# TissueImageAnalytics/cerberus

Measured on AMD Instinct MI355X. Metric: Mpx/sec WSI tiled inference (all heads), higher is better.
Workload: dtype f32

## Files before the change

cerberus_amd/csrc/cerb_api.hip:

```cpp
#include "cerb_net.h"

static thread_local std::string g_err;
int cerb_set_error(const std::string& m) {
    g_err = m;
    return 1;
}
extern "C" int cerb_version(void) { return 4; }
extern "C" const char* cerb_last_error(void) { return g_err.c_str(); }
std::atomic<long long> g_devbuf_bytes{0};
extern "C" size_t cerb_device_bytes_held(void) { const long long v = g_devbuf_bytes.load(); return v > 0 ? (size_t)v : 0; }
thread_local hipStream_t g_call_stream = nullptr;

static int alloc_dev(cerb_net* net, size_t bytes, void** out) {
    if (net->reusing) {
        if (net->reuse_cursor >= net->n_finalize_allocs || net->dev_alloc_bytes[net->reuse_cursor] != bytes)
            return fail("reload: the tensors do not have the shapes the handle was finalized with");
        *out = net->dev_allocs[net->reuse_cursor++];
        return 0;
    }
    void* d = nullptr;
    HIP_OK(hipMalloc(&d, bytes));
    net->dev_allocs.push_back(d);
    net->dev_alloc_bytes.push_back(bytes);
    *out = d;
// ... 246 lines not shown
}

void cerb_host_pack_patch_class(const float* w1, const float* b1, const float* scale2, const float* shift2, const float* w2, const float* b2, int out_ch,
                                std::vector<float>* w1t_out, std::vector<float>* b1f_out, std::vector<float>* w2t_out, std::vector<float>* b2f_out) {
    std::vector<float>&w1t = *w1t_out, &b1f = *b1f_out, &w2t = *w2t_out, &b2f = *b2f_out;
    w1t.assign(512 * 256, 0.f); b1f.assign(256, 0.f); w2t.assign(256 * 16, 0.f); b2f.assign(16, 0.f);
    for (int o = 0; o < 256; ++o) {
        for (int c = 0; c < 512; ++c) w1t[(size_t)c * 256 + o] = w1[(size_t)o * 512 + c] * scale2[o];
        b1f[o] = b1[o] * scale2[o] + shift2[o];
    }
    for (int o = 0; o < out_ch; ++o) {
        for (int c = 0; c < 256; ++c) w2t[(size_t)c * 16 + o] = w2[(size_t)o * 256 + c];
        b2f[o] = b2[o];
    }
}

static int store_bn(cerb_net* net, const std::string& name, const std::vector<std::string>& bnkeys, int ch) {
    std::vector<float> ga, be;
    for (const std::string& k : bnkeys) {
        const HostTensor *w, *b;
        if (get(net, k + ".weight", {ch}, &w) || get(net, k + ".bias", {ch}, &b)) return 1;
        ga.insert(ga.end(), w->data.begin(), w->data.end());
        be.insert(be.end(), b->data.begin(), b->data.end());
    }
    cerb_net::BnDev d;
    d.C = ch;
    d.groups = (int)bnkeys.size();
    if (upload(net, ga, &d.gamma) || upload(net, be, &d.beta)) return 1;
    for (size_t g = 0; g < bnkeys.size(); ++g) {
        net->param_slots[bnkeys[g] + ".weight"].push_back({d.gamma + g * ch, ch});
        net->param_slots[bnkeys[g] + ".bias"].push_back({d.beta + g * ch, ch});
    }
    net->bn[name] = d;
    net->bn_keys[name] = bnkeys;
    return 0;
}

static int make_conv(cerb_net* net, const std::string& name, const std::vector<std::string>& wkeys,
                     const std::vector<std::string>& bkeys, const std::vector<std::string>& bnkeys, int cout, int cin, int ks,
                     int stride) {
    const int CB = cerb_conv_chunk(ks, stride);
    if (cout % 64 || cin % CB) return fail("conv " + name + ": unsupported channel counts");
    std::vector<float> wp, bp, wwino, hw;
    const bool wino = (ks == 3 && stride == 1 && cin % 32 == 0);
    for (size_t g = 0; g < wkeys.size(); ++g) {
        const HostTensor* w;
        if (get(net, wkeys[g], {cout, cin, ks, ks}, &w)) return 1;
        Fold f;
        bool have_bn = !bnkeys.empty() && net->fold_bn;
        if (have_bn && bn_fold(net, bnkeys[g], cout, &f)) return 1;
        if (net->fold_bn) {
            pack_conv(w->data.data(), have_bn ? f.scale.data() : nullptr, cout, cin, ks, CB, &wp);
            if (wino) {
                pack_wino(w->data.data(), have_bn ? f.scale.data() : nullptr, cout, cin, &wwino);
                const size_t b0 = hw.size();
                hw.insert(hw.end(), w->data.begin(), w->data.end());
                if (have_bn)
                    for (int co = 0; co < cout; ++co)
                        for (size_t e = 0; e < (size_t)cin * 9; ++e) hw[b0 + (size_t)co * cin * 9 + e] *= f.scale[co];
            }
        }
        const HostTensor* b = nullptr;
        if (!bkeys.empty() && get(net, bkeys[g], {cout}, &b)) return 1;
        for (int c = 0; c < cout; ++c) {
            float v = b ? b->data[c] : 0.f;
            if (have_bn) v = v * f.scale[c] + f.shift[c];
            bp.push_back(v);
        }
    }
    if (!net->fold_bn && !bnkeys.empty() && store_bn(net, name, bnkeys, cout)) return 1;
    if (!net->fold_bn) {
        std::vector<float> rw, rb;
        for (size_t g = 0; g < wkeys.size(); ++g) {
            const HostTensor* w;
            if (get(net, wkeys[g], {cout, cin, ks, ks}, &w)) return 1;
            rw.insert(rw.end(), w->data.begin(), w->data.end());
            if (!bkeys.empty()) {
                const HostTensor* b;
                if (get(net, bkeys[g], {cout}, &b)) return 1;
                rb.insert(rb.end(), b->data.begin(), b->data.end());
            }
        }
        cerb_net::RawW r;
        r.wkeys = wkeys; r.bkeys = bkeys; r.bnkeys = bnkeys;
        if (upload(net, rw, &r.w) || (!rb.empty() && upload(net, rb, &r.b))) return 1;
        for (size_t g = 0; g < wkeys.size(); ++g) {
            const long long nwg = (long long)cout * cin * ks * ks;
            net->param_slots[wkeys[g]].push_back({r.w + g * nwg, nwg});
            if (r.b) net->param_slots[bkeys[g]].push_back({r.b + g * cout, cout});
        }
        net->raw[name] = r;
    }
    PackedConv pc;
    pc.cin = cin; pc.cout = cout; pc.ks = ks; pc.stride = stride; pc.groups = (int)wkeys.size();
    if (upload(net, bp, &pc.b)) return 1;
    if (!net->fold_bn)
        for (size_t g = 0; g < bkeys.size(); ++g) net->param_slots[bkeys[g]].push_back({pc.b + g * cout, cout});
    if (net->fold_bn) {
        if (upload(net, wp, &pc.w)) return 1;
        if (wino && upload(net, wwino, &pc.wino)) return 1;
        pc.host_w.swap(hw);
    } else {
        const float* rawd = net->raw[name].w;
        const size_t G = wkeys.size(), nw = (size_t)cout * cin * ks * ks, nu = (size_t)cout * cin * 16;
        const bool dgrad = ks == 3 && cin % 64 == 0 && cout % 32 == 0;
        void *dwp = nullptr, *dwi = nullptr, *ddg = nullptr;
        if (alloc_dev(net, G * nw * 4, &dwp) || (wino && alloc_dev(net, G * nu * 4, &dwi)) || (dgrad && alloc_dev(net, G * nu * 4, &ddg))) return 1;
        pc.w = reinterpret_cast<float*>(dwp);
        pc.wino = reinterpret_cast<float*>(dwi);
        pc.wino_dgrad = reinterpret_cast<float*>(ddg);
        for (size_t g = 0; g < G; ++g) {
            HIP_OK(cerb_launch_pack_conv(rawd + g * nw, pc.w + g * nw, cout, cin, ks, CB, 0));
            if (wino) HIP_OK(cerb_launch_pack_wino(rawd + g * nw, pc.wino + g * nu, cout, cin, 0, 0));
            if (dgrad) HIP_OK(cerb_launch_pack_wino(rawd + g * nw, pc.wino_dgrad + g * nu, cin, cout, 1, 0));
        }
    }
    net->conv[name] = pc;
    return 0;
}


extern "C" int cerb_net_finalize(cerb_net* net) {
    if (!net) return fail("cerb_net_finalize: null handle");
    if (net->finalized) return 0;
    if (!net->fold_bn && net->trunk_idx.size() != net->dense_idx.size())
        return fail("cerb_net_finalize: a decoder with several output heads runs in inference only (the training tape sums one head's gradient per decoder)");
    {
        const HostTensor* w;
        if (get(net, "backbone.conv1.weight", {64, 3, 7, 7}, &w)) return 1;
        Fold f;
        if (bn_fold(net, "backbone.bn1", 64, &f)) return 1;
        if (!net->fold_bn) {
            f.scale.assign(64, 1.f);
            f.shift.assign(64, 0.f);
            if (store_bn(net, "stem", {"backbone.bn1"}, 64)) return 1;
        }
        std::vector<float> wp;
        cerb_host_pack_stem(w->data.data(), f.scale.data(), &wp);
        if (upload(net, wp, &net->stem_w) || upload(net, f.shift, &net->stem_b)) return 1;
        if (!net->fold_bn) {
            if (upload(net, w->data, &net->stem_raw)) return 1;
            net->param_slots["backbone.conv1.weight"].push_back({net->stem_raw, 64 * 147});
        }
    }
    int inpl = 64;
    for (int li = 0; li < 4; ++li) {
        const int planes = kFilters[li + 1];
        for (int b = 0; b < kLayers[li]; ++b) {
            const std::string p = "backbone.layer" + std::to_string(li + 1) + "." + std::to_string(b);
            const int stride = (b == 0 && li > 0) ? 2 : 1;
            if (make_conv(net, p + ".conv1", {p + ".conv1.weight"}, {}, {p + ".bn1"}, planes, inpl, 3, stride)) return 1;
            if (make_conv(net, p + ".conv2", {p + ".conv2.weight"}, {}, {p + ".bn2"}, planes, planes, 3, 1)) return 1;
            if (stride != 1 || inpl != planes)
                if (make_conv(net, p + ".downsample", {p + ".downsample.0.weight"}, {}, {p + ".downsample.1"}, planes, inpl, 1, stride)) return 1;
            inpl = planes;
        }
    }
    if (make_conv(net, "conv_map", {"conv_map.weight"}, {}, {}, 256, 512, 1, 1)) return 1;
    const int dec_in[4] = {256, 128, 64, 64};
    const int dec_u[4][2] = {{256, 128}, {128, 64}, {64, 64}, {64, 64}};
    if (!net->dense_idx.empty()) {
        for (int u = 0; u < 4; ++u) {
            int c = dec_in[u];
            for (int j = 0; j < 2; ++j) {
                std::vector<std::string> wk, bk, bnk;
                for (int di : net->trunk_idx) {
                    const std::string p = "decoder_head." + net->dec[di].name + "." + std::to_string(u) + ".block." + std::to_string(j);
                    wk.push_back(p + ".conv.weight");
                    bk.push_back(p + ".conv.bias");
                    bnk.push_back(p + ".bn");
                }
                if (make_conv(net, "dec." + std::to_string(u) + "." + std::to_string(j), wk, bk, bnk, dec_u[u][j], c, 3, 1)) return 1;
                c = dec_u[u][j];
            }
        }
        for (int di : net->dense_idx) {
            const DecoderCfg& d = net->dec[di];
            const std::string p = "output_head." + d.name + "." + d.head + ".x";
            const HostTensor *w1, *b1, *w2, *b2;
            Fold f;
            if (get(net, p + ".0.block.0.conv.weight", {96, 64, 1, 1}, &w1) || get(net, p + ".0.block.0.conv.bias", {96}, &b1) ||
                bn_fold(net, p + ".0.block.0.bn", 96, &f) || get(net, p + ".1.conv.weight", {d.out_ch, 96, 1, 1}, &w2) ||
                get(net, p + ".1.conv.bias", {d.out_ch}, &b2))
                return 1;
            std::vector<float> w1p, b1p, w2p, b2p, w2q;
            cerb_host_pack_head(w1->data.data(), b1->data.data(), f.scale.data(), f.shift.data(), w2->data.data(), b2->data.data(), d.out_ch, &w1p, &b1p, &w2p, &b2p, &w2q);
            if (!net->fold_bn) {
                float *r1, *rb1, *r2, *rb2;
                if (upload(net, w1->data, &r1) || upload(net, b1->data, &rb1) || upload(net, w2->data, &r2) || upload(net, b2->data, &rb2)) return 1;
                net->head_rw1.push_back(r1); net->head_rb1.push_back(rb1); net->head_rw2.push_back(r2); net->head_rb2.push_back(rb2);
                net->param_slots[p + ".0.block.0.conv.weight"].push_back({r1, 96 * 64});
                net->param_slots[p + ".0.block.0.conv.bias"].push_back({rb1, 96});
                net->param_slots[p + ".1.conv.weight"].push_back({r2, (long long)d.out_ch * 96});
                net->param_slots[p + ".1.conv.bias"].push_back({rb2, d.out_ch});
                if (store_bn(net, "head." + std::to_string(net->head_rw1.size() - 1), {p + ".0.block.0.bn"}, 96)) return 1;
            }
            float *dw1, *db1, *dw2, *db2;
            float* dw2q;
            if (upload(net, w1p, &dw1) || upload(net, b1p, &db1) || upload(net, w2p, &dw2) || upload(net, b2p, &db2) || upload(net, w2q, &dw2q)) return 1;
            net->head_w1.push_back(dw1); net->head_b1.push_back(db1); net->head_w2.push_back(dw2); net->head_b2.push_back(db2); net->head_w2q.push_back(dw2q);
        }
    }
    if (net->pc_idx >= 0) {
        const int oc = net->dec[net->pc_idx].out_ch;
        const std::string p = "decoder_head.Patch-Class";
        Fold f1, f2;
        const HostTensor *w1, *b1, *w2, *b2;
        if (bn_fold(net, p + ".bn1", 512, &f1) || bn_fold(net, p + ".bn2", 256, &f2) || get(net, p + ".conv1.weight", {256, 512, 1, 1}, &w1) ||
            get(net, p + ".conv1.bias", {256}, &b1) || get(net, p + ".conv2.weight", {oc, 256, 1, 1}, &w2) || get(net, p + ".conv2.bias", {oc}, &b2))
            return 1;
        if (!net->fold_bn) {
            if (upload(net, w1->data, &net->pc_rw1) || upload(net, b1->data, &net->pc_rb1) || upload(net, w2->data, &net->pc_rw2) ||
                upload(net, b2->data, &net->pc_rb2) || store_bn(net, "pc.bn1", {p + ".bn1"}, 512) || store_bn(net, "pc.bn2", {p + ".bn2"}, 256))
                return 1;
            net->param_slots[p + ".conv1.weight"].push_back({net->pc_rw1, 256 * 512});
            net->param_slots[p + ".conv1.bias"].push_back({net->pc_rb1, 256});
            net->param_slots[p + ".conv2.weight"].push_back({net->pc_rw2, (long long)oc * 256});
            net->param_slots[p + ".conv2.bias"].push_back({net->pc_rb2, oc});
        }
        std::vector<float> w1t, b1f, w2t, b2f;
        cerb_host_pack_patch_class(w1->data.data(), b1->data.data(), f2.scale.data(), f2.shift.data(), w2->data.data(), b2->data.data(), oc, &w1t, &b1f, &w2t, &b2f);
        if (upload(net, f1.scale, &net->pc_bn1s) || upload(net, f1.shift, &net->pc_bn1b) || upload(net, w1t, &net->pc_w1t) ||
            upload(net, b1f, &net->pc_b1) || upload(net, w2t, &net->pc_w2t) || upload(net, b2f, &net->pc_b2))
            return 1;
    }
    if (!net->fold_bn) {
        std::vector<float> z(512, 0.f);
        if (upload(net, z, &net->zero_bias)) return 1;
    }
    if (!net->fold_bn) HIP_OK(hipDeviceSynchronize());
    if (net->reusing && net->reuse_cursor != net->n_finalize_allocs) return fail("reload: fewer tensors than the handle was finalized with");
    if (!net->reusing) net->n_finalize_allocs = net->dev_allocs.size();
    net->reusing = false;
    net->host.clear();
    net->finalized = true;
    return 0;
}

int prof_begin(cerb_net* net, const std::string& name, const std::string& kernel, double flops, hipStream_t st) {
    if (!net->profiling) return 0;
    if (net->prof_n == net->prof.size()) {
        cerb_net::ProfRec r;
        HIP_OK(hipEventCreate(&r.e0));
        HIP_OK(hipEventCreate(&r.e1));
        net->prof.push_back(r);
    }
    cerb_net::ProfRec& r = net->prof[net->prof_n];
    r.name = name; r.kernel = kernel; r.flops = flops;
    HIP_OK(hipEventRecord(r.e0, st));
    net->prof_open = true;
    return 0;
}
int prof_end(cerb_net* net, hipStream_t st) {
    if (!net->profiling) return 0;
    HIP_OK(hipEventRecord(net->prof[net->prof_n].e1, st));
    net->prof_n++;
    net->prof_open = false;
    return 0;
}

int train_wino2_fresh(cerb_net* net, const std::string& name, PackedConv& cm, int dgrad, hipStream_t st) {
    if (net->fold_bn) return 0;
    bool& used = dgrad ? cm.wino_dgrad_used : cm.wino_used;
    bool& stale = dgrad ? cm.wino_dgrad_stale : cm.wino_stale;
    used = true;
    if (!stale) return 0;
    auto rit = net->raw.find(name);
    if (rit == net->raw.end()) return fail("conv " + name + ": no raw weights to re-pack");
    const size_t nw = (size_t)cm.cout * cm.cin * 9, nu = (size_t)cm.cout * cm.cin * 16;
    for (int g = 0; g < cm.groups; ++g)
        HIP_OK(cerb_launch_pack_wino(rit->second.w + g * nw, (dgrad ? cm.wino_dgrad : cm.wino) + g * nu, dgrad ? cm.cin : cm.cout, dgrad ? cm.cout : cm.cin, dgrad, st));
    stale = false;
    return 0;
}

int train_wino4_slot(cerb_net* net, const std::string& name, PackedConv& cm, int w4b, int dgrad, hipStream_t st, float** out) {
    float*& slot = cm.wino4_t[w4b][dgrad];
    if (!slot) {
        auto rit = net->raw.find(name);
        if (rit == net->raw.end()) return fail("conv " + name + ": no raw weights for the F(4x4) transform");
        const size_t nw = (size_t)cm.cout * cm.cin * 9, nu = (size_t)cm.cout * cm.cin * 36;
        void* d = nullptr;
        HIP_OK(hipMalloc(&d, (size_t)cm.groups * nu * 4));
        net->dev_allocs.push_back(d);
        net->dev_alloc_bytes.push_back((size_t)cm.groups * nu * 4);
        slot = (float*)d;
        (void)nw;
        HIP_OK(cerb_launch_pack_wino4(rit->second.w, slot, dgrad ? cm.cin : cm.cout, dgrad ? cm.cout : cm.cin, dgrad, w4b, cm.groups, st));
    }
    *out = slot;
    return 0;
}

static constexpr int kPlanarLowest = 0;
static constexpr int kEncPlanarStages = 0x7;
static const char* const kPlanarFamily[4] = {"conv_wino4_planar<f4x4,16x16x2,eighth-res>", "conv_wino4_planar<f4x4,16x16x2,quarter-res>",
                                             "conv_wino4p<f4x4,16x16x2,planar,half-res>", "conv_wino4p<f4x4,16x16x2,planar>"};
static const char* const kEncPlanarFamily = "conv_wino4_enc<f4x4,16x16x2>";
static const char* const kEncPlanarFamilyRes = "conv_wino4_enc<f4x4,16x16x2,res>";
static const char* const kPlanarEntryFamily[4] = {"upsample2_add_planar<eighth-res>", "upsample2_add_planar<quarter-res>", "upsample2_add_planar", "upsample2_add_planar"};

int run_conv(cerb_net* net, const std::string& name, const float* in, const float* prev, const float* resid, float* out, int N,
             int H, int W, int relu, int mode, long long in_gs, long long prev_gs, hipStream_t st, double* macs,
             const int* roi, long long planar_out_gs) {
    auto it = net->conv.find(name);
    if (it == net->conv.end()) return fail("internal: conv " + name + " not packed");
    const PackedConv& c = it->second;
    struct BnReq {
        cerb_net* n;
        ~BnReq() { n->conv_bn_part = nullptr; }
    } bn_req{net};
    net->conv_bn_bpg = 0;
    ConvParams p;
    memset(&p, 0, sizeof(p));
    p.in = in; p.prev = prev; p.wpack = c.w; p.bias = c.b; p.resid = resid; p.out = out;
    p.N = N; p.H = H; p.W = W; p.Cin = c.cin; p.Cout = c.cout;
    p.Ho = (c.stride == 2) ? H / 2 : H;
    p.Wo = (c.stride == 2) ? W / 2 : W;
    p.relu = relu;
    p.groups = c.groups;
    p.in_gs = in_gs; p.prev_gs = prev_gs;
    p.w_gs = (long long)c.cout * c.cin * c.ks * c.ks;
    p.bias_gs = c.cout;
    p.resid_gs = 0;
    p.out_gs = (long long)N * p.Ho * p.Wo * c.cout;
    p.pk_off = net->packed_items ? 0 : 1;
    if (macs) {
        *macs += (double)c.groups * N * p.Ho * p.Wo * (double)c.cout * c.cin * c.ks * c.ks;
        if (!out) return 0;
    }
    const double fl = 2.0 * (double)c.groups * N * p.Ho * p.Wo * (double)c.cout * c.cin * c.ks * c.ks;
    const long long map_px = (long long)p.Ho * p.Wo;
    const bool use_w4 = net->conv_algo == 5 || net->conv_algo == 7 || (net->conv_algo == 6 && map_px >= 256);
    const bool planar = planar_out_gs > 0;
    static const long long w4b_max_px = [] {
        const char* e = cerb_dev_getenv("CERB_W4B_MAX_PX");
        return e ? atoll(e) : 4096ll;
    }();
    const bool w4b = !planar && (net->conv_algo == 7 || (net->conv_algo == 6 && map_px <= w4b_max_px)) && c.cin % 64 == 0;
    const bool enc_planar = planar && net->planar_level == 4;
    if (enc_planar && c.stride == 2) {
        if (resid || mode != 0 || !net->fold_bn) return fail("internal: conv " + name + " cannot store tile-planar");
        p.out_gs = planar_out_gs;
        p.pl_byp = cerb_planar_blocks(p.Ho);
        p.pl_bxp = cerb_planar_blocks(p.Wo);
        const std::string kn = "conv_igemm_planar<ks" + std::to_string(c.ks) + ",s2" + (p.Wo < 32 ? ",16x16>" : ",8x32>");
        if (prof_begin(net, name, kn, fl, st)) return 1;
        HIP_OK(cerb_launch_conv(p, c.ks, c.stride, mode, st));
        if (prof_end(net, st)) return 1;
        return 0;
    }
    if (planar && !(use_w4 && c.wino && mode == 0 && net->fold_bn && (!resid || enc_planar))) return fail("internal: conv " + name + " cannot take the planar path");
    if (use_w4 && c.wino && mode == 0 && (!it->second.host_w.empty() || !net->fold_bn)) {
        PackedConv& cm = it->second;
        float* train_slot = nullptr;
        if (!net->fold_bn && train_wino4_slot(net, name, cm, w4b ? 1 : 0, 0, st, &train_slot)) return 1;
        float*& slot4 = !net->fold_bn ? train_slot : (w4b ? cm.wino4b : cm.wino4);
        if (!slot4) {
            std::vector<float> w4;
            for (int g = 0; g < cm.groups; ++g) pack_wino4(cm.host_w.data() + (size_t)g * cm.cout * cm.cin * 9, cm.cout, cm.cin, &w4, w4b ? 1 : 0);
            void* d = nullptr;
            HIP_OK(hipMalloc(&d, w4.size() * 4));
            net->dev_allocs.push_back(d);
            net->dev_alloc_bytes.push_back(w4.size() * 4);
            HIP_OK(hipMemcpy(d, w4.data(), w4.size() * 4, hipMemcpyHostToDevice));
            slot4 = (float*)d;
        }
        p.wpack = slot4;
        p.w_gs = (long long)c.cout * c.cin * 36;
        double fl_done = fl;
        if (roi && roi[1] > roi[0] && roi[3] > roi[2]) {
            p.roi_y0 = roi[0]; p.roi_y1 = roi[1]; p.roi_x0 = roi[2]; p.roi_x1 = roi[3];
            const double ty = (roi[1] + 15) / 16 - roi[0] / 16, tx = (roi[3] + 15) / 16 - roi[2] / 16;
            fl_done = fl * (ty * 16.0 * tx * 16.0) / ((double)p.Ho * p.Wo);
        }
        if (planar) {
            p.out_gs = planar_out_gs;
            p.level_tag = enc_planar ? (resid ? 4 : 3) : net->planar_level == 3 ? 1 : net->planar_level == 2 ? 0 : 2;
            p.pl_byp = cerb_planar_blocks(p.Ho);
            p.pl_bxp = cerb_planar_blocks(p.Wo);
        }
        if (prof_begin(net, name, enc_planar ? (resid ? kEncPlanarFamilyRes : kEncPlanarFamily) : planar ? kPlanarFamily[net->planar_level & 3] : w4b ? (cerb_wino4b_packed(p) ? (resid ? "conv_wino4b<f4x4,16t,res>" : "conv_wino4b<f4x4,16t>") : (resid ? "conv_wino4b<f4x4,16x16,res>" : "conv_wino4b<f4x4,16x16>")) : (resid ? "conv_wino4<f4x4,16x16x2,res>" : "conv_wino4<f4x4,16x16x2>"), fl_done, st)) return 1;
        if (net->conv_bn_part && !planar && !resid && !(roi && roi[1] > roi[0] && roi[3] > roi[2])) {
            p.bn_part = net->conv_bn_part;
            net->conv_bn_bpg = w4b ? cerb_wino4b_bn_blocks(p) : N * ((p.Ho + 15) / 16) * ((p.Wo + 15) / 16);
        }
        HIP_OK(planar ? cerb_launch_wino4p(p, st) : w4b ? cerb_launch_wino4b(p, st) : cerb_launch_wino4(p, st));
        if (prof_end(net, st)) return 1;
        return 0;
    }
    if (net->conv_algo && c.wino && mode == 0) {
        if (train_wino2_fresh(net, name, it->second, 0, st)) return 1;
        p.wpack = c.wino;
        p.w_gs = (long long)c.cout * c.cin * 16;
        double fl_done = fl;
        if (roi && roi[1] > roi[0] && roi[3] > roi[2]) {
            p.roi_y0 = roi[0]; p.roi_y1 = roi[1]; p.roi_x0 = roi[2]; p.roi_x1 = roi[3];
            const double ty = (roi[1] + 7) / 8 - roi[0] / 8, tx = (roi[3] + 15) / 16 - roi[2] / 16;
            fl_done = fl * (ty * 8.0 * tx * 16.0) / ((double)p.Ho * p.Wo);
        }
        if (prof_begin(net, name, resid ? "conv_wino<f2x2,8x16,res>" : "conv_wino<f2x2,8x16>", fl_done, st)) return 1;
        HIP_OK(cerb_launch_wino(p, st));
        if (prof_end(net, st)) return 1;
        return 0;
    }
    const std::string kn = "conv_igemm<ks" + std::to_string(c.ks) + ",s" + std::to_string(c.stride) + ",mode" + std::to_string(mode) +
                           (p.Wo < 32 ? ",16x16>" : ",8x32>");
    if (prof_begin(net, name, kn, fl, st)) return 1;
    HIP_OK(cerb_launch_conv(p, c.ks, c.stride, mode, st));
    if (prof_end(net, st)) return 1;
    return 0;
}

static int forward_impl(cerb_net* net, const cerb_forward_io* io, hipStream_t st, double* macs) {
    g_call_stream = st;
    const bool dry = (macs != nullptr) && (io->tiles == nullptr) && (io->tiles_f32 == nullptr);
    const int N = io->n, H = io->h, W = io->w;
    if (N <= 0 || H <= 0 || W <= 0 || (H % 16) || (W % 16)) return fail("cerb_net_forward: tile H,W must be positive multiples of 16");
    const int out_h = io->out_h > 0 ? io->out_h : H, out_w = io->out_w > 0 ? io->out_w : W;
    if (out_h > H || out_w > W) return fail("cerb_net_forward: crop larger than tile");
    const int hs[5] = {H, H / 2, H / 4, H / 8, H / 16}, ws[5] = {W, W / 2, W / 4, W / 8, W / 16};
    const size_t D = net->trunk_idx.size();
    const size_t guard = cerb_conv_guard_bytes(W);
    const int planar_lowest = [] {
        const char* e = cerb_dev_getenv("CERB_PLANAR_LOWEST");
        return e ? atoi(e) : kPlanarLowest;
    }();
    auto level_is_planar = [&](int u) {
        if (dry || !net->planar || !net->fold_bn || net->conv_algo != 6 || net->head_algo < 1) return false;
        for (int v = 3; v >= u; --v) {
            if (v < planar_lowest) return false;
            auto c0 = net->conv.find("dec." + std::to_string(v) + ".0"), c1 = net->conv.find("dec." + std::to_string(v) + ".1");
            if (c0 == net->conv.end() || c1 == net->conv.end() || !c0->second.wino || !c1->second.wino) return false;
            const long long px = (long long)hs[3 - v] * ws[3 - v];
            if ((hs[3 - v] & 3) || (ws[3 - v] & 3)) return false;
            const bool ok = v >= 2 ? px >= 4096 && c0->second.cin == 64 && c0->second.cout == 64 && c1->second.cout == 64
                                   : px >= 256 && c0->second.cin % 16 == 0 && c0->second.cout % 64 == 0 && c1->second.cin == c0->second.cout && c1->second.cout % 64 == 0;
            if (!ok) return false;
        }
        return true;
    };
    if (!dry) {
        if (net->x0.ensure((size_t)N * H * W * 64 * 4, guard) || net->pool.ensure((size_t)N * hs[1] * ws[1] * 64 * 4, guard)) return fail_alloc();
        for (int i = 1; i < 5; ++i)
            if (net->x[i].ensure((size_t)N * hs[i] * ws[i] * kFilters[i] * 4, guard)) return fail_alloc();
        if (net->ta.ensure((size_t)N * hs[1] * ws[1] * 64 * 4, guard) || net->tb.ensure((size_t)N * hs[1] * ws[1] * 64 * 4, guard) ||
            net->cm.ensure((size_t)N * hs[4] * ws[4] * 256 * 4, guard))
            return fail_alloc();
        if (D) {
            static const bool exact_ws = cerb_dev_getenv("CERB_LEGACY_WS") == nullptr;
            size_t need_sum = 0, need_mid = 0;
            const int oc[4] = {128, 64, 64, 64};
            for (int u = 0; u < 4; ++u) {
                if (exact_ws && level_is_planar(u)) continue;
                const std::string n0 = "dec." + std::to_string(u) + ".0";
                auto c0 = net->conv.find(n0);
                const size_t px = (size_t)D * N * hs[3 - u] * ws[3 - u];
                need_sum = std::max(need_sum, px * (size_t)(c0 != net->conv.end() ? c0->second.cin : 256) * 4);
                need_mid = std::max(need_mid, px * (size_t)(c0 != net->conv.end() ? c0->second.cout : 256) * 4);
            }
            if (!exact_ws) need_sum = need_mid = D * (size_t)N * H * W * 64 * 4;
            if (net->dmid.ensure(need_mid, guard)) return fail_alloc();
            if (net->conv_algo && net->dsum.ensure(need_sum, guard)) return fail_alloc();
            for (int u = 0; u < 4; ++u) {
                if (exact_ws && level_is_planar(u)) continue;
                if (net->dout[u].ensure(D * (size_t)N * hs[3 - u] * ws[3 - u] * oc[u] * 4, guard)) return fail_alloc();
            }
        }
    }
    if (macs) *macs += (double)N * H * W * 64.0 * 147.0;
    if (!dry) {
        StemParams sp;
        sp.tiles = io->tiles; sp.tiles_f32 = io->tiles ? nullptr : io->tiles_f32; sp.wpack = net->stem_w; sp.bias = net->stem_b; sp.out = net->x0.p; sp.N = N; sp.H = H; sp.W = W; sp.relu = 1;
        sp.tiles_x = sp.tiles_y = 0;
        if (prof_begin(net, "stem", "stem_conv7x7", 2.0 * N * H * W * 64.0 * 147.0, st)) return 1;
        HIP_OK(cerb_launch_stem(sp, st));
        if (prof_end(net, st)) return 1;
    }
    const int enc_mask = [] {
        const char* e = cerb_dev_getenv("CERB_ENC_PLANAR");
        return e ? atoi(e) : kEncPlanarStages;
    }();
    auto encoder_stage_is_planar = [&](int li) {
        if (dry || !net->planar || !net->fold_bn || net->conv_algo != 6 || !((enc_mask >> li) & 1)) return false;
        const int hh = hs[li + 1], ww = ws[li + 1], planes = kFilters[li + 1];
        if ((hh & 15) || (ww & 15) || hh < 16 || ww < 16 || planes % 64) return false;
        for (int b = 0; b < kLayers[li]; ++b)
            for (int j = 1; j <= 2; ++j) {
                auto c = net->conv.find("backbone.layer" + std::to_string(li + 1) + "." + std::to_string(b) + ".conv" + std::to_string(j));
                if (c == net->conv.end()) return false;
                if (c->second.stride == 1 && (!c->second.wino || c->second.host_w.empty() || c->second.cin % 16)) return false;
            }
        return true;
    };
    if (!dry) {
        if (encoder_stage_is_planar(0)) {
            if (net->enc_a[0].ensure(1, N, hs[1], ws[1], 64, st)) return fail_alloc();
            if (prof_begin(net, "maxpool", "maxpool3x3s2_planar", 0.0, st)) return 1;
            HIP_OK(cerb_launch_maxpool_planar(net->x0.p, net->enc_a[0].b.p, N, H, W, 64, st));
            if (prof_end(net, st)) return 1;
        } else {
            if (prof_begin(net, "maxpool", "maxpool3x3s2", 0.0, st)) return 1;
            HIP_OK(cerb_launch_maxpool(net->x0.p, net->pool.p, N, H, W, 64, st));
            if (prof_end(net, st)) return 1;
        }
    }
    float* cur = dry ? nullptr : net->pool.p;
    int inpl = 64;
    for (int li = 0; li < 4; ++li) {
        const int planes = kFilters[li + 1];
        const int Hi = (li == 0) ? hs[1] : hs[li], Wi = (li == 0) ? ws[1] : ws[li];
        if (encoder_stage_is_planar(li)) {
            PlanarBuf &ba = net->enc_a[li], &bb = net->enc_b[li];
            const int hh = hs[li + 1], ww = ws[li + 1];
            if (ba.ensure(1, N, hh, ww, planes, st) || bb.ensure(1, N, hh, ww, planes, st)) return fail_alloc();
            const int keep_level = net->planar_level;
            net->planar_level = 4;
            struct Restore { cerb_net* n; int v; ~Restore() { n->planar_level = v; } } restore{net, keep_level};
            for (int b = 0; b < kLayers[li]; ++b) {
                const std::string p = "backbone.layer" + std::to_string(li + 1) + "." + std::to_string(b);
                if (b == 0 && li > 0) {
                    if (run_conv(net, p + ".conv1", cur, nullptr, nullptr, bb.b.p, N, Hi, Wi, 1, 0, 0, 0, st, macs, nullptr, bb.gs())) return 1;
                    if (run_conv(net, p + ".downsample", cur, nullptr, nullptr, ba.b.p, N, Hi, Wi, 0, 0, 0, 0, st, macs, nullptr, ba.gs())) return 1;
                } else if (run_conv(net, p + ".conv1", ba.b.p, nullptr, nullptr, bb.b.p, N, hh, ww, 1, 0, ba.gs(), 0, st, macs, nullptr, bb.gs())) {
                    return 1;
                }
                if (run_conv(net, p + ".conv2", bb.b.p, nullptr, ba.b.p, ba.b.p, N, hh, ww, 1, 0, bb.gs(), 0, st, macs, nullptr, ba.gs())) return 1;
            }
            if (prof_begin(net, "backbone.layer" + std::to_string(li + 1) + ".exit", "planar_to_nhwc", 0.0, st)) return 1;
            HIP_OK(cerb_launch_planar_to_nhwc(ba.b.p, net->x[li + 1].p, N, hh, ww, planes, st));
            if (prof_end(net, st)) return 1;
            cur = net->x[li + 1].p;
            inpl = planes;
            continue;
        }
        for (int b = 0; b < kLayers[li]; ++b) {
            const std::string p = "backbone.layer" + std::to_string(li + 1) + "." + std::to_string(b);
            const int stride = (b == 0 && li > 0) ? 2 : 1;
            const int hin = (b == 0) ? Hi : hs[li + 1], win = (b == 0) ? Wi : ws[li + 1];
            float* t1 = dry ? nullptr : net->ta.p;
            const bool last = (b == kLayers[li] - 1);
            float* outb = dry ? nullptr : (((kLayers[li] - 1 - b) % 2 == 0) ? net->x[li + 1].p : net->tb.p);
            (void)last;
            const float* idt = cur;
            if (run_conv(net, p + ".conv1", cur, nullptr, nullptr, t1, N, hin, win, 1, 0, 0, 0, st, macs)) return 1;
            if (stride != 1 || inpl != planes) {
                float* ds = dry ? nullptr : net->pool.p;
                if (run_conv(net, p + ".downsample", cur, nullptr, nullptr, ds, N, hin, win, 0, 0, 0, 0, st, macs)) return 1;
                idt = ds;
            }
            if (run_conv(net, p + ".conv2", t1, nullptr, idt, outb, N, hs[li + 1], ws[li + 1], 1, 0, 0, 0, st, macs)) return 1;
            cur = outb;
            inpl = planes;
        }
    }
    if (run_conv(net, "conv_map", dry ? nullptr : net->x[4].p, nullptr, nullptr, dry ? nullptr : net->cm.p, N, hs[4], ws[4], 0, 0, 0, 0, st, macs)) return 1;

    const long long tile_stride = io->tile_stride ? io->tile_stride : (long long)out_h * out_w;
    const long long row_stride = io->row_stride ? io->row_stride : out_w;
    if (net->pc_idx >= 0) {
        if (macs) *macs += (double)N * (512.0 * 256 + 256.0 * net->dec[net->pc_idx].out_ch);
        const bool want = io->out && io->out[net->pc_idx];
        const bool wantl = io->logits && io->logits[net->pc_idx];
        if (!dry && (want || wantl)) {
            PatchClassParams pp;
            memset(&pp, 0, sizeof(pp));
            pp.x4 = net->x[4].p; pp.bn1_s = net->pc_bn1s; pp.bn1_b = net->pc_bn1b; pp.w1t = net->pc_w1t; pp.b1 = net->pc_b1;
            pp.w2t = net->pc_w2t; pp.b2 = net->pc_b2;
            pp.N = N; pp.Hf = hs[4]; pp.Wf = ws[4]; pp.out_ch = net->dec[net->pc_idx].out_ch;
            pp.out_h = out_h; pp.out_w = out_w;
            pp.logits = wantl ? io->logits[net->pc_idx] : nullptr;
            pp.out = want ? (float*)io->out[net->pc_idx] : nullptr;
            pp.tile_off = io->tile_off; pp.tile_stride = tile_stride; pp.row_stride = row_stride;
            if (prof_begin(net, "patch_class", "patch_class", 2.0 * N * (512.0 * 256 + 256.0 * pp.out_ch), st)) return 1;
            HIP_OK(cerb_launch_patch_class(pp, st));
            if (prof_end(net, st)) return 1;
        }
    }
    if (D) {
        const float* skips[4] = {dry ? nullptr : net->x[3].p, dry ? nullptr : net->x[2].p, dry ? nullptr : net->x[1].p, dry ? nullptr : net->x0.p};
        const float* prev = dry ? nullptr : net->cm.p;
        long long prev_gs = 0;
        const int oc[4] = {128, 64, 64, 64};
        int roi_out[4][4], roi_mid[4][4], roi_sum[4][4];
        const bool any_logits = [&] {
            if (!io->logits) return false;
            for (size_t k = 0; k < net->dec.size(); ++k)
                if (io->logits[k]) return true;
            return false;
        }();
        const bool use_roi = !dry && net->crop_roi && (net->conv_algo == 1 || net->conv_algo >= 5) && !any_logits && (out_h < H || out_w < W);
        if (use_roi) {
            int y0 = (int)((H - out_h) * 0.5), x0 = (int)((W - out_w) * 0.5), y1 = y0 + out_h, x1 = x0 + out_w;
            for (int u = 3; u >= 0; --u) {
                const int hh = hs[3 - u], ww = ws[3 - u];
                auto widen = [&](int* r, const int* in, int d) {
                    r[0] = std::max(0, (in[0] - d) & ~3); r[1] = std::min(hh, (in[1] + d + 3) & ~3);
                    r[2] = std::max(0, (in[2] - d) & ~3); r[3] = std::min(ww, (in[3] + d + 3) & ~3);
                };
                const int win[4] = {y0, y1, x0, x1};
                widen(roi_out[u], win, 0);
                widen(roi_mid[u], roi_out[u], 1);
                widen(roi_sum[u], roi_mid[u], 1);
                y0 = std::max(0, roi_sum[u][0] / 2 - 1); y1 = std::min(hh / 2, (roi_sum[u][1] - 1) / 2 + 2);
                x0 = std::max(0, roi_sum[u][2] / 2 - 1); x1 = std::min(ww / 2, (roi_sum[u][3] - 1) / 2 + 2);
            }
        }
        bool feat_planar = false, prev_planar = false;
        for (int u = 0; u < 4; ++u) {
            const int hh = hs[3 - u], ww = ws[3 - u];
            const std::string n0 = "dec." + std::to_string(u) + ".0", n1 = "dec." + std::to_string(u) + ".1";
            const int cmid = net->conv[n0].cout;
            const int cin0 = net->conv[n0].cin;
            const bool lvl_planar = level_is_planar(u);
            if (lvl_planar) {
                PlanarBuf &bs = u == 3 ? net->psum : u == 2 ? net->psum2 : u == 1 ? net->psum1 : net->psum0;
                PlanarBuf &bm = u == 3 ? net->pmid : u == 2 ? net->pmid2 : u == 1 ? net->pmid1 : net->pmid0;
                const int cout1 = net->conv[n1].cout;
                PlanarBuf& bo = cout1 == cin0 ? bs : u == 1 ? net->pout1 : net->pout0;
                if (bs.ensure((int)D, N, hh, ww, cin0, st) || bm.ensure((int)D, N, hh, ww, cmid, st) || (&bo != &bs && bo.ensure((int)D, N, hh, ww, cout1, st)))
                    return fail_alloc();
                if (prof_begin(net, n0 + ".up", kPlanarEntryFamily[u], 0.0, st)) return 1;
                HIP_OK(cerb_launch_upsample2_add_planar(skips[u], prev, bs.b.p, (int)D, N, hh, ww, cin0, prev_gs, bs.gs(), use_roi ? roi_sum[u] : nullptr, prev_planar ? 1 : 0, st));
                if (prof_end(net, st)) return 1;
                net->planar_level = u;
                if (run_conv(net, n0, bs.b.p, nullptr, nullptr, bm.b.p, N, hh, ww, 1, 0, bs.gs(), 0, st, macs, use_roi ? roi_mid[u] : nullptr, bm.gs()))
                    return 1;
                if (run_conv(net, n1, bm.b.p, nullptr, nullptr, bo.b.p, N, hh, ww, 1, 0, bm.gs(), 0, st, macs, use_roi ? roi_out[u] : nullptr, bo.gs()))
                    return 1;
                if (u == 3) feat_planar = true;
                prev = bo.b.p;
                prev_gs = bo.gs();
                prev_planar = true;
                continue;
            }
            if (prev_planar) return fail("internal: a tile-planar decoder level feeds an NHWC one");
            if (net->conv_algo && net->conv[n0].wino && !dry) {
                if (prof_begin(net, n0 + ".up", "upsample2_add", 0.0, st)) return 1;
                HIP_OK(cerb_launch_upsample2_add(skips[u], prev, net->dsum.p, (int)D, N, hh, ww, cin0, prev_gs, use_roi ? roi_sum[u] : nullptr, st));
                if (prof_end(net, st)) return 1;
                if (run_conv(net, n0, net->dsum.p, nullptr, nullptr, net->dmid.p, N, hh, ww, 1, 0, (long long)N * hh * ww * cin0, 0, st, macs,
                             use_roi ? roi_mid[u] : nullptr))
                    return 1;
            } else if (run_conv(net, n0, skips[u], prev, nullptr, dry ? nullptr : net->dmid.p, N, hh, ww, 1, 1, 0, prev_gs, st, macs)) return 1;
            if (run_conv(net, n1, dry ? nullptr : net->dmid.p, nullptr, nullptr, dry ? nullptr : net->dout[u].p, N, hh, ww, 1, 0,
                         (long long)N * hh * ww * cmid, 0, st, macs, use_roi ? roi_out[u] : nullptr))
                return 1;
            prev = dry ? nullptr : net->dout[u].p;
            prev_gs = (long long)N * hh * ww * oc[u];
        }
        HeadParams hps[8];
        int n_hp = 0;
        double head_flops = 0.0;
        for (size_t k = 0; k < net->dense_idx.size(); ++k) {
            const int di = net->dense_idx[k];
            const size_t tk = (size_t)net->trunk_of[k];
            const DecoderCfg& d = net->dec[di];
            if (macs) *macs += (double)N * H * W * (64.0 * 96 + 96.0 * d.out_ch);
            const bool want = io->out && io->out[di];
            const bool wantl = io->logits && io->logits[di];
            if (dry || !(want || wantl)) continue;
            HeadParams hp;
            memset(&hp, 0, sizeof(hp));
            hp.feat = feat_planar ? net->psum.b.p + tk * net->psum.gs() : net->dout[3].p + tk * (size_t)N * H * W * 64;
            hp.feat_planar = feat_planar ? 1 : 0;
            hp.pl_byp = cerb_planar_blocks(H);
            hp.pl_bxp = cerb_planar_blocks(W);
            hp.w1p = net->head_w1[k]; hp.b1 = net->head_b1[k]; hp.w2p = net->head_w2[k]; hp.b2 = net->head_b2[k]; hp.w2q = net->head_w2q[k];
            hp.N = N; hp.H = H; hp.W = W; hp.out_ch = d.out_ch; hp.kind = d.kind;
            hp.crop_y0 = (int)((H - out_h) * 0.5); hp.crop_x0 = (int)((W - out_w) * 0.5);
            hp.out_h = want ? out_h : 0; hp.out_w = want ? out_w : 0;
            hp.roi = use_roi ? 1 : 0;
            hp.logits = wantl ? io->logits[di] : nullptr;
            hp.absmax_bits = io->logit_absmax ? io->logit_absmax + di : nullptr;
            if (want) {
                if (d.kind == 0) hp.out_inst = (float*)io->out[di];
                else if (io->type_is_u8) hp.out_type_u8 = (unsigned char*)io->out[di];
                else hp.out_type_i64 = (long long*)io->out[di];
            }
            hp.tile_off = io->tile_off; hp.tile_stride = tile_stride; hp.row_stride = row_stride;
            const double head_px = hp.roi ? (double)out_h * (((hp.crop_x0 + out_w + 15) / 16 - hp.crop_x0 / 16) * 16.0) : (double)H * W;
            const double fl = 2.0 * N * head_px * (64.0 * 96 + 96.0 * d.out_ch);
            if (net->head_algo == 0) {
                if (prof_begin(net, "head." + d.name, "head", fl, st)) return 1;
                HIP_OK(cerb_launch_head(hp, st));
                if (prof_end(net, st)) return 1;
            } else {
                if (n_hp == 8) {
                    if (prof_begin(net, "heads", "head_group", head_flops, st)) return 1;
                    HIP_OK(cerb_launch_head_group(hps, n_hp, st, net->head_algo == 1 ? 1 : 0));
                    if (prof_end(net, st)) return 1;
                    n_hp = 0;
                    head_flops = 0.0;
                }
                hps[n_hp++] = hp;
                head_flops += fl;
            }
        }
        if (n_hp > 0) {
            if (prof_begin(net, "heads", "head_group", head_flops, st)) return 1;
            HIP_OK(cerb_launch_head_group(hps, n_hp, st, net->head_algo == 1 ? 1 : 0));
            if (prof_end(net, st)) return 1;
        }
    }
    if (!dry && io->feats) {
        const float* src[6] = {net->x0.p, net->x[1].p, net->x[2].p, net->x[3].p, net->cm.p, net->x[4].p};
        const size_t nb[6] = {(size_t)N * H * W * 64, (size_t)N * hs[1] * ws[1] * 64, (size_t)N * hs[2] * ws[2] * 128,
                              (size_t)N * hs[3] * ws[3] * 256, (size_t)N * hs[4] * ws[4] * 256, (size_t)N * hs[4] * ws[4] * 512};
        for (int i = 0; i < 6; ++i)
            if (io->feats[i]) HIP_OK(hipMemcpyAsync(io->feats[i], src[i], nb[i] * 4, hipMemcpyDeviceToDevice, st));
    }
    return 0;
}

extern "C" int cerb_net_begin_reload(cerb_net* net) {
    if (!net) return fail("cerb_net_begin_reload: null handle");
    HIP_OK(hipDeviceSynchronize());
    while (net->dev_allocs.size() > net->n_finalize_allocs) {
        (void)hipFree(net->dev_allocs.back());
        net->dev_allocs.pop_back();
        net->dev_alloc_bytes.pop_back();
    }
    net->reusing = true;
    net->reuse_cursor = 0;
    net->param_slots.clear();
    net->conv.clear();
    net->bn.clear();
    net->raw.clear();
    net->grads.clear();
    net->head_w1.clear(); net->head_b1.clear(); net->head_w2.clear(); net->head_b2.clear(); net->head_w2q.clear();
    net->head_rw1.clear(); net->head_rb1.clear(); net->head_rw2.clear(); net->head_rb2.clear();
    net->host.clear();
    net->finalized = false;
    return 0;
}
extern "C" int cerb_net_update_params(cerb_net* net, int count, const char* const* keys, const float* const* dev_src, void* hip_stream) {
    if (!net || count < 0 || (count && (!keys || !dev_src))) return fail("cerb_net_update_params: bad arguments");
    if (!net->finalized || net->fold_bn) return fail("cerb_net_update_params: needs a finalized handle packed for training (cerb_net_set_fold_bn(net, 0))");
    hipStream_t st = (hipStream_t)hip_stream;
    std::vector<float*> cd;
    std::vector<const float*> cs;
    std::vector<long long> cn;
    for (int i = 0; i < count; ++i) {
        auto it = net->param_slots.find(keys[i]);
        if (it == net->param_slots.end()) continue;
        if (!dev_src[i]) return fail(std::string("cerb_net_update_params: null source for ") + keys[i]);
        for (const cerb_net::ParamSlot& sl : it->second) {
            cd.push_back(sl.dst); cs.push_back(dev_src[i]); cn.push_back(sl.n);
        }
    }
    HIP_OK(cerb_launch_copy_multi((int)cd.size(), cd.data(), cs.data(), cn.data(), &net->copy_tab, &net->copy_tab_bytes, &net->copy_tab_host, st));
    HIP_OK(cerb_launch_pack_stem(net->stem_raw, net->stem_w, st));
    static const bool per_conv = cerb_dev_getenv("CERB_PACK_PER_CONV") != nullptr;
    std::vector<PackJob> jobs;
    auto job = [&](const float* w, float* out, long long total, int cout, int cin, int kind, int a, int b) { jobs.push_back(PackJob{w, out, total, cout, cin, kind, a, b, 0}); };
    for (auto& kv : net->conv) {
        PackedConv& pc = kv.second;
        const float* rawd = net->raw[kv.first].w;
        if (pc.wino && !pc.wino_used) pc.wino_stale = true;
        if (pc.wino_dgrad && !pc.wino_dgrad_used) pc.wino_dgrad_stale = true;
        const size_t nw = (size_t)pc.cout * pc.cin * pc.ks * pc.ks, nu = (size_t)pc.cout * pc.cin * 16, nu4 = (size_t)pc.cout * pc.cin * 36;
        for (int g = 0; g < pc.groups; ++g) {
            if (per_conv) {
                HIP_OK(cerb_launch_pack_conv(rawd + g * nw, pc.w + g * nw, pc.cout, pc.cin, pc.ks, cerb_conv_chunk(pc.ks, pc.stride), st));
                if (pc.wino && pc.wino_used) HIP_OK(cerb_launch_pack_wino(rawd + g * nw, pc.wino + g * nu, pc.cout, pc.cin, 0, st));
                if (pc.wino_dgrad && pc.wino_dgrad_used) HIP_OK(cerb_launch_pack_wino(rawd + g * nw, pc.wino_dgrad + g * nu, pc.cin, pc.cout, 1, st));
                continue;
            }
            job(rawd + g * nw, pc.w + g * nw, (long long)nw, pc.cout, pc.cin, 0, pc.ks * pc.ks, cerb_conv_chunk(pc.ks, pc.stride));
            if (pc.wino && pc.wino_used) job(rawd + g * nw, pc.wino + g * nu, (long long)nu, pc.cout, pc.cin, 1, 0, 0);
            if (pc.wino_dgrad && pc.wino_dgrad_used) job(rawd + g * nw, pc.wino_dgrad + g * nu, (long long)nu, pc.cin, pc.cout, 1, 1, 0);
        }
        for (int l = 0; l < 2; ++l)
            for (int dg = 0; dg < 2; ++dg)
                if (pc.wino4_t[l][dg]) {
                    if (per_conv) {
                        HIP_OK(cerb_launch_pack_wino4(rawd, pc.wino4_t[l][dg], dg ? pc.cin : pc.cout, dg ? pc.cout : pc.cin, dg, l, pc.groups, st));
                        continue;
                    }
                    for (int g = 0; g < pc.groups; ++g)
                        job(rawd + g * nw, pc.wino4_t[l][dg] + g * nu4, (long long)nu4, dg ? pc.cin : pc.cout, dg ? pc.cout : pc.cin, 2, dg, l);
                }
    }
    if (!jobs.empty()) HIP_OK(cerb_launch_pack_multi(jobs.data(), (int)jobs.size(), &net->pack_tab, &net->pack_tab_bytes, &net->pack_tab_host, st));
    return 0;
}
extern "C" int cerb_net_set_fold_bn(cerb_net* net, int fold) {
    if (!net) return fail("cerb_net_set_fold_bn: null handle");
    if (net->finalized) return fail("cerb_net_set_fold_bn: must be called before cerb_net_finalize");
    net->fold_bn = fold ? 1 : 0;
    return 0;
}

extern "C" int cerb_net_forward(cerb_net* net, const cerb_forward_io* io, void* hip_stream) {
    if (!net || !io) return fail("cerb_net_forward: null argument");
    if (!net->finalized) return fail("cerb_net_forward: call cerb_net_finalize first");
    if (!io->tiles && !io->tiles_f32) return fail("cerb_net_forward: null tiles pointer (neither tiles nor tiles_f32)");
    if (!net->fold_bn) return fail("cerb_net_forward: the network was packed for training (cerb_net_set_fold_bn(net, 0)); use cerb_net_forward_train");
    net->prof_n = 0;
    return forward_impl(net, io, (hipStream_t)hip_stream, nullptr);
}

extern "C" double cerb_net_flops(const cerb_net* net, int n, int h, int w) {
    if (!net || !net->finalized) return -1.0;
    cerb_forward_io io;
    memset(&io, 0, sizeof(io));
    io.n = n; io.h = h; io.w = w;
    double macs = 0.0;
    if (forward_impl(const_cast<cerb_net*>(net), &io, nullptr, &macs)) return -1.0;
    return 2.0 * macs;
}

extern "C" int cerb_net_set_crop_roi(cerb_net* net, int enable) {
    if (!net) return fail("cerb_net_set_crop_roi: null handle");
    net->crop_roi = enable ? 1 : 0;
    return 0;
}
extern "C" int cerb_net_set_conv_algo(cerb_net* net, int algo) {
    if (!net) return fail("cerb_net_set_conv_algo: null handle");
    if (algo < 0 || algo > 7 || (algo >= 2 && algo <= 4))
        return fail("cerb_net_set_conv_algo: algo must be 0 (direct), 1 (Winograd F(2x2) fp32), 5 (Winograd F(4x4) fp32), 7 (F(4x4), one-block items with 32-channel chunks) or 6 (F(4x4) for maps of 16 x 16 pixels and more -- 7's kernel up to 64 x 64, 5's above --, else F(2x2): the default); 2-4 were experiments (scripts/experiments/)");
    net->conv_algo = algo;
    return 0;
}

extern "C" int cerb_net_set_bn_eval(cerb_net* net, const char* bn_prefix, const float* running_mean, const float* running_var, int channels) {
    if (!net || !bn_prefix) return fail("cerb_net_set_bn_eval: null argument");
    if (!net->finalized || net->fold_bn) return fail("cerb_net_set_bn_eval: needs a finalized network packed with cerb_net_set_fold_bn(net, 0)");
    for (auto& kv : net->bn_keys) {
        const std::vector<std::string>& keys = kv.second;
        for (size_t g = 0; g < keys.size(); ++g) {
            if (keys[g] != bn_prefix) continue;
            auto it = net->bn.find(kv.first);
            if (it == net->bn.end()) return fail(std::string("cerb_net_set_bn_eval: internal: no BatchNorm ") + kv.first);
            cerb_net::BnDev& b = it->second;
            if (!running_mean || !running_var) {
                if (g < b.eval.size()) b.eval[g] = 0;
                return 0;
            }
            if (channels != b.C) return fail(std::string("cerb_net_set_bn_eval: ") + bn_prefix + " has " + std::to_string(b.C) + " channels");
            if (!b.run_mean) {
                void* d = nullptr;
                HIP_OK(hipMalloc(&d, (size_t)2 * b.groups * b.C * 4));
                net->dev_allocs.push_back(d);
                net->dev_alloc_bytes.push_back((size_t)2 * b.groups * b.C * 4);
                b.run_mean = (float*)d;
                b.run_rstd = b.run_mean + (size_t)b.groups * b.C;
                b.eval.assign(b.groups, 0);
            }
            std::vector<float> rs(b.C);
            for (int c = 0; c < b.C; ++c) rs[c] = 1.0f / sqrtf(running_var[c] + 1e-5f);
            HIP_OK(hipMemcpy(b.run_mean + g * b.C, running_mean, (size_t)b.C * 4, hipMemcpyHostToDevice));
            HIP_OK(hipMemcpy(b.run_rstd + g * b.C, rs.data(), (size_t)b.C * 4, hipMemcpyHostToDevice));
            b.eval[g] = 1;
            return 0;
        }
    }
    return fail(std::string("cerb_net_set_bn_eval: no BatchNorm with the state-dict prefix ") + bn_prefix);
}

extern "C" int cerb_net_set_planar(cerb_net* net, int enable) {
    if (!net) return fail("cerb_net_set_planar: null handle");
    if (enable < 0 || enable > 1) return fail("cerb_net_set_planar: 0 (NHWC) or 1 (tile-planar, conv_wino4p.hip)");
    net->planar = enable;
    return 0;
}

extern "C" int cerb_net_set_packed_items(cerb_net* net, int enable) {
    if (!net) return fail("cerb_net_set_packed_items: null handle");
    if (enable < 0 || enable > 1) return fail("cerb_net_set_packed_items: 0 (16 x 16 blocks everywhere) or 1 (16 consecutive tiles per item on maps that are not whole blocks)");
    net->packed_items = enable;
    return 0;
}

extern "C" int cerb_net_set_head_algo(cerb_net* net, int algo) {
    if (!net) return fail("cerb_net_set_head_algo: null handle");
    if (algo < 0 || algo > 2) return fail("cerb_net_set_head_algo: algo must be 0 (one launch per head), 1 (grouped launch) or 2 (round 3's grouped launch)");
    net->head_algo = algo;
    return 0;
}

extern "C" int cerb_net_profile_enable(cerb_net* net, int enable) {
    if (!net) return fail("cerb_net_profile_enable: null handle");
    net->profiling = enable != 0;
    net->prof_n = 0;
    return 0;
}
extern "C" int cerb_net_profile_count(cerb_net* net) { return net ? (int)net->prof_n : 0; }
extern "C" int cerb_net_profile_get(cerb_net* net, int idx, char* name, int name_cap, char* kernel, int kernel_cap, double* flops, float* ms) {
    if (!net || idx < 0 || (size_t)idx >= net->prof_n) return fail("cerb_net_profile_get: index out of range");
    cerb_net::ProfRec& r = net->prof[idx];
    HIP_OK(hipEventSynchronize(r.e1));
    HIP_OK(hipEventElapsedTime(ms, r.e0, r.e1));
    snprintf(name, name_cap, "%s", r.name.c_str());
    snprintf(kernel, kernel_cap, "%s", r.kernel.c_str());
    *flops = r.flops;
    return 0;
}

extern "C" int cerb_event_create(void** ev) {
    hipEvent_t e;
    HIP_OK(hipEventCreate(&e));
    *ev = (void*)e;
    return 0;
}
extern "C" int cerb_event_record(void* ev, void* hip_stream) {
    HIP_OK(hipEventRecord((hipEvent_t)ev, (hipStream_t)hip_stream));
    return 0;
}
extern "C" int cerb_event_elapsed_ms(void* a, void* b, float* ms) {
    HIP_OK(hipEventSynchronize((hipEvent_t)b));
    HIP_OK(hipEventElapsedTime(ms, (hipEvent_t)a, (hipEvent_t)b));
    return 0;
}
extern "C" int cerb_event_destroy(void* ev) {
    HIP_OK(hipEventDestroy((hipEvent_t)ev));
    return 0;
}
```

cerberus_amd/csrc/cerb_common.h:

```cpp
#pragma once
#include "cerb_dev.h"
#include <hip/hip_runtime.h>
#include <stdint.h>

typedef float f32x4 __attribute__((ext_vector_type(4)));
typedef float f32x16 __attribute__((ext_vector_type(16)));

#define CERB_WAVE 64

struct ConvParams {
    const float* in;
    const float* prev;
    const float* wpack;
    const float* bias;
    const float* resid;
    float* out;
    int N, H, W, Cin, Ho, Wo, Cout;
    int relu;
    int tiles_x, tiles_y;
    int roi_y0, roi_y1, roi_x0, roi_x1;
    int ty_off, tx_off;
    int groups;
    long long in_gs, prev_gs, w_gs, bias_gs, resid_gs, out_gs;
    int pl_byp, pl_bxp;
    int level_tag;
    double* bn_part;
    int bn_bpg;
    int pk_ty, pk_tx, pk_ntile;
    const float *bst_y, *bst_mean, *bst_rstd, *bst_gamma, *bst_beta;
    long long bst_y_gs;
    int pk_off;
};

__host__ __device__ static inline int cerb_planar_blocks(int px) { return (px + 15) / 16 + 2; }
static inline long long cerb_planar_elems(int n, int h, int w, int c) {
    return (long long)n * cerb_planar_blocks(h) * cerb_planar_blocks(w) * (c / 16) * 4096;
}
__host__ __device__ __forceinline__ long long cerb_planar_offset(int n, int y, int x, int cc, int byp, int bxp, int ncc) {
    return ((((long long)n * byp + (y >> 4) + 1) * bxp + (x >> 4) + 1) * ncc + cc) * 4096 + ((((y & 3) << 2) + (x & 3)) * 16 + (((y >> 2) & 3) << 2) + ((x >> 2) & 3)) * 16;
}

struct HeadParams {
    const float* feat;
    const float* w1p;
    const float* b1;
    const float* w2p;
    const float* w2q;
    const float* b2;
    int N, H, W;
    int out_ch;
    int kind;
    int crop_y0, crop_x0, out_h, out_w;
    int roi;
    int rows, row0, xa0, nxb;
    float* logits;
    float* out_inst;
    unsigned char* out_type_u8;
    long long* out_type_i64;
    const long long* tile_off;
    long long tile_stride;
    long long row_stride;
    unsigned int* absmax_bits;
    int feat_planar;
    int pl_byp, pl_bxp;
};

__device__ __forceinline__ int xcd_remap(int bid, int nblk) {
    const int q = nblk >> 3, r = nblk & 7;
    const int xcd = bid & 7, idx = bid >> 3;
    const int base = (xcd < r) ? xcd * (q + 1) : r * (q + 1) + (xcd - r) * q;
    return base + idx;
}
```

cerberus_amd/csrc/cerb_net.h:

```cpp
#ifndef CERB_NET_H
#define CERB_NET_H
#include <hip/hip_runtime.h>

#include <algorithm>
#include <cmath>
#include <cstdio>
#include <cstdlib>
#include <cstring>
#include <map>
#include <atomic>
#include <string>
#include <vector>

#include "../../include/cerberus_hip.h"
#include "cerb_common.h"

hipError_t cerb_launch_conv(const ConvParams& p, int ks, int stride, int mode, hipStream_t st);
hipError_t cerb_launch_wino(ConvParams p, hipStream_t st);
hipError_t cerb_launch_wino4(ConvParams p, hipStream_t st);
hipError_t cerb_launch_wino4b(ConvParams p, hipStream_t st);
int cerb_wino4b_bn_blocks(const ConvParams& p);
bool cerb_wino4b_packed(const ConvParams& p);
hipError_t cerb_launch_wino4p(ConvParams p, hipStream_t st);
hipError_t cerb_launch_upsample2_add_planar(const float* skip, const float* prev, float* out, int groups, int N, int H, int W, int C, long long prev_gs,
                                            long long out_gs, const int* roi, int prev_planar, hipStream_t st);
hipError_t cerb_launch_upsample2_add(const float* skip, const float* prev, float* out, int groups, int N, int H, int W, int C,
                                     long long prev_gs, const int* roi, hipStream_t st);
extern "C" int cerb_conv_chunk(int ks, int stride);
struct StemParams {
    const unsigned char* tiles;
    const float* tiles_f32;
    const float* wpack;
    const float* bias;
    float* out;
    int N, H, W, tiles_x, tiles_y;
    int relu;
};
hipError_t cerb_launch_stem(StemParams p, hipStream_t st);
size_t cerb_bn_workspace_bytes(int groups, long long rows, int C);
hipError_t cerb_launch_bn_stats(const float* x, long long group_stride, long long rows, int C, int groups, float eps, float* mean, float* rstd,
                                float* var_unbiased, void* ws, hipStream_t st);
hipError_t cerb_launch_bn_apply(float* x, const float* src, const float* resid, long long group_stride, long long rows, int C, int groups, const float* mean,
                                const float* rstd, const float* gamma, const float* beta, int relu, hipStream_t st);
hipError_t cerb_launch_bn_finalize(const double* partial, int blocks, long long rows, int C, float eps, float* mean, float* rstd, float* var_unbiased, hipStream_t st,
                                   int groups = 1, void* fold_ws = nullptr);
size_t cerb_bn_fold_workspace_bytes(int groups, int C);
hipError_t cerb_launch_pointwise(const float* in, const float* w, const float* bias, float* out, long long rows, int cin, int cout, const float* in_scale,
                                 hipStream_t st, double* bn_part = nullptr, int* bn_blocks = nullptr);
hipError_t cerb_launch_crop_gap(const float* x, int N, int H, int W, int C, int y0, int ch, int x0, int cw, float* out, hipStream_t st);
hipError_t cerb_launch_copy_multi(int count, float* const* dst, const float* const* src, const long long* n, void** dev_tab, size_t* dev_bytes,
                                  std::vector<char>* host_prev, hipStream_t st);
hipError_t cerb_launch_bn_bwd(const float* dz, const float* z, const float* y, float* dy, float* dresid, long long group_stride, long long rows, int C, int groups,
                              const float* mean, const float* rstd, const float* gamma, const float* beta, float* dgamma, float* dbeta, int relu, int dy_assign, void* ws, hipStream_t st, unsigned long long eval_mask = 0, int dresid_assign = 0,
                              const double* pre_part = nullptr, int pre_bpg = 0);
int cerb_head_bwd2_blocks();
hipError_t cerb_launch_conv_bwd(const float* x, const float* dy, const float* w, float* dx, float* dw, float* db, int G, int N, int H, int W, int Cin, int Cout,
                                int ks, int stride, long long x_gs, hipStream_t st);
hipError_t cerb_launch_stem_wgrad(const unsigned char* tiles, const float* dy, float* dw, int N, int H, int W, hipStream_t st);
hipError_t cerb_launch_maxpool_bwd(const float* x, const float* ypool, const float* dy, float* dx, int N, int H, int W, int C, hipStream_t st);
hipError_t cerb_launch_maxpool_idx(const float* in, float* out, unsigned* idx, int N, int H, int W, int C, hipStream_t st);
hipError_t cerb_launch_maxpool_bwd_idx(const unsigned* idx, const float* dy, float* dx, int N, int H, int W, int C, hipStream_t st);
bool cerb_upadd_bwd_fused_ok(int H, int W, int C, int G);
hipError_t cerb_launch_upadd_bwd(const float* dout, float* dskip, float* dprev, int G, int N, int H, int W, int C, long long prev_gs, int shared_prev, hipStream_t st,
                                 unsigned group_mask = 0xffffffffu, int skip_assign = 0, int prev_assign = 0);
hipError_t cerb_launch_pointwise_bwd(const float* x, const float* dy, const float* w, float* dx, float* dw, float* db, long long rows, int cin, int cout,
                                     const float* in_scale, int dx_assign, hipStream_t st);
hipError_t cerb_launch_crop_gap_bwd(const float* dg, float* dx, int N, int H, int W, int C, int y0, int ch, int x0, int cw, hipStream_t st);
hipError_t cerb_launch_adam(float* p, const float* g, float* m, float* v, long long n, float lr, float b1, float b2, float eps, int step, hipStream_t st);
size_t cerb_wgrad_workspace_bytes(int G, int N, int Ho, int Wo, int Cin, int Cout, int ks, int* slices_out);
size_t cerb_stem_wgrad_workspace_bytes();
hipError_t cerb_launch_pack_stem(const float* w_raw, float* out, hipStream_t st);
struct PackJob {
    const float* w;
    float* out;
    long long total;
    int cout, cin, kind, a, b, pad;
};
hipError_t cerb_launch_pack_multi(const PackJob* jobs, int count, void** dev_tab, size_t* dev_bytes, std::vector<char>* host_prev, hipStream_t st);
hipError_t cerb_launch_adam_multi(int count, float* const* p, const float* const* g, float* const* m, float* const* v, const long long* n, float lr, float b1,
                                  float b2, float eps, int step, hipStream_t st);
hipError_t cerb_launch_pack_conv(const float* w_raw, float* out, int cout, int cin, int ks, int chunk, hipStream_t st);
hipError_t cerb_launch_pack_wino(const float* w_raw, float* out, int cout, int cin, int dgrad, hipStream_t st);
hipError_t cerb_launch_pack_wino4(const float* w_raw, float* out, int cout, int cin, int dgrad, int chunk32, int groups, hipStream_t st);
hipError_t cerb_launch_dilate2(const float* dy, float* d, long long n, int H, int W, int C, hipStream_t st);
size_t cerb_pw_wgrad_small_workspace_bytes(long long rows, int cin, int cout);
hipError_t cerb_launch_pw_wgrad_small(const float* x, const float* dy, float* dw, long long rows, int cin, int cout, void* ws, hipStream_t st);
size_t cerb_pw_bwd_small_workspace_bytes(long long rows, int cin, int cout);
hipError_t cerb_launch_pw_bwd_small(const float* x, const float* dy, const float* w, float* dx, float* dw, float* db, long long rows, int cin, int cout,
                                    int dx_assign, void* ws, hipStream_t st);
hipError_t cerb_launch_stem_wgrad_mfma(const unsigned char* tiles, const float* dy, float* dw, int N, int H, int W, void* ws, hipStream_t st);
hipError_t cerb_launch_colsum(const float* d, long long group_stride, long long rows, int C, int G, float* out, void* ws, hipStream_t st);
bool cerb_wgrad_wino_supported(int H, int W, int Cin, int Cout);
size_t cerb_wgrad_wino_workspace_bytes(int G, int N, int H, int W, int Cin, int Cout);
hipError_t cerb_launch_wgrad_wino(const float* x, const float* dy, float* dw, int G, int N, int H, int W, int Cin, int Cout, long long x_gs, void* ws, hipStream_t st,
                                  float* db);
hipError_t cerb_launch_wgrad(const float* x, const float* dy, float* dw, int G, int N, int H, int W, int Cin, int Cout, int ks, int stride, long long x_gs, void* ws,
                             hipStream_t st, float* db = nullptr);
bool cerb_head_train_supported(long long rows, int cin, int chid, int out);
hipError_t cerb_launch_head_fwd1(const float* prev, const float* w1, const float* b1, float* hid, long long rows, double* bn_part, int* bn_blocks, hipStream_t st,
                                 const float* const* in_bn = nullptr);
hipError_t cerb_launch_head_fwd2(const float* hid, const float* mean, const float* rstd, const float* gamma, const float* beta, const float* w2, const float* b2,
                                 float* logits, long long rows, int out, hipStream_t st);
size_t cerb_head_bwd_workspace_bytes(long long rows, int out);
hipError_t cerb_launch_head_bwd1(const float* hid, const float* dlog, const float* mean, const float* rstd, const float* gamma, const float* beta, const float* w2,
                                 float* dw2, float* db2, float* dgamma, float* dbeta, long long rows, int out, void* ws, hipStream_t st);
hipError_t cerb_launch_head_bwd2(const float* hid, const float* dlog, const float* prev, const float* mean, const float* rstd, const float* gamma, const float* beta,
                                 const float* dgamma, const float* dbeta, const float* w1, const float* w2, float* dprev, float* dw1, float* db1, long long rows, int out,
                                 int eval_mode, int assign, void* ws, hipStream_t st, const float* const* in_bn = nullptr, double* in_part = nullptr);
hipError_t cerb_launch_maxpool(const float* in, float* out, int N, int H, int W, int C, hipStream_t st);
hipError_t cerb_launch_maxpool_planar(const float* in, float* out, int N, int H, int W, int C, hipStream_t st);
hipError_t cerb_launch_planar_to_nhwc(const float* in, float* out, int N, int H, int W, int C, hipStream_t st);
hipError_t cerb_launch_head(const HeadParams& p, hipStream_t st);
hipError_t cerb_launch_head_group(const HeadParams* heads, int n_heads, hipStream_t st, int w2_44);
struct PatchClassParams {
    const float* x4;
    const float* bn1_s;
    const float* bn1_b;
    const float* w1t;
    const float* b1;
    const float* w2t;
    const float* b2;
    int N, Hf, Wf, out_ch;
    int out_h, out_w;
    float* logits;
    float* out;
    const long long* tile_off;
    long long tile_stride, row_stride;
};
hipError_t cerb_launch_patch_class(const PatchClassParams& p, hipStream_t st);

int cerb_set_error(const std::string& m);
static inline int fail(const std::string& m) { return cerb_set_error(m); }
static inline int fail_alloc() { return cerb_set_error("workspace allocation failed") + 1; }
#define HIP_OK(expr)                                                                              \
    do {                                                                                          \
        hipError_t e_ = (expr);                                                                   \
        if (e_ != hipSuccess) return fail(std::string(#expr) + ": " + hipGetErrorString(e_));     \
    } while (0)

struct HostTensor {
    std::vector<int64_t> shape;
    std::vector<float> data;
};

extern "C" size_t cerb_conv_guard_bytes(int tile_w);
extern thread_local hipStream_t g_call_stream;
extern std::atomic<long long> g_devbuf_bytes;
struct DevBuf {
    float* p = nullptr;
    char* raw = nullptr;
    size_t bytes = 0, guard = 0, held = 0;
    int ensure(size_t need, size_t g) {
        if (need <= bytes && g <= guard) return 0;
        release();
        if (hipMalloc(&raw, need + 2 * g) != hipSuccess) {
            raw = nullptr;
            return 1;
        }
        g_devbuf_bytes += (long long)(need + 2 * g);
        held = need + 2 * g;
        if (hipMemsetAsync(raw, 0, need + 2 * g, g_call_stream) != hipSuccess) return 1;
        p = reinterpret_cast<float*>(raw + g);
        bytes = need;
        guard = g;
        return 0;
    }
    void release() {
        if (raw) {
            (void)hipFree(raw);
            g_devbuf_bytes -= (long long)held;
        }
        held = 0;
        raw = nullptr;
        p = nullptr;
        bytes = guard = 0;
    }
};

struct PlanarBuf {
    DevBuf b;
    int h = 0, w = 0, c = 0, groups = 0;
    long long cap_n = 0;
    long long per_image() const { return cerb_planar_elems(1, h, w, c); }
    long long gs() const { return cap_n * per_image(); }
    int ensure(int G, int N, int H, int W, int C, hipStream_t st) {
        if (H == h && W == w && C == c && G == groups && N <= cap_n) return 0;
        const size_t need = (size_t)G * (size_t)N * (size_t)cerb_planar_elems(1, H, W, C) * 4;
        if (need > b.bytes) {
            if (b.ensure(need, 0)) return 1;
        } else if (hipMemsetAsync(b.raw, 0, b.bytes + 2 * b.guard, st) != hipSuccess) {
            return 1;
        }
        h = H; w = W; c = C; groups = G;
        cap_n = (long long)(b.bytes / ((size_t)G * (size_t)cerb_planar_elems(1, H, W, C) * 4));
        return 0;
    }
    void release() { b.release(); h = w = c = groups = 0; cap_n = 0; }
};

struct PackedConv {
    int cin = 0, cout = 0, ks = 0, stride = 1, groups = 1;
    float* w = nullptr;
    float* wino = nullptr;
    float* wino_dgrad = nullptr;
    bool wino_used = false, wino_dgrad_used = false, wino_stale = false, wino_dgrad_stale = false;
    float* wino4_t[2][2] = {{nullptr, nullptr}, {nullptr, nullptr}};
    float* wino4b = nullptr;
    float* wino4 = nullptr;
    std::vector<float> host_w;
    float* b = nullptr;
};

struct DecoderCfg {
    std::string name, head;
    int out_ch = 0;
    int kind = 0;
};

struct cerb_net {
    std::vector<DecoderCfg> dec;
    std::vector<int> dense_idx;
    std::vector<int> trunk_idx;
    std::vector<int> trunk_of;
    int pc_idx = -1;
    std::map<std::string, HostTensor> host;
    bool finalized = false;
    float *stem_w = nullptr, *stem_b = nullptr;
    std::map<std::string, PackedConv> conv;
    std::vector<float*> head_w1, head_b1, head_w2, head_b2, head_w2q;
    float *pc_bn1s = nullptr, *pc_bn1b = nullptr, *pc_w1t = nullptr, *pc_b1 = nullptr, *pc_w2t = nullptr, *pc_b2 = nullptr;
    std::vector<void*> dev_allocs;
    std::vector<size_t> dev_alloc_bytes;
    size_t n_finalize_allocs = 0, reuse_cursor = 0;
    bool reusing = false;
    int fold_bn = 1;
    struct BnDev {
        float *gamma = nullptr, *beta = nullptr;
        int C = 0, groups = 1;
        float *run_mean = nullptr, *run_rstd = nullptr;
        std::vector<char> eval;
    };
    std::map<std::string, BnDev> bn;
    std::vector<float*> head_rw1, head_rb1, head_rw2, head_rb2;
    float *pc_rw1 = nullptr, *pc_rb1 = nullptr, *pc_rw2 = nullptr, *pc_rb2 = nullptr;
    DevBuf t_mean, t_rstd, t_ws, t_hid, t_gap, t_pc1, t_idn, t_dil;
    struct RawW { float* w = nullptr; float* b = nullptr; std::vector<std::string> wkeys, bkeys, bnkeys; };
    std::map<std::string, RawW> raw;
    struct ParamSlot { float* dst; long long n; };
    std::map<std::string, std::vector<ParamSlot>> param_slots;
    float* stem_raw = nullptr;
    std::vector<DevBuf> tape;
    size_t tape_pos = 0;
    void* copy_tab = nullptr;
    size_t copy_tab_bytes = 0;
    std::vector<char> copy_tab_host;
    void* pack_tab = nullptr;
    size_t pack_tab_bytes = 0;
    std::vector<char> pack_tab_host;
    float* zero_bias = nullptr;
    std::map<std::string, std::pair<float*, long long>> grads;
    std::map<std::string, std::vector<std::string>> bn_keys;
    DevBuf x0, pool, x[5], ta, tb, cm, dmid, dsum, dout[4];
    PlanarBuf psum, pmid, pout;
    int planar_level = 3;
    PlanarBuf psum2, pmid2, pout2;
    PlanarBuf psum1, pmid1, pout1, psum0, pmid0, pout0;
    PlanarBuf enc_a[4], enc_b[4];
    int packed_items = 1;
    int planar = 1;
    bool profiling = false;
    int crop_roi = 1;
    int head_algo = 1;
    int conv_algo = 6;
    struct ProfRec { std::string name, kernel; double flops; hipEvent_t e0, e1; };
    std::vector<ProfRec> prof;
    size_t prof_n = 0;
    bool prof_open = false;
    double* conv_bn_part = nullptr;
    int conv_bn_bpg = 0;
    hipStream_t side = nullptr;
    hipEvent_t ev_fork = nullptr, ev_join = nullptr;
    DevBuf t_ws2;
    ~cerb_net() {
        if (side) { (void)hipStreamSynchronize(side); (void)hipStreamDestroy(side); }
        if (ev_fork) (void)hipEventDestroy(ev_fork);
        if (ev_join) (void)hipEventDestroy(ev_join);
        t_ws2.release();
        for (auto& r : prof) { (void)hipEventDestroy(r.e0); (void)hipEventDestroy(r.e1); }
        for (void* p : dev_allocs) (void)hipFree(p);
        if (copy_tab) (void)hipFree(copy_tab);
        if (pack_tab) (void)hipFree(pack_tab);
        x0.release(); pool.release(); ta.release(); tb.release(); cm.release(); dmid.release(); dsum.release(); psum.release(); pmid.release(); pout.release(); psum2.release(); pmid2.release(); pout2.release(); psum1.release(); pmid1.release(); pout1.release(); psum0.release(); pmid0.release(); pout0.release();
        t_mean.release(); t_rstd.release(); t_ws.release(); t_hid.release(); t_gap.release(); t_pc1.release(); t_idn.release(); t_dil.release();
        for (auto& b : enc_a) b.release();
        for (auto& b : enc_b) b.release();
        for (auto& b : tape) b.release();
        for (auto& b : x) b.release();
        for (auto& b : dout) b.release();
    }
};


static const int kLayers[4] = {3, 4, 6, 3};
static const int kFilters[5] = {64, 64, 128, 256, 512};
void cerb_host_pack_conv(const float* w, int cout, int cin, int ks, int chunk, std::vector<float>* out);
void cerb_host_pack_stem(const float* w, const float* scale, std::vector<float>* out);
void cerb_host_pack_head(const float* w1, const float* b1, const float* scale, const float* shift, const float* w2, const float* b2, int out_ch,
                         std::vector<float>* w1p, std::vector<float>* b1p, std::vector<float>* w2p, std::vector<float>* b2p, std::vector<float>* w2q);
void cerb_host_pack_patch_class(const float* w1, const float* b1, const float* scale2, const float* shift2, const float* w2, const float* b2, int out_ch,
                                std::vector<float>* w1t, std::vector<float>* b1f, std::vector<float>* w2t, std::vector<float>* b2f);
void cerb_host_pack_wino(const float* w, int cout, int cin, std::vector<float>* out);
void cerb_host_pack_wino4(const float* w, int cout, int cin, int layout, std::vector<float>* out);
int prof_begin(cerb_net* net, const std::string& name, const std::string& kernel, double flops, hipStream_t st);
int prof_end(cerb_net* net, hipStream_t st);
int train_wino2_fresh(cerb_net* net, const std::string& name, PackedConv& cm, int dgrad, hipStream_t st);
int train_wino4_slot(cerb_net* net, const std::string& name, PackedConv& cm, int w4b, int dgrad, hipStream_t st, float** out);
int run_conv(cerb_net* net, const std::string& name, const float* in, const float* prev, const float* resid, float* out, int N, int H, int W, int relu, int mode,
             long long in_gs, long long prev_gs, hipStream_t st, double* macs, const int* roi = nullptr, long long planar_out_gs = 0);
#endif
```

cerberus_amd/csrc/conv_igemm.hip:

```cpp
#include "wino_common.h"

__device__ __forceinline__ f32x4 splat4(float x) {
    f32x4 r = {x, x, x, x};
    return r;
}

template <int KS, int STRIDE, int TH, int TW, int CB, int MODE>
struct ConvCfg {
    static constexpr int PAD = KS / 2;
    static constexpr int GSTEP = (KS == 1) ? STRIDE : 1;
    static constexpr int LSTEP = (KS == 1) ? 1 : STRIDE;
    static constexpr int IH = (KS == 1) ? TH : (TH - 1) * STRIDE + KS;
    static constexpr int IW = (KS == 1) ? TW : (TW - 1) * STRIDE + KS;
    static constexpr int PS = CB + 4;
    static constexpr int NG = CB / 8;
    static constexpr int T = KS * KS;
    static constexpr int NQ = T * NG;
    static constexpr int PARTS = CB / 4;
    static constexpr int PPS = 256 / PARTS;
    static constexpr int NF = IH * IW * PARTS;
    static constexpr int RPS = 32 / TW;
    static constexpr int NM = (IH + RPS - 1) / RPS;
    static constexpr int NE = (2 * IH * 8 + 255) / 256;
    static constexpr int ITER = (MODE == 1) ? NM + NE : (NF + 255) / 256;
    static constexpr int MAIN_FLOATS = IH * IW * PS;
    static constexpr int AR = TH / 2 + 2, AC = TW / 2 + 2;
    static constexpr int NA = AR * AC * PARTS;
    static constexpr int AITER = (NA + 255) / 256;
    static constexpr int AUX_FLOATS = (MODE == 1) ? AR * AC * PS : 0;
    static constexpr int LDS_FLOATS = MAIN_FLOATS + AUX_FLOATS;
    static constexpr int LDS_BYTES = LDS_FLOATS * 4;
    static constexpr int S_PREV = ITER;
    static constexpr int S_BAR = ITER + AITER + 6;
    static constexpr int S_COMB = S_BAR + 1;
    static constexpr int WD = (MODE == 0 && STRIDE == 1) ? 3 : 2;
};

struct Item {
    int g, cb, n, oy0, ox0, tx, ty;
};

template <int KS, int STRIDE, int TH, int TW, int CB, int MODE, bool PL = false>
__global__ __launch_bounds__(256, 2) void conv_igemm_kernel(ConvParams p) {
    using C = ConvCfg<KS, STRIDE, TH, TW, CB, MODE>;
    constexpr int WD = C::WD;
    static_assert(TH * TW == 256, "tile must hold 256 pixels (4 waves x 2 x 32)");
    static_assert(MODE == 0 || (KS == 3 && STRIDE == 1 && CB == 32 && C::IH % C::RPS == 0 && C::S_COMB + C::ITER <= C::NQ),
                  "MODE 1 schedule must fit in one chunk");
    static_assert(C::ITER <= 2 * C::NQ || KS == 1, "every staging slice needs a step");
    extern __shared__ __attribute__((aligned(16))) float lds[];

    const int tid = threadIdx.x;
    const int lane = tid & 63;
    const int wave = tid >> 6;
    const int j = lane & 31;
    const int h = lane >> 5;

    const int ncb = p.Cout >> 6;
    const int ntile = p.N * p.tiles_y * p.tiles_x;
    const int per_group = ntile * ncb;
    const int total = per_group * p.groups;
    const int nchunk = p.Cin / CB;
    const int lb = xcd_remap(blockIdx.x, gridDim.x);
    const int base_cnt = total / (int)gridDim.x, rem_cnt = total % (int)gridDim.x;
    int item = lb * base_cnt + min(lb, rem_cnt);
    const int item_end = item + base_cnt + (lb < rem_cnt ? 1 : 0);
    if (item >= item_end) return;

    auto decode = [&](int it) {
        Item w;
        w.g = it / per_group;
        int L = it - w.g * per_group;
        w.cb = L % ncb;
        int t_ = L / ncb;
        w.tx = t_ % p.tiles_x;
        t_ /= p.tiles_x;
        w.ty = t_ % p.tiles_y;
        w.n = t_ / p.tiles_y;
        w.oy0 = w.ty * TH;
        w.ox0 = w.tx * TW;
        return w;
    };
    auto advance = [&](Item w) {
        if (++w.cb == ncb) {
            w.cb = 0;
            if (++w.tx == p.tiles_x) {
                w.tx = 0;
                if (++w.ty == p.tiles_y) {
                    w.ty = 0;
                    if (++w.n == p.N) {
                        w.n = 0;
                        ++w.g;
                    }
                }
            }
        }
        w.oy0 = w.ty * TH;
        w.ox0 = w.tx * TW;
        return w;
    };
    auto in_base = [&](const Item& w) {
        return reinterpret_cast<const char*>(p.in + w.g * p.in_gs) +
               ((((long long)w.n * p.H + (w.oy0 * STRIDE - C::PAD)) * p.W + (w.ox0 * STRIDE - C::PAD)) * p.Cin) * 4;
    };
    auto w_base = [&](const Item& w) {
        return reinterpret_cast<const char*>(p.wpack + w.g * p.w_gs + (long long)w.cb * nchunk * C::NQ * 2 * 256);
    };
    auto touches_border = [&](const Item& w) {
        const int y0 = w.oy0 * STRIDE - C::PAD, x0 = w.ox0 * STRIDE - C::PAD;
        return y0 < 0 || x0 < 0 || y0 + (C::IH - 1) * C::GSTEP + 1 > p.H || x0 + (C::IW - 1) * C::GSTEP + 1 > p.W;
    };

    constexpr int RPS = C::RPS, NM = C::NM, NE = C::NE;
    unsigned soff[MODE == 1 ? 1 + NE : C::ITER];
    int ldsw0, ldswE = 0;
    bool e_last_ok = true;
    const int rowb = p.W * p.Cin * 4;
    if (MODE == 1) {
        const int mrow = (tid >> 3) / TW, mcol = (tid >> 3) % TW, part = tid & 7;
        soff[0] = (unsigned)(((mrow * p.W + mcol) * p.Cin + part * 4) * 4);
        ldsw0 = (mrow * C::IW + mcol) * C::PS + part * 4;
        const int e_iy = tid >> 4, e_ix = TW + ((tid >> 3) & 1);
#pragma unroll
        for (int k = 0; k < NE; ++k) {
            const int iy = min(e_iy + 16 * k, C::IH - 1);
            soff[1 + k] = (unsigned)(((iy * p.W + e_ix) * p.Cin + part * 4) * 4);
        }
        ldswE = (e_iy * C::IW + e_ix) * C::PS + part * 4;
        e_last_ok = e_iy + 16 * (NE - 1) < C::IH;
    } else {
#pragma unroll
        for (int s = 0; s < C::ITER; ++s) {
            const int f = min(tid + s * 256, C::NF - 1);
            const int pix = f / C::PARTS, part = f % C::PARTS;
            soff[s] = (unsigned)((((pix / C::IW) * C::GSTEP * p.W + (pix % C::IW) * C::GSTEP) * p.Cin + part * 4) * 4);
        }
        ldsw0 = (tid / C::PARTS) * C::PS + (tid % C::PARTS) * 4;
    }
    const unsigned wlane = (unsigned)lane * 16u;
    int ldsb[2];
    unsigned ooff[2];
#pragma unroll
    for (int q = 0; q < 2; ++q) {
        const int pl = (wave * 2 + q) * 32 + j;
        const int py = pl / TW, px = pl % TW;
        ldsb[q] = ((py * C::LSTEP) * C::IW + px * C::LSTEP) * C::PS + 4 * h;
        if constexpr (PL)
            ooff[q] = (unsigned)(((px >> 4) * (p.Cout >> 4) * 4096 + ((py & 3) * 4 + (px & 3)) * 256 + ((py >> 2) * 4 + ((px >> 2) & 3)) * 16 + 4 * h) * 4);
        else
            ooff[q] = (unsigned)(((py * p.Wo + px) * p.Cout + 4 * h) * 4);
    }
    float* aux = lds + C::MAIN_FLOATS;
    int aoffM = 0, aoffE[NE];
    float wM[4] = {0.f, 0.f, 0.f, 0.f}, wE[4] = {0.f, 0.f, 0.f, 0.f};
    int auxw0 = 0;
    if (MODE == 1) {
        const int mrow = (tid >> 3) / TW, mcol = (tid >> 3) % TW, part = tid & 7;
        aoffM = (mcol >> 1) * C::PS + part * 4;
        const float lxM = (mcol & 1) ? 0.75f : 0.25f;
        const float lyM = (RPS == 2 && (mrow & 1)) ? 0.75f : 0.25f;
        wM[0] = (1.f - lyM) * (1.f - lxM), wM[1] = (1.f - lyM) * lxM, wM[2] = lyM * (1.f - lxM), wM[3] = lyM * lxM;
        const int e_iy = tid >> 4, e_b = (tid >> 3) & 1;
#pragma unroll
        for (int k = 0; k < NE; ++k) aoffE[k] = ((min(e_iy + 16 * k, C::IH - 1) >> 1) * C::AC + TW / 2) * C::PS + part * 4;
        const float lxE = e_b ? 0.75f : 0.25f, lyE = (e_iy & 1) ? 0.75f : 0.25f;
        wE[0] = (1.f - lyE) * (1.f - lxE), wE[1] = (1.f - lyE) * lxE, wE[2] = lyE * (1.f - lxE), wE[3] = lyE * lxE;
        auxw0 = (tid / C::PARTS) * C::PS + (tid % C::PARTS) * 4;
    }

    f32x4 v[C::ITER];
    f32x4 pvv[C::AITER > 0 ? C::AITER : 1];
    unsigned poff[MODE == 1 ? C::AITER : 1];

    auto issue = [&](__amdgpu_buffer_rsrc_t r, int chunk_off, int s) {
        if (MODE == 1) {
            if (s < NM) v[s] = buf_load(r, soff[0], chunk_off + s * RPS * rowb);
            else v[s] = buf_load(r, soff[1 + s - NM], chunk_off);
        } else {
            v[s] = buf_load(r, soff[s], chunk_off);
        }
    };
    auto prev_offsets = [&](const Item& w) {
        const int Hp = p.H >> 1, Wp = p.W >> 1;
#pragma unroll
        for (int k = 0; k < C::AITER; ++k) {
            const int f = min(tid + k * 256, C::NA - 1);
            const int apix = f / C::PARTS, part = f % C::PARTS;
            const int py = min(max((w.oy0 >> 1) - 1 + apix / C::AC, 0), Hp - 1), px = min(max((w.ox0 >> 1) - 1 + apix % C::AC, 0), Wp - 1);
            poff[k] = (unsigned)(((py * Wp + px) * p.Cin + part * 4) * 4);
        }
    };
    auto prev_base = [&](const Item& w) {
        return reinterpret_cast<const char*>(p.prev + w.g * p.prev_gs + (long long)w.n * (p.H >> 1) * (p.W >> 1) * p.Cin);
    };
    auto write_prev = [&]() {
#pragma unroll
        for (int k = 0; k < C::AITER; ++k)
            if (tid + k * 256 < C::NA) *reinterpret_cast<f32x4*>(aux + auxw0 + k * C::PPS * C::PS) = pvv[k];
    };
    auto combine = [&](int s) {
        const bool main = s < NM;
        const float* a = main ? aux + aoffM + ((s * RPS) >> 1) * C::AC * C::PS : aux + aoffE[main ? 0 : s - NM];
        const f32x4 p00 = *reinterpret_cast<const f32x4*>(a);
        const f32x4 p01 = *reinterpret_cast<const f32x4*>(a + C::PS);
        const f32x4 p10 = *reinterpret_cast<const f32x4*>(a + C::AC * C::PS);
        const f32x4 p11 = *reinterpret_cast<const f32x4*>(a + C::AC * C::PS + C::PS);
        const bool swap = main && RPS == 1 && (s & 1);
        const float* wt = main ? wM : wE;
        f32x4 r = v[s];
        r = __builtin_elementwise_fma(splat4(wt[swap ? 2 : 0]), p00, r);
        r = __builtin_elementwise_fma(splat4(wt[swap ? 3 : 1]), p01, r);
        r = __builtin_elementwise_fma(splat4(wt[swap ? 0 : 2]), p10, r);
        r = __builtin_elementwise_fma(splat4(wt[swap ? 1 : 3]), p11, r);
        v[s] = r;
    };
    auto slice_iy = [&](int s) { return MODE == 1 ? (s < NM ? s * RPS + (tid >> 3) / TW : (tid >> 4) + 16 * (s - NM)) : ((tid + s * 256) / C::PARTS) / C::IW; };
    auto slice_ix = [&](int s) { return MODE == 1 ? (s < NM ? (tid >> 3) % TW : TW + ((tid >> 3) & 1)) : ((tid + s * 256) / C::PARTS) % C::IW; };
    auto slice_ptr = [&](int s) { return MODE == 1 ? (s < NM ? lds + ldsw0 + s * RPS * C::IW * C::PS : lds + ldswE + (s - NM) * 16 * C::IW * C::PS) : lds + ldsw0 + s * C::PPS * C::PS; };
    auto slice_live = [&](int s) { return MODE == 1 ? (s < C::ITER - 1 || e_last_ok) : (tid + s * 256 < C::NF); };
    auto write_tile = [&](const Item& w, bool masked) {
        if (!masked) {
#pragma unroll
            for (int s = 0; s < C::ITER; ++s)
                if (slice_live(s)) *reinterpret_cast<f32x4*>(slice_ptr(s)) = v[s];
        } else {
#pragma unroll
            for (int s = 0; s < C::ITER; ++s) {
                const int gy = w.oy0 * STRIDE - C::PAD + slice_iy(s) * C::GSTEP, gx = w.ox0 * STRIDE - C::PAD + slice_ix(s) * C::GSTEP;
                const bool ok = gy >= 0 && gy < p.H && gx >= 0 && gx < p.W;
                const f32x4 z = {0.f, 0.f, 0.f, 0.f};
                if (slice_live(s)) *reinterpret_cast<f32x4*>(slice_ptr(s)) = ok ? v[s] : z;
            }
        }
    };

    Item w = decode(item);
    {
        const __amdgpu_buffer_rsrc_t r0 = make_rsrc(in_base(w));
#pragma unroll
        for (int s = 0; s < C::ITER; ++s) issue(r0, 0, s);
    }
    if (MODE == 1) {
        prev_offsets(w);
        const __amdgpu_buffer_rsrc_t rp = make_rsrc(prev_base(w));
#pragma unroll
        for (int k = 0; k < C::AITER; ++k) pvv[k] = buf_load(rp, poff[k], 0);
        write_prev();
        __syncthreads();
#pragma unroll
        for (int s = 0; s < C::ITER; ++s) combine(s);
    }
    __amdgpu_buffer_rsrc_t rw = make_rsrc(w_base(w));
    f32x4 wq[WD + 1][2];
#pragma unroll
    for (int d = 0; d < WD; ++d)
#pragma unroll
        for (int s = 0; s < 2; ++s) wq[d][s] = buf_load(rw, wlane, (d * 2 + s) * 1024);

    for (;;) {
        f32x16 acc[2][2];
#pragma unroll
        for (int s = 0; s < 2; ++s)
#pragma unroll
            for (int q = 0; q < 2; ++q)
#pragma unroll
                for (int r = 0; r < 16; ++r) acc[s][q][r] = 0.f;

        const bool more_items = item + 1 < item_end;
        const Item wnx = more_items ? advance(w) : w;
        const __amdgpu_buffer_rsrc_t rw_nx = more_items ? make_rsrc(w_base(wnx)) : rw;
        const bool mask_cur = touches_border(w);

        for (int ch = 0; ch < nchunk; ++ch) {
            __syncthreads();
            write_tile(w, mask_cur);
            __syncthreads();

            const bool last_ch = (ch == nchunk - 1);
            const Item wp_ = last_ch ? wnx : w;
            const int chp = last_ch ? 0 : ch + 1;
            const __amdgpu_buffer_rsrc_t r_stage = make_rsrc(in_base(wp_));
            const int stage_off = chp * (CB * 4);
            __amdgpu_buffer_rsrc_t r_prev = r_stage;
            if (MODE == 1) {
                r_prev = make_rsrc(prev_base(wp_));
                if (last_ch) prev_offsets(wp_);
            }
            const int wcur_off = ch * (C::NQ * 2048);
            const __amdgpu_buffer_rsrc_t rw_over = last_ch ? rw_nx : rw;
            const int wover_off = last_ch ? 0 : (ch + 1) * (C::NQ * 2048);

            f32x4 b0 = *reinterpret_cast<const f32x4*>(lds + ldsb[0]), b1 = *reinterpret_cast<const f32x4*>(lds + ldsb[1]);
            f32x4 bn0 = b0, bn1 = b1;
#pragma unroll
            for (int tap = 0; tap < C::T; ++tap) {
#pragma unroll
                for (int G = 0; G < C::NG; ++G) {
                    const int q = tap * C::NG + G;
                    {
                        if (q + WD < C::NQ) {
                            wq[WD][0] = buf_load(rw, wlane, wcur_off + ((q + WD) * 2 + 0) * 1024);
                            wq[WD][1] = buf_load(rw, wlane, wcur_off + ((q + WD) * 2 + 1) * 1024);
                        } else {
                            wq[WD][0] = buf_load(rw_over, wlane, wover_off + ((q + WD - C::NQ) * 2 + 0) * 1024);
                            wq[WD][1] = buf_load(rw_over, wlane, wover_off + ((q + WD - C::NQ) * 2 + 1) * 1024);
                        }
                        if (q + 1 < C::NQ) {
                            const int tap1 = (q + 1) / C::NG, G1 = (q + 1) % C::NG;
                            const int toff1 = ((tap1 / KS) * C::IW + (tap1 % KS)) * C::PS + G1 * 8;
                            bn0 = *reinterpret_cast<const f32x4*>(lds + ldsb[0] + toff1);
                            bn1 = *reinterpret_cast<const f32x4*>(lds + ldsb[1] + toff1);
                        }
                    }
#pragma unroll
                    for (int s = q; s < C::ITER; s += C::NQ) issue(r_stage, stage_off, s);
                    if (MODE == 1) {
                        if (q >= C::S_PREV && q < C::S_PREV + C::AITER) pvv[q - C::S_PREV] = buf_load(r_prev, poff[q - C::S_PREV], stage_off);
                        if (q == C::S_BAR) {
                            write_prev();
                            __syncthreads();
                        }
                        if (q >= C::S_COMB && q - C::S_COMB < C::ITER) combine(q - C::S_COMB);
                    }
                    __builtin_amdgcn_sched_barrier(0);
#pragma unroll
                    for (int t = 0; t < 4; ++t) {
                        acc[0][0] = __builtin_amdgcn_mfma_f32_32x32x2f32(wq[0][0][t], b0[t], acc[0][0], 0, 0, 0);
                        acc[1][0] = __builtin_amdgcn_mfma_f32_32x32x2f32(wq[0][1][t], b0[t], acc[1][0], 0, 0, 0);
                        acc[0][1] = __builtin_amdgcn_mfma_f32_32x32x2f32(wq[0][0][t], b1[t], acc[0][1], 0, 0, 0);
                        acc[1][1] = __builtin_amdgcn_mfma_f32_32x32x2f32(wq[0][1][t], b1[t], acc[1][1], 0, 0, 0);
                    }
#pragma unroll
                    for (int d = 0; d < WD; ++d) {
                        wq[d][0] = wq[d + 1][0];
                        wq[d][1] = wq[d + 1][1];
                    }
                    b0 = bn0;
                    b1 = bn1;
                }
            }
        }

        {
            const float* bias = p.bias + w.g * p.bias_gs + w.cb * 64 + h * 4;
            const long long origin = PL ? ((((long long)w.n * p.pl_byp + (w.oy0 >> 4) + 1) * p.pl_bxp + (w.ox0 >> 4) + 1) * (p.Cout >> 4) + w.cb * 4) * 4096 + ((w.oy0 >> 2) & 3) * 64
                                        : (((long long)w.n * p.Ho + w.oy0) * p.Wo + w.ox0) * p.Cout + w.cb * 64;
            const __amdgpu_buffer_rsrc_t r_out = make_rsrc(p.out + w.g * p.out_gs + origin);
            const __amdgpu_buffer_rsrc_t r_res = make_rsrc(p.resid ? p.resid + w.g * p.resid_gs + origin : p.out);
            const bool has_res = p.resid != nullptr;
            const bool partial = (w.oy0 + TH > p.Ho) || (w.ox0 + TW > p.Wo);
#pragma unroll
            for (int q = 0; q < 2; ++q) {
                if (partial) {
                    const int pl = (wave * 2 + q) * 32 + j;
                    if (w.oy0 + pl / TW >= p.Ho || w.ox0 + pl % TW >= p.Wo) continue;
                }
#pragma unroll
                for (int s = 0; s < 2; ++s) {
#pragma unroll
                    for (int rq = 0; rq < 4; ++rq) {
                        const int co = s * 32 + rq * 8;
                        f32x4 o = {acc[s][q][rq * 4 + 0], acc[s][q][rq * 4 + 1], acc[s][q][rq * 4 + 2], acc[s][q][rq * 4 + 3]};
                        o = o + *reinterpret_cast<const f32x4*>(bias + co);
                        if (!PL && has_res) o = o + buf_load(r_res, ooff[q], co * 4);
                        if (p.relu) {
                            o[0] = fmaxf(o[0], 0.f);
                            o[1] = fmaxf(o[1], 0.f);
                            o[2] = fmaxf(o[2], 0.f);
                            o[3] = fmaxf(o[3], 0.f);
                        }
                        buf_store(o, r_out, ooff[q], PL ? (co >> 4) * 16384 + (co & 15) * 4 : co * 4);
                    }
                }
            }
        }
        if (!more_items) break;
        ++item;
        w = wnx;
        rw = rw_nx;
    }
}

template <int KS, int STRIDE, int TH, int TW, int CB, int MODE, bool PL = false>
static hipError_t launch_cfg(ConvParams p, hipStream_t st) {
    using C = ConvCfg<KS, STRIDE, TH, TW, CB, MODE>;
    p.tiles_x = (p.Wo + TW - 1) / TW;
    p.tiles_y = (p.Ho + TH - 1) / TH;
    const long long items = (long long)p.groups * p.N * p.tiles_x * p.tiles_y * (p.Cout / 64);
    auto kern = conv_igemm_kernel<KS, STRIDE, TH, TW, CB, MODE, PL>;
    static bool attr_done[64] = {};
    if (cerb_attr_needed(attr_done)) {
        hipError_t e = hipFuncSetAttribute(reinterpret_cast<const void*>(kern), hipFuncAttributeMaxDynamicSharedMemorySize, C::LDS_BYTES);
        if (e != hipSuccess) return e;
    }
    const int blocks_per_cu = (C::LDS_BYTES * 2 <= 160 * 1024) ? 2 : 1;
    long long grid = 256ll * blocks_per_cu;
    if (grid > items) grid = items;
    hipLaunchKernelGGL(kern, dim3((unsigned)grid), dim3(256), C::LDS_BYTES, st, p);
    return hipGetLastError();
}

extern "C" int cerb_conv_chunk(int ks, int stride) { return (stride == 2) ? 16 : 32; }

extern "C" size_t cerb_conv_guard_bytes(int tile_w) { return (size_t)17 * (size_t)tile_w * 64 * 4 + (64u << 10); }

hipError_t cerb_launch_conv(const ConvParams& p, int ks, int stride, int mode, hipStream_t st) {
    const bool small = p.Wo < 32;
    if (p.pl_byp > 0) {
        if (stride != 2 || mode != 0 || p.resid || (p.Ho & 15) || (p.Wo & 15) || p.Ho < 16 || p.Wo < 16 || p.groups != 1 || p.pl_byp != cerb_planar_blocks(p.Ho) ||
            p.pl_bxp != cerb_planar_blocks(p.Wo))
            return hipErrorInvalidValue;
        if (ks == 3) return small ? launch_cfg<3, 2, 16, 16, 16, 0, true>(p, st) : launch_cfg<3, 2, 8, 32, 16, 0, true>(p, st);
        if (ks == 1) return small ? launch_cfg<1, 2, 16, 16, 16, 0, true>(p, st) : launch_cfg<1, 2, 8, 32, 16, 0, true>(p, st);
        return hipErrorInvalidValue;
    }
    if (ks == 3 && stride == 1 && mode == 0) return small ? launch_cfg<3, 1, 16, 16, 32, 0>(p, st) : launch_cfg<3, 1, 8, 32, 32, 0>(p, st);
    if (ks == 3 && stride == 1 && mode == 1) return small ? launch_cfg<3, 1, 16, 16, 32, 1>(p, st) : launch_cfg<3, 1, 8, 32, 32, 1>(p, st);
    if (ks == 3 && stride == 2 && mode == 0) return small ? launch_cfg<3, 2, 16, 16, 16, 0>(p, st) : launch_cfg<3, 2, 8, 32, 16, 0>(p, st);
    if (ks == 1 && stride == 1 && mode == 0) return small ? launch_cfg<1, 1, 16, 16, 32, 0>(p, st) : launch_cfg<1, 1, 8, 32, 32, 0>(p, st);
    if (ks == 1 && stride == 2 && mode == 0) return small ? launch_cfg<1, 2, 16, 16, 16, 0>(p, st) : launch_cfg<1, 2, 8, 32, 16, 0>(p, st);
    return hipErrorInvalidValue;
}
```

cerberus_amd/csrc/dev_entry.hip:

```cpp
#include "cerb_net.h"

#define DEV_NEED(cond) \
    do {               \
        if (!(cond)) return (int)hipErrorInvalidValue; \
    } while (0)

extern "C" {

int cerb_dev_wgrad_wino_supported(int H, int W, int Cin, int Cout) { return cerb_wgrad_wino_supported(H, W, Cin, Cout) ? 1 : 0; }
size_t cerb_dev_wgrad_wino_workspace_bytes(int G, int N, int H, int W, int Cin, int Cout) {
    return cerb_wgrad_wino_supported(H, W, Cin, Cout) ? cerb_wgrad_wino_workspace_bytes(G, N, H, W, Cin, Cout) : 0;
}
int cerb_dev_wgrad_wino(const float* x, const float* dy, float* dw, float* db, int G, int N, int H, int W, int Cin, int Cout, long long x_gs, void* ws, void* st) {
    DEV_NEED(x && dy && dw && ws && G > 0 && N > 0);
    return (int)cerb_launch_wgrad_wino(x, dy, dw, G, N, H, W, Cin, Cout, x_gs, ws, (hipStream_t)st, db);
}

size_t cerb_dev_wgrad_workspace_bytes(int G, int N, int Ho, int Wo, int Cin, int Cout, int ks, int* slices_out) {
    return cerb_wgrad_workspace_bytes(G, N, Ho, Wo, Cin, Cout, ks, slices_out);
}
int cerb_dev_wgrad(const float* x, const float* dy, float* dw, float* db, int G, int N, int H, int W, int Cin, int Cout, int ks, int stride, long long x_gs, void* ws,
                   void* st) {
    DEV_NEED(x && dy && dw && ws && G > 0 && N > 0 && H > 0 && W > 0);
    return (int)cerb_launch_wgrad(x, dy, dw, G, N, H, W, Cin, Cout, ks, stride, x_gs, ws, (hipStream_t)st, db);
}

size_t cerb_dev_stem_wgrad_mfma_workspace_bytes() { return cerb_stem_wgrad_workspace_bytes(); }
int cerb_dev_stem_wgrad_mfma(const unsigned char* tiles, const float* dy, float* dw, int N, int H, int W, void* ws, void* st) {
    DEV_NEED(tiles && dy && dw && ws && N > 0 && H > 0 && W > 0);
    return (int)cerb_launch_stem_wgrad_mfma(tiles, dy, dw, N, H, W, ws, (hipStream_t)st);
}
int cerb_dev_stem_wgrad(const unsigned char* tiles, const float* dy, float* dw, int N, int H, int W, void* st) {
    DEV_NEED(tiles && dy && dw && N > 0 && H > 0 && W > 0);
    return (int)cerb_launch_stem_wgrad(tiles, dy, dw, N, H, W, (hipStream_t)st);
}

int cerb_dev_conv_bwd(const float* x, const float* dy, const float* w, float* dx, float* dw, float* db, int G, int N, int H, int W, int Cin, int Cout, int ks, int stride,
                      long long x_gs, void* st) {
    DEV_NEED(dy && (dx || dw || db) && (!dx || w) && (!dw || x) && G > 0 && N > 0 && (ks == 1 || ks == 3) && (stride == 1 || stride == 2));
    return (int)cerb_launch_conv_bwd(x, dy, w, dx, dw, db, G, N, H, W, Cin, Cout, ks, stride, x_gs, (hipStream_t)st);
}

size_t cerb_dev_bn_workspace_bytes(int groups, long long rows, int C) { return cerb_bn_workspace_bytes(groups, rows, C); }
size_t cerb_dev_bn_fold_workspace_bytes(int groups, int C) { return cerb_bn_fold_workspace_bytes(groups, C); }
int cerb_dev_bn_stats(const float* x, long long group_stride, long long rows, int C, int groups, float eps, float* mean, float* rstd, float* var_unbiased, void* ws,
                      void* st) {
    DEV_NEED(x && mean && rstd && ws && rows > 0 && groups > 0);
    return (int)cerb_launch_bn_stats(x, group_stride, rows, C, groups, eps, mean, rstd, var_unbiased, ws, (hipStream_t)st);
}
int cerb_dev_bn_finalize(const double* partial, int blocks, long long rows, int C, float eps, float* mean, float* rstd, float* var_unbiased, int groups, void* fold_ws,
                         void* st) {
    DEV_NEED(partial && mean && rstd && blocks > 0 && rows > 0 && groups > 0);
    return (int)cerb_launch_bn_finalize(partial, blocks, rows, C, eps, mean, rstd, var_unbiased, (hipStream_t)st, groups, fold_ws);
}
int cerb_dev_bn_bwd(const float* dz, const float* z, const float* y, float* dy, float* dresid, long long group_stride, long long rows, int C, int groups, const float* mean,
                    const float* rstd, const float* gamma, const float* beta, float* dgamma, float* dbeta, int relu, int dy_assign, int dresid_assign,
                    unsigned long long eval_mask, void* ws, void* st) {
    DEV_NEED(dz && y && dy && mean && rstd && gamma && dgamma && dbeta && ws && rows > 0 && groups > 0 && (!relu || z || (beta && !dresid)));
    return (int)cerb_launch_bn_bwd(dz, z, y, dy, dresid, group_stride, rows, C, groups, mean, rstd, gamma, beta, dgamma, dbeta, relu, dy_assign, ws, (hipStream_t)st, eval_mask,
                                   dresid_assign);
}

int cerb_dev_upadd_bwd_fused_ok(int H, int W, int C, int G) { return cerb_upadd_bwd_fused_ok(H, W, C, G) ? 1 : 0; }
int cerb_dev_upadd_bwd(const float* dout, float* dskip, float* dprev, int G, int N, int H, int W, int C, long long prev_gs, int shared_prev, unsigned group_mask,
                       int skip_assign, int prev_assign, void* st) {
    DEV_NEED(dout && dskip && dprev && G > 0 && N > 0 && H > 0 && W > 0 && H % 2 == 0 && W % 2 == 0 && C % 4 == 0);
    return (int)cerb_launch_upadd_bwd(dout, dskip, dprev, G, N, H, W, C, prev_gs, shared_prev, (hipStream_t)st, group_mask, skip_assign, prev_assign);
}

int cerb_dev_maxpool_idx(const float* in, float* out, unsigned* idx, int N, int H, int W, int C, void* st) {
    DEV_NEED(in && out && idx && N > 0 && H > 0 && W > 0 && C % 4 == 0);
    return (int)cerb_launch_maxpool_idx(in, out, idx, N, H, W, C, (hipStream_t)st);
}
int cerb_dev_maxpool_bwd_idx(const unsigned* idx, const float* dy, float* dx, int N, int H, int W, int C, void* st) {
    DEV_NEED(idx && dy && dx && N > 0 && H > 0 && W > 0 && H % 2 == 0 && W % 2 == 0 && C % 4 == 0);
    return (int)cerb_launch_maxpool_bwd_idx(idx, dy, dx, N, H, W, C, (hipStream_t)st);
}
int cerb_dev_maxpool_bwd(const float* x, const float* ypool, const float* dy, float* dx, int N, int H, int W, int C, void* st) {
    DEV_NEED(x && ypool && dy && dx && N > 0 && H > 0 && W > 0 && H % 2 == 0 && W % 2 == 0 && C % 4 == 0);
    return (int)cerb_launch_maxpool_bwd(x, ypool, dy, dx, N, H, W, C, (hipStream_t)st);
}

int cerb_dev_pointwise_bwd(const float* x, const float* dy, const float* w, float* dx, float* dw, float* db, long long rows, int cin, int cout, const float* in_scale,
                           int dx_assign, void* st) {
    DEV_NEED(dy && (dx || dw || db) && (!dx || w) && (!dw || x) && rows > 0 && cin > 0 && cout > 0);
    return (int)cerb_launch_pointwise_bwd(x, dy, w, dx, dw, db, rows, cin, cout, in_scale, dx_assign, (hipStream_t)st);
}
size_t cerb_dev_pw_bwd_small_workspace_bytes(long long rows, int cin, int cout) { return cerb_pw_bwd_small_workspace_bytes(rows, cin, cout); }
int cerb_dev_pw_bwd_small(const float* x, const float* dy, const float* w, float* dx, float* dw, float* db, long long rows, int cin, int cout, int dx_assign, void* ws,
                          void* st) {
    DEV_NEED(x && dy && w && ws && rows > 0 && cin > 0 && cout > 0);
    return (int)cerb_launch_pw_bwd_small(x, dy, w, dx, dw, db, rows, cin, cout, dx_assign, ws, (hipStream_t)st);
}
size_t cerb_dev_pw_wgrad_small_workspace_bytes(long long rows, int cin, int cout) { return cerb_pw_wgrad_small_workspace_bytes(rows, cin, cout); }
int cerb_dev_pw_wgrad_small(const float* x, const float* dy, float* dw, long long rows, int cin, int cout, void* ws, void* st) {
    DEV_NEED(x && dy && dw && ws && rows > 0 && cin > 0 && cout > 0);
    return (int)cerb_launch_pw_wgrad_small(x, dy, dw, rows, cin, cout, ws, (hipStream_t)st);
}

size_t cerb_dev_colsum_workspace_bytes(int C, int G) { return (size_t)G * 2048 * C * 4; }
int cerb_dev_colsum(const float* d, long long group_stride, long long rows, int C, int G, float* out, void* ws, void* st) {
    DEV_NEED(d && out && ws && rows > 0 && C > 0 && G > 0);
    return (int)cerb_launch_colsum(d, group_stride, rows, C, G, out, ws, (hipStream_t)st);
}
int cerb_dev_crop_gap(const float* x, int N, int H, int W, int C, int y0, int ch, int x0, int cw, float* out, void* st) {
    DEV_NEED(x && out && N > 0 && C > 0 && y0 >= 0 && x0 >= 0 && ch > 0 && cw > 0 && y0 + ch <= H && x0 + cw <= W);
    return (int)cerb_launch_crop_gap(x, N, H, W, C, y0, ch, x0, cw, out, (hipStream_t)st);
}
int cerb_dev_crop_gap_bwd(const float* dg, float* dx, int N, int H, int W, int C, int y0, int ch, int x0, int cw, void* st) {
    DEV_NEED(dg && dx && N > 0 && C > 0 && y0 >= 0 && x0 >= 0 && ch > 0 && cw > 0 && y0 + ch <= H && x0 + cw <= W);
    return (int)cerb_launch_crop_gap_bwd(dg, dx, N, H, W, C, y0, ch, x0, cw, (hipStream_t)st);
}
int cerb_dev_dilate2(const float* dy, float* d, long long n, int H, int W, int C, void* st) {
    DEV_NEED(dy && d && n > 0 && H > 0 && W > 0);
    return (int)cerb_launch_dilate2(dy, d, n, H, W, C, (hipStream_t)st);
}

long long cerb_devfwd_planar_elems(int N, int H, int W, int C) { return cerb_planar_elems(N, H, W, C); }
int cerb_devfwd_upsample2_add(const float* skip, const float* prev, float* out, int G, int N, int H, int W, int C, long long prev_gs, void* st) {
    DEV_NEED(skip && prev && out && G > 0 && N > 0 && H > 0 && W > 0 && H % 2 == 0 && W % 2 == 0 && C % 4 == 0);
    return (int)cerb_launch_upsample2_add(skip, prev, out, G, N, H, W, C, prev_gs, nullptr, (hipStream_t)st);
}
int cerb_devfwd_upsample2_add_planar(const float* skip, const float* prev, float* out, int G, int N, int H, int W, int C, long long prev_gs, long long out_gs,
                                     int prev_planar, void* st) {
    DEV_NEED(skip && prev && out && G > 0 && N > 0 && H > 0 && W > 0 && out_gs >= cerb_planar_elems(N, H, W, C));
    return (int)cerb_launch_upsample2_add_planar(skip, prev, out, G, N, H, W, C, prev_gs, out_gs, nullptr, prev_planar, (hipStream_t)st);
}

static int devfwd_upload(const std::vector<float>& v, float** out) {
    if (hipMalloc((void**)out, v.size() * 4) != hipSuccess) return 1;
    return hipMemcpy(*out, v.data(), v.size() * 4, hipMemcpyHostToDevice) != hipSuccess;
}
int cerb_devfwd_conv3x3(const float* w_host, const float* bias, const float* in, const float* resid, float* out, int N, int H, int W, int Cin, int Cout, int relu,
                        int planar, void* st) {
    DEV_NEED(w_host && bias && in && out && N > 0 && H >= 16 && W >= 16 && H % 16 == 0 && W % 16 == 0 && Cin % 64 == 0 && Cout % 64 == 0);
    std::vector<float> w4;
    cerb_host_pack_wino4(w_host, Cout, Cin, planar ? 0 : 1, &w4);
    float* dw = nullptr;
    DEV_NEED(devfwd_upload(w4, &dw) == 0);
    ConvParams p;
    memset(&p, 0, sizeof(p));
    p.in = in; p.wpack = dw; p.bias = bias; p.resid = resid; p.out = out;
    p.N = N; p.H = p.Ho = H; p.W = p.Wo = W; p.Cin = Cin; p.Cout = Cout; p.relu = relu; p.groups = 1;
    p.w_gs = (long long)Cout * Cin * 36; p.bias_gs = Cout; p.pk_off = 1;
    p.out_gs = planar ? cerb_planar_elems(N, H, W, Cout) : (long long)N * H * W * Cout;
    if (planar) {
        p.level_tag = resid ? 4 : 3;
        p.pl_byp = cerb_planar_blocks(H);
        p.pl_bxp = cerb_planar_blocks(W);
    }
    hipError_t e = planar ? cerb_launch_wino4p(p, (hipStream_t)st) : cerb_launch_wino4b(p, (hipStream_t)st);
    if (e == hipSuccess) e = hipStreamSynchronize((hipStream_t)st);
    (void)hipFree(dw);
    return (int)e;
}
int cerb_devfwd_conv_s2(const float* w_host, const float* bias, const float* in, float* out, int N, int H, int W, int Cin, int Cout, int ks, int relu, int planar, void* st) {
    DEV_NEED(w_host && bias && in && out && N > 0 && H % 32 == 0 && W % 32 == 0 && Cin % 16 == 0 && Cout % 64 == 0 && (ks == 1 || ks == 3));
    std::vector<float> wp;
    cerb_host_pack_conv(w_host, Cout, Cin, ks, cerb_conv_chunk(ks, 2), &wp);
    float* dw = nullptr;
    DEV_NEED(devfwd_upload(wp, &dw) == 0);
    ConvParams p;
    memset(&p, 0, sizeof(p));
    p.in = in; p.wpack = dw; p.bias = bias; p.out = out;
    p.N = N; p.H = H; p.W = W; p.Ho = H / 2; p.Wo = W / 2; p.Cin = Cin; p.Cout = Cout; p.relu = relu; p.groups = 1;
    p.w_gs = (long long)Cout * Cin * ks * ks; p.bias_gs = Cout;
    p.out_gs = planar ? cerb_planar_elems(N, p.Ho, p.Wo, Cout) : (long long)N * p.Ho * p.Wo * Cout;
    if (planar) {
        p.pl_byp = cerb_planar_blocks(p.Ho);
        p.pl_bxp = cerb_planar_blocks(p.Wo);
    }
    hipError_t e = cerb_launch_conv(p, ks, 2, 0, (hipStream_t)st);
    if (e == hipSuccess) e = hipStreamSynchronize((hipStream_t)st);
    (void)hipFree(dw);
    return (int)e;
}
int cerb_devfwd_conv(int launcher, int ks, int stride, int mode, int level_tag, const float* w_raw, int host_pack, int dgrad, const float* in, const float* prev,
                     const float* bias, const float* resid, float* out, double* bn_part, int G, int N, int H, int W, int Cin, int Cout, int relu, long long in_gs,
                     long long prev_gs, long long bias_gs, long long resid_gs, long long out_gs, const int* roi, int pk_off, int pl_byp, int pl_bxp, void* st) {
    DEV_NEED(launcher >= 0 && launcher <= 4 && w_raw && in && bias && out && G > 0 && N > 0 && H > 0 && W > 0 && Cin > 0 && Cout > 0);
    DEV_NEED(!(host_pack && dgrad) && (!bn_part || launcher == 2 || launcher == 3) && ((mode == 1) == (prev != nullptr)));
    if (launcher == 0) {
        DEV_NEED((ks == 1 || ks == 3) && (stride == 1 || stride == 2) && (mode == 0 || (mode == 1 && ks == 3 && stride == 1 && H % 2 == 0 && W % 2 == 0)));
        DEV_NEED(Cin % cerb_conv_chunk(ks, stride) == 0 && Cout % 64 == 0 && !roi && !dgrad && (stride == 1 || (H % 2 == 0 && W % 2 == 0)));
    } else {
        DEV_NEED(ks == 3 && stride == 1 && mode == 0 && Cin % ((launcher == 1 || launcher == 3) ? 32 : 16) == 0 && Cout % 64 == 0);
    }
    const hipStream_t s = (hipStream_t)st;
    const int taps = launcher == 0 ? ks * ks : (launcher == 1 ? 16 : 36);
    const size_t nw = (size_t)Cout * Cin * ks * ks, nu = (size_t)Cout * Cin * taps;
    float* dw = nullptr;
    hipError_t e = hipSuccess;
    if (host_pack) {
        std::vector<float> raw(nw * G), pk;
        DEV_NEED(hipMemcpy(raw.data(), w_raw, raw.size() * 4, hipMemcpyDeviceToHost) == hipSuccess);
        for (int g = 0; g < G; ++g) {
            if (launcher == 0) cerb_host_pack_conv(raw.data() + g * nw, Cout, Cin, ks, cerb_conv_chunk(ks, stride), &pk);
            else if (launcher == 1) cerb_host_pack_wino(raw.data() + g * nw, Cout, Cin, &pk);
            else cerb_host_pack_wino4(raw.data() + g * nw, Cout, Cin, launcher == 3 ? 1 : 0, &pk);
        }
        DEV_NEED(pk.size() == nu * G && devfwd_upload(pk, &dw) == 0);
    } else {
        DEV_NEED(hipMalloc((void**)&dw, nu * G * 4) == hipSuccess);
        if (launcher >= 2) {
            e = cerb_launch_pack_wino4(w_raw, dw, Cout, Cin, dgrad, launcher == 3 ? 1 : 0, G, s);
        } else {
            for (int g = 0; g < G && e == hipSuccess; ++g)
                e = launcher == 0 ? cerb_launch_pack_conv(w_raw + g * nw, dw + g * nu, Cout, Cin, ks, cerb_conv_chunk(ks, stride), s)
                                  : cerb_launch_pack_wino(w_raw + g * nw, dw + g * nu, Cout, Cin, dgrad, s);
        }
    }
    ConvParams p;
    memset(&p, 0, sizeof(p));
    p.in = in; p.prev = prev; p.wpack = dw; p.bias = bias; p.resid = resid; p.out = out; p.bn_part = bn_part;
    p.N = N; p.H = H; p.W = W; p.Cin = Cin; p.Cout = Cout; p.relu = relu; p.groups = G;
    p.Ho = stride == 2 ? H / 2 : H;
    p.Wo = stride == 2 ? W / 2 : W;
    p.in_gs = in_gs; p.prev_gs = prev_gs; p.w_gs = (long long)nu; p.bias_gs = bias_gs; p.resid_gs = resid_gs; p.out_gs = out_gs;
    if (roi) { p.roi_y0 = roi[0]; p.roi_y1 = roi[1]; p.roi_x0 = roi[2]; p.roi_x1 = roi[3]; }
    p.pk_off = pk_off; p.level_tag = level_tag; p.pl_byp = pl_byp; p.pl_bxp = pl_bxp;
    if (e == hipSuccess) {
        switch (launcher) {
            case 0: e = cerb_launch_conv(p, ks, stride, mode, s); break;
            case 1: e = cerb_launch_wino(p, s); break;
            case 2: e = cerb_launch_wino4(p, s); break;
            case 3: e = cerb_launch_wino4b(p, s); break;
            default: e = cerb_launch_wino4p(p, s); break;
        }
    }
    const hipError_t es = hipStreamSynchronize(s);
    if (e == hipSuccess) e = es;
    (void)hipFree(dw);
    return (int)e;
}
static ConvParams devfwd_geom(int N, int H, int W, int Cin, int Cout, int pk_off) {
    ConvParams q;
    memset(&q, 0, sizeof(q));
    q.N = N; q.H = q.Ho = H; q.W = q.Wo = W; q.Cin = Cin; q.Cout = Cout; q.pk_off = pk_off;
    return q;
}
int cerb_devfwd_wino4b_packed(int N, int H, int W, int Cin, int Cout, int pk_off) { return cerb_wino4b_packed(devfwd_geom(N, H, W, Cin, Cout, pk_off)) ? 1 : 0; }
int cerb_devfwd_wino4b_bn_blocks(int N, int H, int W, int Cin, int Cout, int pk_off) { return cerb_wino4b_bn_blocks(devfwd_geom(N, H, W, Cin, Cout, pk_off)); }

int cerb_devfwd_maxpool(const float* in, float* out, int N, int H, int W, int C, int planar, void* st) {
    DEV_NEED(in && out && N > 0 && H > 0 && W > 0 && C % 4 == 0);
    return (int)(planar ? cerb_launch_maxpool_planar(in, out, N, H, W, C, (hipStream_t)st) : cerb_launch_maxpool(in, out, N, H, W, C, (hipStream_t)st));
}
int cerb_devfwd_planar_to_nhwc(const float* in, float* out, int N, int H, int W, int C, void* st) {
    DEV_NEED(in && out && N > 0);
    return (int)cerb_launch_planar_to_nhwc(in, out, N, H, W, C, (hipStream_t)st);
}

int cerb_devfwd_stem(const unsigned char* tiles, const float* tiles_f32, const float* w_raw, const float* scale, const float* shift, int host_pack, float* out, int N,
                     int H, int W, int relu, void* st) {
    DEV_NEED((tiles != nullptr) != (tiles_f32 != nullptr) && w_raw && scale && shift && out && N > 0 && H > 0 && W > 0);
    const hipStream_t s = (hipStream_t)st;
    float *dw = nullptr, *db = nullptr;
    hipError_t e = hipSuccess;
    if (host_pack) {
        std::vector<float> raw(64 * 147), wp;
        DEV_NEED(hipMemcpy(raw.data(), w_raw, raw.size() * 4, hipMemcpyDeviceToHost) == hipSuccess);
        cerb_host_pack_stem(raw.data(), scale, &wp);
        DEV_NEED(devfwd_upload(wp, &dw) == 0);
    } else {
        for (int c = 0; c < 64; ++c) DEV_NEED(scale[c] == 1.f);
        DEV_NEED(hipMalloc((void**)&dw, 7 * 12 * 2 * 64 * 4) == hipSuccess);
        e = cerb_launch_pack_stem(w_raw, dw, s);
    }
    if (devfwd_upload(std::vector<float>(shift, shift + 64), &db) != 0) e = hipErrorOutOfMemory;
    StemParams p;
    memset(&p, 0, sizeof(p));
    p.tiles = tiles; p.tiles_f32 = tiles_f32; p.wpack = dw; p.bias = db; p.out = out; p.N = N; p.H = H; p.W = W; p.relu = relu;
    if (e == hipSuccess) e = cerb_launch_stem(p, s);
    const hipError_t es = hipStreamSynchronize(s);
    if (e == hipSuccess) e = es;
    (void)hipFree(dw);
    (void)hipFree(db);
    return (int)e;
}

struct DevHead {
    const float *w1, *b1, *scale, *shift, *w2, *b2;
    int out_ch, kind, crop_y0, crop_x0, out_h, out_w, roi, pad_;
    float* logits;
    float* out_inst;
    unsigned char* out_type_u8;
    long long* out_type_i64;
    const long long* tile_off;
    long long tile_stride, row_stride;
    unsigned int* absmax_bits;
};
int cerb_devfwd_head(int launcher, const float* feat, int feat_planar, int N, int H, int W, const DevHead* heads, int n_heads, void* st) {
    DEV_NEED(launcher >= 0 && launcher <= 2 && feat && heads && N > 0 && H > 0 && W > 0 && n_heads >= 1 && n_heads <= 8);
    DEV_NEED(launcher != 0 || (n_heads == 1 && !feat_planar));
    for (int i = 0; i < n_heads; ++i) {
        const DevHead& h = heads[i];
        DEV_NEED(h.w1 && h.b1 && h.scale && h.shift && h.w2 && h.b2 && h.out_ch >= 2 && h.out_ch <= 8 && (h.kind == 0 || h.kind == 1));
        DEV_NEED(h.kind == 1 || h.out_ch == 2 || h.out_ch == 3);
        DEV_NEED(h.crop_y0 >= 0 && h.crop_x0 >= 0 && h.out_h > 0 && h.out_w > 0 && h.crop_y0 + h.out_h <= H && h.crop_x0 + h.out_w <= W);
        DEV_NEED(!(h.roi && h.logits) && (h.kind == 0 ? h.out_inst != nullptr : (h.out_type_u8 || h.out_type_i64)));
    }
    const hipStream_t s = (hipStream_t)st;
    HeadParams hp[8];
    std::vector<float*> owned;
    hipError_t e = hipSuccess;
    for (int i = 0; i < n_heads && e == hipSuccess; ++i) {
        const DevHead& h = heads[i];
        std::vector<float> pk[5];
        cerb_host_pack_head(h.w1, h.b1, h.scale, h.shift, h.w2, h.b2, h.out_ch, &pk[0], &pk[1], &pk[2], &pk[3], &pk[4]);
        float* d[5] = {nullptr, nullptr, nullptr, nullptr, nullptr};
        for (int k = 0; k < 5; ++k) {
            if (devfwd_upload(pk[k], &d[k]) != 0) e = hipErrorOutOfMemory;
            owned.push_back(d[k]);
        }
        HeadParams& p = hp[i];
        memset(&p, 0, sizeof(p));
        p.feat = feat; p.w1p = d[0]; p.b1 = d[1]; p.w2p = d[2]; p.b2 = d[3]; p.w2q = d[4];
        p.N = N; p.H = H; p.W = W; p.out_ch = h.out_ch; p.kind = h.kind;
        p.crop_y0 = h.crop_y0; p.crop_x0 = h.crop_x0; p.out_h = h.out_h; p.out_w = h.out_w; p.roi = h.roi;
        p.logits = h.logits; p.out_inst = h.out_inst; p.out_type_u8 = h.out_type_u8; p.out_type_i64 = h.out_type_i64;
        p.tile_off = h.tile_off; p.tile_stride = h.tile_stride; p.row_stride = h.row_stride; p.absmax_bits = h.absmax_bits;
        p.feat_planar = feat_planar;
        if (feat_planar) { p.pl_byp = cerb_planar_blocks(H); p.pl_bxp = cerb_planar_blocks(W); }
    }
    if (e == hipSuccess) e = launcher == 0 ? cerb_launch_head(hp[0], s) : cerb_launch_head_group(hp, n_heads, s, launcher == 2);
    const hipError_t es = hipStreamSynchronize(s);
    if (e == hipSuccess) e = es;
    for (float* q : owned) (void)hipFree(q);
    return (int)e;
}

int cerb_devfwd_patch_class(const float* x4, const float* bn1_scale, const float* bn1_shift, const float* w1, const float* b1, const float* bn2_scale,
                            const float* bn2_shift, const float* w2, const float* b2, int N, int Hf, int Wf, int out_ch, int out_h, int out_w, float* logits, float* out,
                            const long long* tile_off, long long tile_stride, long long row_stride, void* st) {
    DEV_NEED(x4 && bn1_scale && bn1_shift && w1 && b1 && bn2_scale && bn2_shift && w2 && b2 && N > 0 && Hf > 0 && Wf > 0 && out_ch >= 1 && out_ch <= 16);
    DEV_NEED((logits || out) && (!out || (out_h > 0 && out_w > 0)));
    const hipStream_t s = (hipStream_t)st;
    std::vector<float> pk[4];
    cerb_host_pack_patch_class(w1, b1, bn2_scale, bn2_shift, w2, b2, out_ch, &pk[0], &pk[1], &pk[2], &pk[3]);
    float* d[6] = {nullptr, nullptr, nullptr, nullptr, nullptr, nullptr};
    hipError_t e = hipSuccess;
    for (int k = 0; k < 4; ++k)
        if (devfwd_upload(pk[k], &d[k]) != 0) e = hipErrorOutOfMemory;
    if (devfwd_upload(std::vector<float>(bn1_scale, bn1_scale + 512), &d[4]) != 0) e = hipErrorOutOfMemory;
    if (devfwd_upload(std::vector<float>(bn1_shift, bn1_shift + 512), &d[5]) != 0) e = hipErrorOutOfMemory;
    PatchClassParams p;
    memset(&p, 0, sizeof(p));
    p.x4 = x4; p.bn1_s = d[4]; p.bn1_b = d[5]; p.w1t = d[0]; p.b1 = d[1]; p.w2t = d[2]; p.b2 = d[3];
    p.N = N; p.Hf = Hf; p.Wf = Wf; p.out_ch = out_ch; p.out_h = out_h; p.out_w = out_w; p.logits = logits; p.out = out;
    p.tile_off = tile_off; p.tile_stride = tile_stride; p.row_stride = row_stride;
    if (e == hipSuccess) e = cerb_launch_patch_class(p, s);
    const hipError_t es = hipStreamSynchronize(s);
    if (e == hipSuccess) e = es;
    for (float* q : d) (void)hipFree(q);
    return (int)e;
}

int cerb_devfwd_upsample2_add_roi(const float* skip, const float* prev, float* out, int G, int N, int H, int W, int C, long long prev_gs, const int* roi, void* st) {
    DEV_NEED(skip && prev && out && G > 0 && N > 0 && H > 0 && W > 0 && H % 2 == 0 && W % 2 == 0 && C % 4 == 0);
    DEV_NEED(!roi || (roi[0] >= 0 && roi[0] <= roi[1] && roi[1] <= H && roi[2] >= 0 && roi[2] <= roi[3] && roi[3] <= W));
    return (int)cerb_launch_upsample2_add(skip, prev, out, G, N, H, W, C, prev_gs, roi, (hipStream_t)st);
}
int cerb_devfwd_upsample2_add_planar_roi(const float* skip, const float* prev, float* out, int G, int N, int H, int W, int C, long long prev_gs, long long out_gs,
                                         const int* roi, int prev_planar, void* st) {
    DEV_NEED(skip && prev && out && G > 0 && N > 0 && H > 0 && W > 0 && out_gs >= cerb_planar_elems(N, H, W, C));
    DEV_NEED(!roi || (roi[0] >= 0 && roi[0] <= roi[1] && roi[1] <= H && roi[2] >= 0 && roi[2] <= roi[3] && roi[3] <= W));
    return (int)cerb_launch_upsample2_add_planar(skip, prev, out, G, N, H, W, C, prev_gs, out_gs, roi, prev_planar, (hipStream_t)st);
}

int cerb_dev_head_train_supported(long long rows, int cin, int chid, int out) { return cerb_head_train_supported(rows, cin, chid, out) ? 1 : 0; }
int cerb_dev_head_fwd1(const float* prev, const float* w1, const float* b1, float* hid, long long rows, double* bn_part, int* bn_blocks, const float* in_mean,
                       const float* in_rstd, const float* in_gamma, const float* in_beta, void* st) {
    DEV_NEED(prev && w1 && b1 && hid && rows > 0);
    DEV_NEED((in_mean != nullptr) == (in_rstd != nullptr) && (in_mean != nullptr) == (in_gamma != nullptr) && (in_mean != nullptr) == (in_beta != nullptr));
    const float* in_bn[4] = {in_mean, in_rstd, in_gamma, in_beta};
    return (int)cerb_launch_head_fwd1(prev, w1, b1, hid, rows, bn_part, bn_blocks, (hipStream_t)st, in_mean ? in_bn : nullptr);
}
int cerb_dev_head_fwd2(const float* hid, const float* mean, const float* rstd, const float* gamma, const float* beta, const float* w2, const float* b2, float* logits,
                       long long rows, int out, void* st) {
    DEV_NEED(hid && mean && rstd && gamma && beta && w2 && b2 && logits && rows > 0 && out > 0);
    return (int)cerb_launch_head_fwd2(hid, mean, rstd, gamma, beta, w2, b2, logits, rows, out, (hipStream_t)st);
}
size_t cerb_dev_head_bwd_workspace_bytes(long long rows, int out) { return rows > 0 && out > 0 ? cerb_head_bwd_workspace_bytes(rows, out) : 0; }
int cerb_dev_head_bwd1(const float* hid, const float* dlog, const float* mean, const float* rstd, const float* gamma, const float* beta, const float* w2, float* dw2,
                       float* db2, float* dgamma, float* dbeta, long long rows, int out, void* ws, void* st) {
    DEV_NEED(hid && dlog && mean && rstd && gamma && beta && w2 && dw2 && db2 && dgamma && dbeta && ws && rows > 0 && rows % 16 == 0);
    return (int)cerb_launch_head_bwd1(hid, dlog, mean, rstd, gamma, beta, w2, dw2, db2, dgamma, dbeta, rows, out, ws, (hipStream_t)st);
}
int cerb_dev_head_bwd2(const float* hid, const float* dlog, const float* prev, const float* mean, const float* rstd, const float* gamma, const float* beta,
                       const float* dgamma, const float* dbeta, const float* w1, const float* w2, float* dprev, float* dw1, float* db1, long long rows, int out, int eval_mode,
                       int assign, void* ws, const float* in_mean, const float* in_rstd, const float* in_gamma, const float* in_beta, double* in_part, int* in_blocks,
                       void* st) {
    DEV_NEED(hid && dlog && prev && mean && rstd && gamma && beta && dgamma && dbeta && w1 && w2 && dprev && dw1 && db1 && ws && rows > 0);
    DEV_NEED((in_mean != nullptr) == (in_rstd != nullptr) && (in_mean != nullptr) == (in_gamma != nullptr) && (in_mean != nullptr) == (in_beta != nullptr));
    DEV_NEED(!in_part || in_mean);
    if (in_blocks) *in_blocks = (int)std::min<long long>(rows / 64, cerb_head_bwd2_blocks());
    const float* in_bn[4] = {in_mean, in_rstd, in_gamma, in_beta};
    return (int)cerb_launch_head_bwd2(hid, dlog, prev, mean, rstd, gamma, beta, dgamma, dbeta, w1, w2, dprev, dw1, db1, rows, out, eval_mode, assign, ws, (hipStream_t)st,
                                      in_mean ? in_bn : nullptr, in_part);
}
int cerb_dev_pointwise(const float* in, const float* w, const float* bias, float* out, long long rows, int cin, int cout, const float* in_scale, double* bn_part,
                       int* bn_blocks, void* st) {
    DEV_NEED(in && w && bias && out && rows > 0 && cin > 0 && cout > 0);
    return (int)cerb_launch_pointwise(in, w, bias, out, rows, cin, cout, in_scale, (hipStream_t)st, bn_part, bn_blocks);
}
int cerb_dev_bn_apply(float* x, const float* src, const float* resid, long long group_stride, long long rows, int C, int groups, const float* mean, const float* rstd,
                      const float* gamma, const float* beta, int relu, void* st) {
    DEV_NEED(x && mean && rstd && gamma && beta && rows > 0 && C > 0 && groups > 0 && group_stride >= rows * C);
    return (int)cerb_launch_bn_apply(x, src, resid, group_stride, rows, C, groups, mean, rstd, gamma, beta, relu, (hipStream_t)st);
}

}
```

cerberus_amd/csrc/net_kernels.hip:

```cpp
#include "cerb_common.h"

struct StemParams {
    const unsigned char* tiles;
    const float* tiles_f32;
    const float* wpack;
    const float* bias;
    float* out;
    int N, H, W, tiles_x, tiles_y;
    int relu;
};

template <bool F32IN>
__global__ __launch_bounds__(256, 2) void stem_conv7x7_kernel(StemParams p) {
    constexpr int TH = 8, TW = 32, IH = TH + 6, IW = TW + 6, ROW = 120;
    __shared__ __attribute__((aligned(16))) float wl[7 * 12 * 2 * 64];
    __shared__ __attribute__((aligned(16))) float xl[IH * ROW];
    const int tid = threadIdx.x, lane = tid & 63, wave = tid >> 6, j = lane & 31, h = lane >> 5;
    for (int i = tid; i < 7 * 12 * 2 * 64; i += 256) wl[i] = p.wpack[i];
    const int ntile = p.N * p.tiles_y * p.tiles_x;
    for (int tile = blockIdx.x; tile < ntile; tile += gridDim.x) {
        int t_ = tile;
        const int tx = t_ % p.tiles_x;
        t_ /= p.tiles_x;
        const int ty = t_ % p.tiles_y;
        const int n = t_ / p.tiles_y;
        const int oy0 = ty * TH, ox0 = tx * TW;
        __syncthreads();
        const unsigned char* img = F32IN ? nullptr : p.tiles + (long long)n * p.H * p.W * 3;
        const float* imgf = F32IN ? p.tiles_f32 + (long long)n * p.H * p.W * 3 : nullptr;
        for (int i = tid; i < IH * ROW; i += 256) {
            const int iy = i / ROW, c = i % ROW;
            const int gy = oy0 - 3 + iy, gx = ox0 - 3 + c / 3;
            float v = 0.f;
            if (c < IW * 3 && gy >= 0 && gy < p.H && gx >= 0 && gx < p.W) {
                const long long at = ((long long)gy * p.W + gx) * 3 + c % 3;
                v = (F32IN ? imgf[at] : (float)img[at]) / 255.0f;
            }
            xl[i] = v;
        }
        __syncthreads();
        f32x16 acc[2][2];
#pragma unroll
        for (int s = 0; s < 2; ++s)
#pragma unroll
            for (int q = 0; q < 2; ++q)
#pragma unroll
                for (int r = 0; r < 16; ++r) acc[s][q][r] = 0.f;
        const int b0 = (wave * 2 + 0) * ROW + j * 3 + h;
        const int b1 = (wave * 2 + 1) * ROW + j * 3 + h;
#pragma unroll
        for (int ky = 0; ky < 7; ++ky) {
#pragma unroll
            for (int t = 0; t < 12; ++t) {
                const float a0 = wl[((ky * 12 + t) * 2 + 0) * 64 + lane];
                const float a1 = wl[((ky * 12 + t) * 2 + 1) * 64 + lane];
                const float x0 = xl[b0 + ky * ROW + 2 * t];
                const float x1 = xl[b1 + ky * ROW + 2 * t];
                acc[0][0] = __builtin_amdgcn_mfma_f32_32x32x2f32(a0, x0, acc[0][0], 0, 0, 0);
                acc[1][0] = __builtin_amdgcn_mfma_f32_32x32x2f32(a1, x0, acc[1][0], 0, 0, 0);
                acc[0][1] = __builtin_amdgcn_mfma_f32_32x32x2f32(a0, x1, acc[0][1], 0, 0, 0);
                acc[1][1] = __builtin_amdgcn_mfma_f32_32x32x2f32(a1, x1, acc[1][1], 0, 0, 0);
            }
        }
#pragma unroll
        for (int q = 0; q < 2; ++q) {
            const int oy = oy0 + wave * 2 + q, ox = ox0 + j;
            if (oy >= p.H || ox >= p.W) continue;
            float* o = p.out + (((long long)n * p.H + oy) * p.W + ox) * 64;
#pragma unroll
            for (int s = 0; s < 2; ++s)
#pragma unroll
                for (int rq = 0; rq < 4; ++rq) {
                    const int co = s * 32 + rq * 8 + h * 4;
                    f32x4 v = {acc[s][q][rq * 4 + 0], acc[s][q][rq * 4 + 1], acc[s][q][rq * 4 + 2], acc[s][q][rq * 4 + 3]};
                    v = v + *reinterpret_cast<const f32x4*>(p.bias + co);
                    const float floor_ = p.relu ? 0.f : -3.402823466e38f;
                    v[0] = fmaxf(v[0], floor_);
                    v[1] = fmaxf(v[1], floor_);
                    v[2] = fmaxf(v[2], floor_);
                    v[3] = fmaxf(v[3], floor_);
                    *reinterpret_cast<f32x4*>(o + co) = v;
                }
        }
    }
}

hipError_t cerb_launch_stem(StemParams p, hipStream_t st) {
    p.tiles_x = (p.W + 31) / 32;
    p.tiles_y = (p.H + 7) / 8;
    const long long ntile = (long long)p.N * p.tiles_x * p.tiles_y;
    const unsigned grid = (unsigned)(ntile < 256 * 6 ? ntile : 256 * 6);
    if (p.tiles) hipLaunchKernelGGL(stem_conv7x7_kernel<false>, dim3(grid), dim3(256), 0, st, p);
    else hipLaunchKernelGGL(stem_conv7x7_kernel<true>, dim3(grid), dim3(256), 0, st, p);
    return hipGetLastError();
}

__global__ void maxpool3x3s2_kernel(const float* __restrict__ in, float* __restrict__ out, int N, int H, int W, int C, int Ho, int Wo) {
    const long long total = (long long)N * Ho * Wo * (C / 4);
    const long long per_xcd = gridDim.x / 8, vb = (long long)(blockIdx.x & 7) * per_xcd + (blockIdx.x >> 3);
    for (long long i = vb * (long long)blockDim.x + threadIdx.x; i < total; i += (long long)gridDim.x * blockDim.x) {
        const int c4 = (int)(i % (C / 4));
        long long r = i / (C / 4);
        const int ox = (int)(r % Wo);
        r /= Wo;
        const int oy = (int)(r % Ho);
        const int n = (int)(r / Ho);
        f32x4 m = {-INFINITY, -INFINITY, -INFINITY, -INFINITY};
#pragma unroll
        for (int ky = 0; ky < 3; ++ky) {
            const int y = oy * 2 - 1 + ky;
            if (y < 0 || y >= H) continue;
#pragma unroll
            for (int kx = 0; kx < 3; ++kx) {
                const int x = ox * 2 - 1 + kx;
                if (x < 0 || x >= W) continue;
                const f32x4 v = *reinterpret_cast<const f32x4*>(in + (((long long)n * H + y) * W + x) * C + c4 * 4);
                m[0] = fmaxf(m[0], v[0]);
                m[1] = fmaxf(m[1], v[1]);
                m[2] = fmaxf(m[2], v[2]);
                m[3] = fmaxf(m[3], v[3]);
            }
        }
        *reinterpret_cast<f32x4*>(out + i * 4) = m;
    }
}

__global__ void maxpool3x3s2_idx_kernel(const float* __restrict__ in, float* __restrict__ out, unsigned* __restrict__ idx, int N, int H, int W, int C, int Ho, int Wo) {
    const long long total = (long long)N * Ho * Wo * (C / 4);
    const long long per_xcd = gridDim.x / 8, vb = (long long)(blockIdx.x & 7) * per_xcd + (blockIdx.x >> 3);
    for (long long i = vb * (long long)blockDim.x + threadIdx.x; i < total; i += (long long)gridDim.x * blockDim.x) {
        const int c4 = (int)(i % (C / 4));
        long long r = i / (C / 4);
        const int ox = (int)(r % Wo);
        r /= Wo;
        const int oy = (int)(r % Ho);
        const int n = (int)(r / Ho);
        f32x4 m = {-INFINITY, -INFINITY, -INFINITY, -INFINITY};
        unsigned w0 = 0, w1 = 0, w2 = 0, w3 = 0;
        bool first = true;
#pragma unroll
        for (int ky = 0; ky < 3; ++ky) {
            const int y = oy * 2 - 1 + ky;
            if (y < 0 || y >= H) continue;
#pragma unroll
            for (int kx = 0; kx < 3; ++kx) {
                const int x = ox * 2 - 1 + kx;
                if (x < 0 || x >= W) continue;
                const f32x4 v = *reinterpret_cast<const f32x4*>(in + (((long long)n * H + y) * W + x) * C + c4 * 4);
                const unsigned k = (unsigned)(ky * 3 + kx);
                if (first || v[0] > m[0]) w0 = k;
                if (first || v[1] > m[1]) w1 = k;
                if (first || v[2] > m[2]) w2 = k;
                if (first || v[3] > m[3]) w3 = k;
                first = false;
                m[0] = fmaxf(m[0], v[0]);
                m[1] = fmaxf(m[1], v[1]);
                m[2] = fmaxf(m[2], v[2]);
                m[3] = fmaxf(m[3], v[3]);
            }
        }
        *reinterpret_cast<f32x4*>(out + i * 4) = m;
        idx[i] = w0 | (w1 << 8) | (w2 << 16) | (w3 << 24);
    }
}

hipError_t cerb_launch_maxpool_idx(const float* in, float* out, unsigned* idx, int N, int H, int W, int C, hipStream_t st) {
    const int Ho = (H + 2 - 3) / 2 + 1, Wo = (W + 2 - 3) / 2 + 1;
    const long long total = (long long)N * Ho * Wo * (C / 4);
    long long blocks = ((total + 255) / 256 + 7) / 8 * 8;
    if (blocks > 256 * 64) blocks = 256 * 64;
    hipLaunchKernelGGL(maxpool3x3s2_idx_kernel, dim3((unsigned)blocks), dim3(256), 0, st, in, out, idx, N, H, W, C, Ho, Wo);
    return hipGetLastError();
}

hipError_t cerb_launch_maxpool(const float* in, float* out, int N, int H, int W, int C, hipStream_t st) {
    const int Ho = (H + 2 - 3) / 2 + 1, Wo = (W + 2 - 3) / 2 + 1;
    const long long total = (long long)N * Ho * Wo * (C / 4);
    long long blocks = ((total + 255) / 256 + 7) / 8 * 8;
    if (blocks > 256 * 64) blocks = 256 * 64;
    hipLaunchKernelGGL(maxpool3x3s2_kernel, dim3((unsigned)blocks), dim3(256), 0, st, in, out, N, H, W, C, Ho, Wo);
    return hipGetLastError();
}

__global__ void maxpool3x3s2_planar_kernel(const float* __restrict__ in, float* __restrict__ out, int N, int H, int W, int C, int Ho, int Wo) {
    const long long total = (long long)N * Ho * Wo * (C / 4);
    const int byp = cerb_planar_blocks(Ho), bxp = cerb_planar_blocks(Wo), ncc = C >> 4;
    const long long per_xcd = gridDim.x / 8, vb = (long long)(blockIdx.x & 7) * per_xcd + (blockIdx.x >> 3);
    for (long long i = vb * (long long)blockDim.x + threadIdx.x; i < total; i += (long long)gridDim.x * blockDim.x) {
        const int c4 = (int)(i % (C / 4));
        long long r = i / (C / 4);
        const int ox = (int)(r % Wo);
        r /= Wo;
        const int oy = (int)(r % Ho);
        const int n = (int)(r / Ho);
        f32x4 m = {-INFINITY, -INFINITY, -INFINITY, -INFINITY};
#pragma unroll
        for (int ky = 0; ky < 3; ++ky) {
            const int y = oy * 2 - 1 + ky;
            if (y < 0 || y >= H) continue;
#pragma unroll
            for (int kx = 0; kx < 3; ++kx) {
                const int x = ox * 2 - 1 + kx;
                if (x < 0 || x >= W) continue;
                const f32x4 v = *reinterpret_cast<const f32x4*>(in + (((long long)n * H + y) * W + x) * C + c4 * 4);
                m[0] = fmaxf(m[0], v[0]);
                m[1] = fmaxf(m[1], v[1]);
                m[2] = fmaxf(m[2], v[2]);
                m[3] = fmaxf(m[3], v[3]);
            }
        }
        *reinterpret_cast<f32x4*>(out + cerb_planar_offset(n, oy, ox, c4 >> 2, byp, bxp, ncc) + (c4 & 3) * 4) = m;
    }
}

hipError_t cerb_launch_maxpool_planar(const float* in, float* out, int N, int H, int W, int C, hipStream_t st) {
    const int Ho = (H + 2 - 3) / 2 + 1, Wo = (W + 2 - 3) / 2 + 1;
    if (C % 64 || (Ho & 15) || (Wo & 15) || Ho < 16 || Wo < 16) return hipErrorInvalidValue;
    const long long total = (long long)N * Ho * Wo * (C / 4);
    long long blocks = ((total + 255) / 256 + 7) / 8 * 8;
    if (blocks > 256 * 64) blocks = 256 * 64;
    hipLaunchKernelGGL(maxpool3x3s2_planar_kernel, dim3((unsigned)blocks), dim3(256), 0, st, in, out, N, H, W, C, Ho, Wo);
    return hipGetLastError();
}

__global__ __launch_bounds__(256) void planar_to_nhwc_kernel(const float* __restrict__ in, float* __restrict__ out, int N, int H, int W, int C) {
    const int ncc = C >> 4, ncb = C >> 6, nby = H >> 4, nbx = W >> 4, byp = nby + 2, bxp = nbx + 2;
    const int q = threadIdx.x & 15, pp = threadIdx.x >> 4;
    const int nwork = N * nby * nbx * ncb;
    for (int wk = blockIdx.x; wk < nwork; wk += gridDim.x) {
        const int blk = wk / ncb, cb = wk % ncb;
        const int bx = blk % nbx, r_ = blk / nbx, by = r_ % nby, n = r_ / nby;
        const float* ib = in + ((((long long)n * byp + by + 1) * bxp + bx + 1) * ncc + cb * 4 + (q >> 2)) * 4096 + (q & 3) * 4;
        float* ob = out + (((long long)n * H + 16 * by) * W + 16 * bx) * C + cb * 64 + q * 4;
#pragma unroll
        for (int k = 0; k < 16; ++k) {
            const int y = k, x = pp;
            const f32x4 v = *reinterpret_cast<const f32x4*>(ib + (((y & 3) * 4 + (x & 3)) * 16 + (y >> 2) * 4 + (x >> 2)) * 16);
            *reinterpret_cast<f32x4*>(ob + ((long long)y * W + x) * C) = v;
        }
    }
}

hipError_t cerb_launch_planar_to_nhwc(const float* in, float* out, int N, int H, int W, int C, hipStream_t st) {
    if (C % 64 || (H & 15) || (W & 15) || H < 16 || W < 16) return hipErrorInvalidValue;
    const long long nwork = (long long)N * (H / 16) * (W / 16) * (C / 64);
    if (nwork >= (1ll << 31)) return hipErrorInvalidValue;
    const long long blocks = nwork < 256 * 16 ? nwork : 256 * 16;
    hipLaunchKernelGGL(planar_to_nhwc_kernel, dim3((unsigned)blocks), dim3(256), 0, st, in, out, N, H, W, C);
    return hipGetLastError();
}

__device__ __forceinline__ f32x4 blend2(float a, const f32x4& x, float b, const f32x4& y) {
    f32x4 r;
#pragma unroll
    for (int e = 0; e < 4; ++e) r[e] = __builtin_fmaf(a, x[e], b * y[e]);
    return r;
}
__global__ void upsample2_add_kernel(const float* __restrict__ skip, const float* __restrict__ prev, float* __restrict__ out, int groups,
                                     int N, int H, int W, int C, long long prev_gs, int bm_lo, int bm_cnt, int bn_lo, int bn_cnt) {
    const int Hp = H >> 1, Wp = W >> 1, C4 = C >> 2;
    const long long total = (long long)N * bm_cnt * bn_cnt * C4;
    const long long out_gs = (long long)N * H * W * C;
    for (long long i = blockIdx.x * (long long)blockDim.x + threadIdx.x; i < total; i += (long long)gridDim.x * blockDim.x) {
        const int c4 = (int)(i % C4);
        long long r = i / C4;
        const int bn = (int)(r % bn_cnt) + bn_lo;
        r /= bn_cnt;
        const int bm = (int)(r % bm_cnt) + bm_lo;
        const int n = (int)(r / bm_cnt);
        const int m0 = max(bm, 0), m1 = min(bm + 1, Hp - 1), n0 = max(bn, 0), n1 = min(bn + 1, Wp - 1);
        f32x4 sk[2][2];
        bool ok[2][2];
        long long o[2][2];
#pragma unroll
        for (int dy = 0; dy < 2; ++dy)
#pragma unroll
            for (int dx = 0; dx < 2; ++dx) {
                const int y = 2 * bm + 1 + dy, x = 2 * bn + 1 + dx;
                ok[dy][dx] = y >= 0 && y < H && x >= 0 && x < W;
                o[dy][dx] = (((long long)n * H + y) * W + x) * C + c4 * 4;
                if (ok[dy][dx]) sk[dy][dx] = *reinterpret_cast<const f32x4*>(skip + o[dy][dx]);
            }
        const long long pb = (long long)n * Hp * Wp * C + c4 * 4;
        for (int g = 0; g < groups; ++g) {
            const float* pg = prev + g * prev_gs + pb;
            const f32x4 p00 = *reinterpret_cast<const f32x4*>(pg + ((long long)m0 * Wp + n0) * C);
            const f32x4 p01 = *reinterpret_cast<const f32x4*>(pg + ((long long)m0 * Wp + n1) * C);
            const f32x4 p10 = *reinterpret_cast<const f32x4*>(pg + ((long long)m1 * Wp + n0) * C);
            const f32x4 p11 = *reinterpret_cast<const f32x4*>(pg + ((long long)m1 * Wp + n1) * C);
            const f32x4 top_l = blend2(0.75f, p00, 0.25f, p01), top_r = blend2(0.25f, p00, 0.75f, p01);
            const f32x4 bot_l = blend2(0.75f, p10, 0.25f, p11), bot_r = blend2(0.25f, p10, 0.75f, p11);
            const f32x4 u[2][2] = {{blend2(0.75f, top_l, 0.25f, bot_l), blend2(0.75f, top_r, 0.25f, bot_r)},
                                   {blend2(0.25f, top_l, 0.75f, bot_l), blend2(0.25f, top_r, 0.75f, bot_r)}};
#pragma unroll
            for (int dy = 0; dy < 2; ++dy)
#pragma unroll
                for (int dx = 0; dx < 2; ++dx)
                    if (ok[dy][dx]) __builtin_nontemporal_store(sk[dy][dx] + u[dy][dx], reinterpret_cast<f32x4*>(out + g * out_gs + o[dy][dx]));
        }
    }
}

hipError_t cerb_launch_upsample2_add(const float* skip, const float* prev, float* out, int groups, int N, int H, int W, int C,
                                     long long prev_gs, const int* roi, hipStream_t st) {
    int bm_lo = -1, bm_hi = H / 2 - 1, bn_lo = -1, bn_hi = W / 2 - 1;
    if (roi && roi[1] > roi[0] && roi[3] > roi[2]) {
        auto lo = [](int v) { return (v - 2 >= 0 ? (v - 2) / 2 : -1); };
        bm_lo = lo(roi[0]);
        bn_lo = lo(roi[2]);
        if ((roi[1] - 1) / 2 < bm_hi) bm_hi = (roi[1] - 1) / 2;
        if ((roi[3] - 1) / 2 < bn_hi) bn_hi = (roi[3] - 1) / 2;
    }
    const int bm_cnt = bm_hi - bm_lo + 1, bn_cnt = bn_hi - bn_lo + 1;
    const long long total = (long long)N * bm_cnt * bn_cnt * (C / 4);
    long long blocks = (total + 255) / 256;
    if (blocks > 256 * 32) blocks = 256 * 32;
    if (blocks < 1) blocks = 1;
    hipLaunchKernelGGL(upsample2_add_kernel, dim3((unsigned)blocks), dim3(256), 0, st, skip, prev, out, groups, N, H, W, C, prev_gs, bm_lo, bm_cnt, bn_lo,
                       bn_cnt);
    return hipGetLastError();
}

template <bool PREV_PLANAR, int C>
__global__ __launch_bounds__(256) void upsample2_add_planar_kernel(const float* __restrict__ skip, const float* __restrict__ prev, float* __restrict__ out,
                                                                   int groups, int N, int H, int W, long long prev_gs, long long out_gs, int byp, int bxp,
                                                                   int by_lo, int by_cnt, int bx_lo, int bx_cnt) {
    static_assert(C % 64 == 0, "four 16-channel planes per pass");
    constexpr int NCC = C / 16, NPASS = NCC / 4;
    const int Hp = H >> 1, Wp = W >> 1;
    const int lane = threadIdx.x & 63, m = lane >> 2, cq = lane & 3, ty = m >> 2, tx = m & 3;
    const int nwork = N * by_cnt * bx_cnt * NPASS;
    for (int wk = blockIdx.x; wk < nwork; wk += gridDim.x) {
        const int blk = wk / NPASS, cc = (wk % NPASS) * 4 + (int)(threadIdx.x >> 6);
        const int bx = blk % bx_cnt + bx_lo;
        const int r_ = blk / bx_cnt;
        const int by = r_ % by_cnt + by_lo, n = r_ / by_cnt;
        const int y0 = 16 * by + 4 * ty, x0 = 16 * bx + 4 * tx;
        if (y0 >= H || x0 >= W) continue;
        const int ch = cc * 16 + cq * 4;
        f32x4 sk[4][4];
#pragma unroll
        for (int i = 0; i < 4; ++i)
#pragma unroll
            for (int j = 0; j < 4; ++j) sk[i][j] = *reinterpret_cast<const f32x4*>(skip + (((long long)n * H + y0 + i) * W + x0 + j) * C + ch);
        int rr[4], qq[4];
#pragma unroll
        for (int k = 0; k < 4; ++k) {
            rr[k] = min(max((y0 >> 1) - 1 + k, 0), Hp - 1);
            qq[k] = min(max((x0 >> 1) - 1 + k, 0), Wp - 1);
        }
        float* ob = out + ((((long long)n * byp + by + 1) * bxp + bx + 1) * NCC + cc) * 4096 + lane * 4;
        long long pcol[4];
        if constexpr (PREV_PLANAR) {
#pragma unroll
            for (int k = 0; k < 4; ++k) pcol[k] = (long long)((qq[k] >> 4) + 1) * NCC * 4096 + ((qq[k] & 3) * 16 + ((qq[k] >> 2) & 3)) * 16;
        }
        const int pbyp = cerb_planar_blocks(Hp), pbxp = cerb_planar_blocks(Wp);
        for (int g = 0; g < groups; ++g) {
            const float* pg = PREV_PLANAR ? prev + g * prev_gs + (long long)cc * 4096 + cq * 4 : prev + g * prev_gs + (long long)n * Hp * Wp * C + ch;
            f32x4 h[4][4];
#pragma unroll
            for (int k = 0; k < 4; ++k) {
                f32x4 p0, p1, p2, p3;
                if constexpr (PREV_PLANAR) {
                    const float* pr = pg + (((long long)n * pbyp + (rr[k] >> 4) + 1) * pbxp) * NCC * 4096 + (((rr[k] & 3) << 2) * 16 + (((rr[k] >> 2) & 3) << 2)) * 16;
                    p0 = *reinterpret_cast<const f32x4*>(pr + pcol[0]); p1 = *reinterpret_cast<const f32x4*>(pr + pcol[1]);
                    p2 = *reinterpret_cast<const f32x4*>(pr + pcol[2]); p3 = *reinterpret_cast<const f32x4*>(pr + pcol[3]);
                } else {
                    const float* pr = pg + (long long)rr[k] * Wp * C;
                    p0 = *reinterpret_cast<const f32x4*>(pr + (long long)qq[0] * C); p1 = *reinterpret_cast<const f32x4*>(pr + (long long)qq[1] * C);
                    p2 = *reinterpret_cast<const f32x4*>(pr + (long long)qq[2] * C); p3 = *reinterpret_cast<const f32x4*>(pr + (long long)qq[3] * C);
                }
                h[k][0] = blend2(0.25f, p0, 0.75f, p1);
                h[k][1] = blend2(0.75f, p1, 0.25f, p2);
                h[k][2] = blend2(0.25f, p1, 0.75f, p2);
                h[k][3] = blend2(0.75f, p2, 0.25f, p3);
            }
            float* og = ob + g * out_gs;
#pragma unroll
            for (int j = 0; j < 4; ++j) {
                const f32x4 u0 = blend2(0.25f, h[0][j], 0.75f, h[1][j]), u1 = blend2(0.75f, h[1][j], 0.25f, h[2][j]), u2 = blend2(0.25f, h[1][j], 0.75f, h[2][j]),
                            u3 = blend2(0.75f, h[2][j], 0.25f, h[3][j]);
#ifndef UPP_PLAIN_STORE
                __builtin_nontemporal_store(sk[0][j] + u0, reinterpret_cast<f32x4*>(og + (0 * 4 + j) * 256));
                __builtin_nontemporal_store(sk[1][j] + u1, reinterpret_cast<f32x4*>(og + (1 * 4 + j) * 256));
                __builtin_nontemporal_store(sk[2][j] + u2, reinterpret_cast<f32x4*>(og + (2 * 4 + j) * 256));
                __builtin_nontemporal_store(sk[3][j] + u3, reinterpret_cast<f32x4*>(og + (3 * 4 + j) * 256));
#else
                *reinterpret_cast<f32x4*>(og + (0 * 4 + j) * 256) = sk[0][j] + u0;
                *reinterpret_cast<f32x4*>(og + (1 * 4 + j) * 256) = sk[1][j] + u1;
                *reinterpret_cast<f32x4*>(og + (2 * 4 + j) * 256) = sk[2][j] + u2;
                *reinterpret_cast<f32x4*>(og + (3 * 4 + j) * 256) = sk[3][j] + u3;
#endif
            }
        }
    }
}

hipError_t cerb_launch_upsample2_add_planar(const float* skip, const float* prev, float* out, int groups, int N, int H, int W, int C, long long prev_gs,
                                            long long out_gs, const int* roi, int prev_planar, hipStream_t st) {
    if ((C != 64 && C != 128 && C != 256) || (H & 3) || (W & 3)) return hipErrorInvalidValue;
    int by_lo = 0, by_hi = (H + 15) / 16, bx_lo = 0, bx_hi = (W + 15) / 16;
    if (roi && roi[1] > roi[0] && roi[3] > roi[2]) {
        by_lo = roi[0] / 16; by_hi = (roi[1] + 15) / 16;
        bx_lo = roi[2] / 16; bx_hi = (roi[3] + 15) / 16;
    }
    const long long nblk = (long long)N * (by_hi - by_lo) * (bx_hi - bx_lo);
    if (nblk <= 0 || nblk >= (1ll << 31)) return hipErrorInvalidValue;
#ifndef UPP_GRID
#define UPP_GRID 16
#endif
    const long long nwork = nblk * (C / 64);
    if (nwork >= (1ll << 31)) return hipErrorInvalidValue;
    long long blocks = nwork < 256 * UPP_GRID ? nwork : 256 * UPP_GRID;
    auto kern = C == 64    ? (prev_planar ? upsample2_add_planar_kernel<true, 64> : upsample2_add_planar_kernel<false, 64>)
                : C == 128 ? (prev_planar ? upsample2_add_planar_kernel<true, 128> : upsample2_add_planar_kernel<false, 128>)
                           : (prev_planar ? upsample2_add_planar_kernel<true, 256> : upsample2_add_planar_kernel<false, 256>);
    hipLaunchKernelGGL(kern, dim3((unsigned)blocks), dim3(256), 0, st, skip, prev, out, groups, N, H, W, prev_gs, out_gs,
                       cerb_planar_blocks(H), cerb_planar_blocks(W), by_lo, by_hi - by_lo, bx_lo, bx_hi - bx_lo);
    return hipGetLastError();
}

#ifndef HEAD_TPW
#define HEAD_TPW 2
#endif
typedef float f32x4h __attribute__((ext_vector_type(4)));
__device__ __forceinline__ void head_absmax_commit(unsigned int* word, float m) {
#pragma unroll
    for (int o = 32; o >= 1; o >>= 1) m = fmaxf(m, __shfl_xor(m, o));
    if ((threadIdx.x & 63) == 0) {
        const unsigned int b = __float_as_uint(m);
        if (b > __atomic_load_n(word, __ATOMIC_RELAXED)) atomicMax(word, b);
    }
}

template <bool ROI>
__global__ __launch_bounds__(256, 2) void head_kernel(HeadParams p) {
    const int tid = threadIdx.x, lane = tid & 63, px = lane & 15, ks = lane >> 4;
    const f32x4h* w1v = reinterpret_cast<const f32x4h*>(p.w1p) + lane;
    const f32x4h* w2v = reinterpret_cast<const f32x4h*>(p.w2p) + lane;
    struct BPos {
        int n, row, xb;
    };
    auto inc = [&](BPos b) {
        if (++b.xb == p.nxb) {
            b.xb = 0;
            if (++b.row == p.rows) {
                b.row = 0;
                ++b.n;
            }
        }
        return b;
    };
    const long long npix = (long long)p.N * p.H * p.W;
    long long pbase = ((long long)blockIdx.x * 4 + (tid >> 6)) * (64 * HEAD_TPW);
    BPos cur[4], nxt[4];
    if constexpr (ROI) {
        const int wave = __builtin_amdgcn_readfirstlane(tid >> 6);
        const unsigned nblk = (unsigned)p.N * (unsigned)p.rows * (unsigned)p.nxb;
        const unsigned b0 = ((unsigned)blockIdx.x * 4u + (unsigned)wave) * (4u * HEAD_TPW);
        const unsigned bc = b0 < nblk ? b0 : nblk;
        const unsigned r = bc / (unsigned)p.nxb;
        cur[0].xb = (int)(bc - r * (unsigned)p.nxb);
        cur[0].n = (int)(r / (unsigned)p.rows);
        cur[0].row = (int)(r - (unsigned)cur[0].n * (unsigned)p.rows);
#pragma unroll
        for (int pb = 1; pb < 4; ++pb) cur[pb] = inc(cur[pb - 1]);
        nxt[0] = inc(cur[3]);
#pragma unroll
        for (int pb = 1; pb < 4; ++pb) nxt[pb] = inc(nxt[pb - 1]);
    }
    auto ptr_of = [&](const BPos& b) {
        const int n = min(b.n, p.N - 1), x = min(p.xa0 + 16 * b.xb + px, p.W - 1);
        return p.feat + (((long long)n * p.H + p.row0 + b.row) * p.W + x) * 64 + 4 * ks;
    };
    auto feat_ptr = [&](int pb, bool next) {
        if constexpr (ROI) return ptr_of(next ? nxt[pb] : cur[pb]);
        const long long P = pbase + (next ? 64 : 0) + pb * 16 + px;
        return p.feat + (P < npix ? P : npix - 1) * 64 + 4 * ks;
    };
    f32x4h x[4];
#pragma unroll
    for (int pb = 0; pb < 4; ++pb) x[pb] = *reinterpret_cast<const f32x4h*>(feat_ptr(pb, false));
    float amax = 0.f;
#pragma unroll 1
    for (int task = 0; task < HEAD_TPW; ++task, pbase += 64) {
    f32x4h acc1[6][4];
#pragma unroll
    for (int blk = 0; blk < 6; ++blk) {
        const f32x4h bb = *reinterpret_cast<const f32x4h*>(p.b1 + blk * 16 + ks * 4);
#pragma unroll
        for (int pb = 0; pb < 4; ++pb) acc1[blk][pb] = bb;
    }
    const float* xp[4];
#pragma unroll
    for (int pb = 0; pb < 4; ++pb) xp[pb] = feat_ptr(pb, false);
#pragma unroll
    for (int g = 0; g < 4; ++g) {
        f32x4h xn[4];
        if (g + 1 < 4) {
#pragma unroll
            for (int pb = 0; pb < 4; ++pb) xn[pb] = *reinterpret_cast<const f32x4h*>(xp[pb] + (g + 1) * 16);
        } else if (task + 1 < HEAD_TPW) {
#pragma unroll
            for (int pb = 0; pb < 4; ++pb) xn[pb] = *reinterpret_cast<const f32x4h*>(feat_ptr(pb, true));
        }
#pragma unroll
        for (int blk = 0; blk < 6; ++blk) {
            const f32x4h a = w1v[(blk * 4 + g) * 64];
#pragma unroll
            for (int t = 0; t < 4; ++t)
#pragma unroll
                for (int pb = 0; pb < 4; ++pb) acc1[blk][pb] = __builtin_amdgcn_mfma_f32_16x16x4f32(a[t], x[pb][t], acc1[blk][pb], 0, 0, 0);
        }
        if (g + 1 < 4 || task + 1 < HEAD_TPW) {
#pragma unroll
            for (int pb = 0; pb < 4; ++pb) x[pb] = xn[pb];
        }
    }
#pragma unroll
    for (int blk = 0; blk < 6; ++blk)
#pragma unroll
        for (int pb = 0; pb < 4; ++pb)
#pragma unroll
            for (int r = 0; r < 4; ++r) acc1[blk][pb][r] = fmaxf(acc1[blk][pb][r], 0.f);
    f32x4h acc2[4];
    {
        const f32x4h b2 = *reinterpret_cast<const f32x4h*>(p.b2 + 4 * ks);
#pragma unroll
        for (int pb = 0; pb < 4; ++pb) acc2[pb] = b2;
    }
#pragma unroll
    for (int blk = 0; blk < 6; ++blk) {
        const f32x4h a = w2v[blk * 64];
#pragma unroll
        for (int r = 0; r < 4; ++r)
#pragma unroll
            for (int pb = 0; pb < 4; ++pb) acc2[pb] = __builtin_amdgcn_mfma_f32_16x16x4f32(a[r], acc1[blk][pb][r], acc2[pb], 0, 0, 0);
    }
    float lg[8];
#pragma unroll
    for (int e = 0; e < 4; ++e) {
        float lo = 0.f, hi = 0.f;
#pragma unroll
        for (int pb = 0; pb < 4; ++pb) {
            const float t0 = __shfl(acc2[pb][e], px), t1 = __shfl(acc2[pb][e], 16 + px);
            lo = (ks == pb) ? t0 : lo;
            hi = (ks == pb) ? t1 : hi;
        }
        lg[e] = lo;
        lg[4 + e] = hi;
    }
    int n, y_, x_;
    if constexpr (ROI) {
        int xb_ = cur[0].xb;
        n = cur[0].n;
        y_ = cur[0].row;
#pragma unroll
        for (int pb = 1; pb < 4; ++pb) {
            n = (ks == pb) ? cur[pb].n : n;
            y_ = (ks == pb) ? cur[pb].row : y_;
            xb_ = (ks == pb) ? cur[pb].xb : xb_;
        }
        y_ += p.row0;
        x_ = p.xa0 + 16 * xb_ + px;
#pragma unroll
        for (int pb = 0; pb < 4; ++pb) cur[pb] = nxt[pb];
        nxt[0] = inc(cur[3]);
#pragma unroll
        for (int pb = 1; pb < 4; ++pb) nxt[pb] = inc(nxt[pb - 1]);
        if (n >= p.N || x_ >= p.W) continue;
    } else {
        const long long P = pbase + ks * 16 + px;
        if (P >= npix) continue;
        x_ = (int)(P % p.W);
        const long long r_ = P / p.W;
        y_ = (int)(r_ % p.H);
        n = (int)(r_ / p.H);
    }
    if (p.logits) {
        const long long P = ((long long)n * p.H + y_) * p.W + x_;
        for (int e = 0; e < p.out_ch; ++e) p.logits[P * p.out_ch + e] = lg[e];
    }
    float mx = lg[0];
#pragma unroll
    for (int e = 1; e < 8; ++e)
        if (e < p.out_ch) mx = fmaxf(mx, lg[e]);
    float ex[8], sum = 0.f;
#pragma unroll
    for (int e = 0; e < 8; ++e) {
        ex[e] = (e < p.out_ch) ? expf(lg[e] - mx) : 0.f;
        sum += ex[e];
    }
    const int cy = y_ - p.crop_y0, cx = x_ - p.crop_x0;
    const bool inside = cy >= 0 && cy < p.out_h && cx >= 0 && cx < p.out_w;
    if (inside || p.logits) {
#pragma unroll
        for (int e = 0; e < 8; ++e)
            if (e < p.out_ch) amax = fmaxf(amax, fabsf(lg[e]));
    }
    if (!inside) continue;
    const long long dst = (p.tile_off ? p.tile_off[n] : (long long)n * p.tile_stride) + (long long)cy * p.row_stride + cx;
    if (p.kind == 0 && p.out_ch == 2) {
        p.out_inst[dst] = ex[1] / sum;
    } else if (p.kind == 0) {
        float2 o;
        o.x = ex[1] / sum;
        o.y = ex[2] / sum;
        *reinterpret_cast<float2*>(p.out_inst + dst * 2) = o;
    } else {
        int best = 0;
        float bv = ex[0] / sum;
#pragma unroll
        for (int e = 1; e < 8; ++e) {
            const float pe = ex[e] / sum;
            if (e < p.out_ch && pe > bv) {
                bv = pe;
                best = e;
            }
        }
        if (p.out_type_i64) p.out_type_i64[dst] = best;
        if (p.out_type_u8) p.out_type_u8[dst] = (unsigned char)best;
    }
    }
    if (p.absmax_bits) head_absmax_commit(p.absmax_bits, amax);
}

hipError_t cerb_launch_head(const HeadParams& p_in, hipStream_t st) {
    HeadParams p = p_in;
    if (p.W % 16) return hipErrorInvalidValue;
    p.rows = p.H; p.row0 = 0; p.xa0 = 0; p.nxb = p.W / 16;
    if (p.roi && !p.logits && p.out_h > 0 && p.out_w > 0) {
        p.rows = p.out_h; p.row0 = p.crop_y0;
        p.xa0 = p.crop_x0 & ~15;
        p.nxb = (p.crop_x0 + p.out_w - p.xa0 + 15) / 16;
    }
    const long long nblk = (long long)p.N * p.rows * p.nxb;
    const long long blocks = (nblk + 16 * HEAD_TPW - 1) / (16 * HEAD_TPW);
    if (p.rows == p.H && p.nxb * 16 == p.W) hipLaunchKernelGGL(head_kernel<false>, dim3((unsigned)blocks), dim3(256), 0, st, p);
    else hipLaunchKernelGGL(head_kernel<true>, dim3((unsigned)blocks), dim3(256), 0, st, p);
    return hipGetLastError();
}

#ifndef HEAD_G_TPW
#define HEAD_G_TPW 8
#endif
#ifndef HEAD_G_OCC
#define HEAD_G_OCC 3
#endif
struct HeadGroupParams {
    HeadParams h[8];
    int n_heads;
    int generic;
};
__device__ __forceinline__ float head_relu(float v) {
    float r;
    asm volatile("v_max_f32 %0, 0, %1" : "=v"(r) : "v"(v));
    return r;
}
template <bool W2_44, int OUT_CH, int KIND>
__device__ __forceinline__ void head_group_body(const HeadParams& p, const float* s_w1, const float* s_w2, const float* s_b1, const float* s_b2) {
    constexpr bool GEN = OUT_CH == 0;
    constexpr int NL = GEN ? 8 : OUT_CH;
    static_assert(GEN || W2_44, "the specialised bodies are written for the 4x4x1 second GEMM");
    const int tid = threadIdx.x, lane = tid & 63, px = lane & 15, ks = lane >> 4;
    const f32x4h* w1v = reinterpret_cast<const f32x4h*>(s_w1) + lane;
    const f32x4h* w2v = reinterpret_cast<const f32x4h*>(s_w2) + lane;
    const int out_ch = GEN ? p.out_ch : OUT_CH;
    const bool wide = GEN ? p.out_ch > 4 : OUT_CH > 4;
    const unsigned nblk = (unsigned)p.N * (unsigned)p.rows * (unsigned)p.nxb;
    const unsigned ntask = (nblk + 1u) >> 1;
    const unsigned wave = (unsigned)__builtin_amdgcn_readfirstlane(tid >> 6);
    unsigned task = ((unsigned)blockIdx.x * 4u + wave) * (unsigned)HEAD_G_TPW;
    if (task >= ntask) return;
    const unsigned task_end = min(task + (unsigned)HEAD_G_TPW, ntask);
    struct BPos {
        int n, row, xb;
    };
    auto decode = [&](unsigned b) {
        BPos r;
        const unsigned bc = min(b, nblk);
        const unsigned q = bc / (unsigned)p.nxb;
        r.xb = (int)(bc - q * (unsigned)p.nxb);
        r.n = (int)(q / (unsigned)p.rows);
        r.row = (int)(q - (unsigned)r.n * (unsigned)p.rows);
        return r;
    };
    auto inc = [&](BPos b) {
        if (++b.xb == p.nxb) {
            b.xb = 0;
            if (++b.row == p.rows) {
                b.row = 0;
                ++b.n;
            }
        }
        return b;
    };
    const int gstride = p.feat_planar ? 4096 : 16;
    auto ptr_of = [&](const BPos& b) {
        const int n = min(b.n, p.N - 1), x = min(p.xa0 + 16 * b.xb + px, p.W - 1), y = p.row0 + b.row;
        if (p.feat_planar) return p.feat + cerb_planar_offset(n, y, x, 0, p.pl_byp, p.pl_bxp, 4) + 4 * ks;
        return p.feat + (((long long)n * p.H + y) * p.W + x) * 64 + 4 * ks;
    };
    f32x4h xn[4][2];
    auto request_at = [&](const BPos& b, int pb) {
        const float* fp = ptr_of(b);
#pragma unroll
        for (int g = 0; g < 4; ++g) xn[g][pb] = *reinterpret_cast<const f32x4h*>(fp + gstride * g);
    };
    auto request = [&](unsigned t) {
        request_at(decode(2u * t), 0);
        request_at(decode(2u * t + 1u), 1);
    };
    BPos nb[2] = {};
    if constexpr (GEN) {
        request(task);
    } else {
        nb[0] = decode(2u * task);
        nb[1] = inc(nb[0]);
        request_at(nb[0], 0);
// ... 337 lines not shown
```

Measured before the change: 154.4.

## Feed tile-planar encoder outputs directly to next stage and decoder skips

Encoder stages that already produce tile-planar activations no longer convert them back to NHWC. Instead, the next stage's stride-2 entry convs (conv1 and downsample) read the planar layout directly through a new IPL variant of the igemm kernel, and the decoder's upsample-add reads the planar buffer as its skip input. Separately, when prev is a single NHWC map, the decoder sum buffer is allocated with one group instead of D. The goal is to drop the planar_to_nhwc passes and their memory traffic, at the cost of more kernel template variants and more complex addressing and eligibility logic.

```diff
diff --git a/cerberus_amd/csrc/cerb_api.hip b/cerberus_amd/csrc/cerb_api.hip
--- a/cerberus_amd/csrc/cerb_api.hip
+++ b/cerberus_amd/csrc/cerb_api.hip
@@ -572,7 +572,7 @@
 
 int run_conv(cerb_net* net, const std::string& name, const float* in, const float* prev, const float* resid, float* out, int N,
              int H, int W, int relu, int mode, long long in_gs, long long prev_gs, hipStream_t st, double* macs,
-             const int* roi, long long planar_out_gs) {
+             const int* roi, long long planar_out_gs, int in_planar) {
     auto it = net->conv.find(name);
     if (it == net->conv.end()) return fail("internal: conv " + name + " not packed");
     const PackedConv& c = it->second;
@@ -609,12 +609,15 @@
     }();
     const bool w4b = !planar && (net->conv_algo == 7 || (net->conv_algo == 6 && map_px <= w4b_max_px)) && c.cin % 64 == 0;
     const bool enc_planar = planar && net->planar_level == 4;
+    if (in_planar && (c.stride != 2 || mode != 0 || resid || !net->fold_bn || c.wino || c.groups != 1 || (planar && !enc_planar)))
+        return fail("internal: conv " + name + " cannot read a tile-planar input");
+    p.in_pl = in_planar ? 1 : 0;
     if (enc_planar && c.stride == 2) {
         if (resid || mode != 0 || !net->fold_bn) return fail("internal: conv " + name + " cannot store tile-planar");
         p.out_gs = planar_out_gs;
         p.pl_byp = cerb_planar_blocks(p.Ho);
         p.pl_bxp = cerb_planar_blocks(p.Wo);
-        const std::string kn = "conv_igemm_planar<ks" + std::to_string(c.ks) + ",s2" + (p.Wo < 32 ? ",16x16>" : ",8x32>");
+        const std::string kn = "conv_igemm_planar<ks" + std::to_string(c.ks) + ",s2" + (p.Wo < 32 ? ",16x16" : ",8x32") + (in_planar ? ",in-planar>" : ">");
         if (prof_begin(net, name, kn, fl, st)) return 1;
         HIP_OK(cerb_launch_conv(p, c.ks, c.stride, mode, st));
         if (prof_end(net, st)) return 1;
@@ -675,7 +678,7 @@
         return 0;
     }
     const std::string kn = "conv_igemm<ks" + std::to_string(c.ks) + ",s" + std::to_string(c.stride) + ",mode" + std::to_string(mode) +
-                           (p.Wo < 32 ? ",16x16>" : ",8x32>");
+                           (p.Wo < 32 ? ",16x16" : ",8x32") + (in_planar ? ",in-planar>" : ">");
     if (prof_begin(net, name, kn, fl, st)) return 1;
     HIP_OK(cerb_launch_conv(p, c.ks, c.stride, mode, st));
     if (prof_end(net, st)) return 1;
@@ -710,10 +713,51 @@
         }
         return true;
     };
+    const int enc_mask = [] {
+        const char* e = cerb_dev_getenv("CERB_ENC_PLANAR");
+        return e ? atoi(e) : kEncPlanarStages;
+    }();
+    auto encoder_stage_is_planar = [&](int li) {
+        if (dry || !net->planar || !net->fold_bn || net->conv_algo != 6 || !((enc_mask >> li) & 1)) return false;
+        const int hh = hs[li + 1], ww = ws[li + 1], planes = kFilters[li + 1];
+        if ((hh & 15) || (ww & 15) || hh < 16 || ww < 16 || planes % 64) return false;
+        for (int b = 0; b < kLayers[li]; ++b)
+            for (int j = 1; j <= 2; ++j) {
+                auto c = net->conv.find("backbone.layer" + std::to_string(li + 1) + "." + std::to_string(b) + ".conv" + std::to_string(j));
+                if (c == net->conv.end()) return false;
+                if (c->second.stride == 1 && (!c->second.wino || c->second.host_w.empty() || c->second.cin % 16)) return false;
+            }
+        return true;
+    };
+    const bool side_outputs = [&] {
+        if (io->feats) return true;
+        if (io->logits)
+            for (size_t k = 0; k < net->dec.size(); ++k)
+                if (io->logits[k]) return true;
+        return false;
+    }();
+    const bool keep_exits = side_outputs || [] {
+        const char* e = cerb_dev_getenv("CERB_ENC_EXIT");
+        return e && atoi(e) != 0;
+    }();
+    auto entry_reads_planar = [&](int li) {
+        const std::string p = "backbone.layer" + std::to_string(li + 1) + ".0";
+        auto c1 = net->conv.find(p + ".conv1"), cd = net->conv.find(p + ".downsample");
+        if (c1 == net->conv.end() || cd == net->conv.end()) return false;
+        auto ok = [](const PackedConv& c, int ks) { return c.ks == ks && c.stride == 2 && c.groups == 1 && !c.wino && c.cin % 16 == 0 && c.cout % 64 == 0; };
+        return ok(c1->second, 3) && ok(cd->second, 1);
+    };
+    auto next_reads_planar = [&](int li) { return !keep_exits && li < 3 && entry_reads_planar(li + 1); };
+    auto stage_exits = [&](int li) {
+        if (keep_exits || !next_reads_planar(li)) return true;
+        return D > 0 && !level_is_planar(2 - li);
+    };
     if (!dry) {
         if (net->x0.ensure((size_t)N * H * W * 64 * 4, guard) || net->pool.ensure((size_t)N * hs[1] * ws[1] * 64 * 4, guard)) return fail_alloc();
-        for (int i = 1; i < 5; ++i)
+        for (int i = 1; i < 5; ++i) {
+            if (encoder_stage_is_planar(i - 1) && !stage_exits(i - 1)) continue;
             if (net->x[i].ensure((size_t)N * hs[i] * ws[i] * kFilters[i] * 4, guard)) return fail_alloc();
+        }
         if (net->ta.ensure((size_t)N * hs[1] * ws[1] * 64 * 4, guard) || net->tb.ensure((size_t)N * hs[1] * ws[1] * 64 * 4, guard) ||
             net->cm.ensure((size_t)N * hs[4] * ws[4] * 256 * 4, guard))
             return fail_alloc();
@@ -747,22 +791,6 @@
         HIP_OK(cerb_launch_stem(sp, st));
         if (prof_end(net, st)) return 1;
     }
-    const int enc_mask = [] {
-        const char* e = cerb_dev_getenv("CERB_ENC_PLANAR");
-        return e ? atoi(e) : kEncPlanarStages;
-    }();
-    auto encoder_stage_is_planar = [&](int li) {
-        if (dry || !net->planar || !net->fold_bn || net->conv_algo != 6 || !((enc_mask >> li) & 1)) return false;
-        const int hh = hs[li + 1], ww = ws[li + 1], planes = kFilters[li + 1];
-        if ((hh & 15) || (ww & 15) || hh < 16 || ww < 16 || planes % 64) return false;
-        for (int b = 0; b < kLayers[li]; ++b)
-            for (int j = 1; j <= 2; ++j) {
-                auto c = net->conv.find("backbone.layer" + std::to_string(li + 1) + "." + std::to_string(b) + ".conv" + std::to_string(j));
-                if (c == net->conv.end()) return false;
-                if (c->second.stride == 1 && (!c->second.wino || c->second.host_w.empty() || c->second.cin % 16)) return false;
-            }
-        return true;
-    };
     if (!dry) {
         if (encoder_stage_is_planar(0)) {
             if (net->enc_a[0].ensure(1, N, hs[1], ws[1], 64, st)) return fail_alloc();
@@ -776,6 +804,8 @@
         }
     }
     float* cur = dry ? nullptr : net->pool.p;
+    bool cur_planar = false;
+    const float* enc_skip[3] = {nullptr, nullptr, nullptr};
     int inpl = 64;
     for (int li = 0; li < 4; ++li) {
         const int planes = kFilters[li + 1];
@@ -790,18 +820,23 @@
             for (int b = 0; b < kLayers[li]; ++b) {
                 const std::string p = "backbone.layer" + std::to_string(li + 1) + "." + std::to_string(b);
                 if (b == 0 && li > 0) {
-                    if (run_conv(net, p + ".conv1", cur, nullptr, nullptr, bb.b.p, N, Hi, Wi, 1, 0, 0, 0, st, macs, nullptr, bb.gs())) return 1;
-                    if (run_conv(net, p + ".downsample", cur, nullptr, nullptr, ba.b.p, N, Hi, Wi, 0, 0, 0, 0, st, macs, nullptr, ba.gs())) return 1;
+                    if (run_conv(net, p + ".conv1", cur, nullptr, nullptr, bb.b.p, N, Hi, Wi, 1, 0, 0, 0, st, macs, nullptr, bb.gs(), cur_planar)) return 1;
+                    if (run_conv(net, p + ".downsample", cur, nullptr, nullptr, ba.b.p, N, Hi, Wi, 0, 0, 0, 0, st, macs, nullptr, ba.gs(), cur_planar)) return 1;
                 } else if (run_conv(net, p + ".conv1", ba.b.p, nullptr, nullptr, bb.b.p, N, hh, ww, 1, 0, ba.gs(), 0, st, macs, nullptr, bb.gs())) {
                     return 1;
                 }
                 if (run_conv(net, p + ".conv2", bb.b.p, nullptr, ba.b.p, ba.b.p, N, hh, ww, 1, 0, bb.gs(), 0, st, macs, nullptr, ba.gs())) return 1;
             }
-            if (prof_begin(net, "backbone.layer" + std::to_string(li + 1) + ".exit", "planar_to_nhwc", 0.0, st)) return 1;
-            HIP_OK(cerb_launch_planar_to_nhwc(ba.b.p, net->x[li + 1].p, N, hh, ww, planes, st));
-            if (prof_end(net, st)) return 1;
-            cur = net->x[li + 1].p;
             inpl = planes;
+            if (stage_exits(li)) {
+                if (prof_begin(net, "backbone.layer" + std::to_string(li + 1) + ".exit", "planar_to_nhwc", 0.0, st)) return 1;
+                HIP_OK(cerb_launch_planar_to_nhwc(ba.b.p, net->x[li + 1].p, N, hh, ww, planes, st));
+                if (prof_end(net, st)) return 1;
+            } else {
+                enc_skip[li] = ba.b.p;
+            }
+            cur_planar = next_reads_planar(li);
+            cur = cur_planar ? ba.b.p : net->x[li + 1].p;
             continue;
         }
         for (int b = 0; b < kLayers[li]; ++b) {
@@ -813,14 +848,16 @@
             float* outb = dry ? nullptr : (((kLayers[li] - 1 - b) % 2 == 0) ? net->x[li + 1].p : net->tb.p);
             (void)last;
             const float* idt = cur;
-            if (run_conv(net, p + ".conv1", cur, nullptr, nullptr, t1, N, hin, win, 1, 0, 0, 0, st, macs)) return 1;
+            if (cur_planar && stride != 2) return fail("internal: a tile-planar stage output feeds " + p + ", which has no stride-2 entry");
+            if (run_conv(net, p + ".conv1", cur, nullptr, nullptr, t1, N, hin, win, 1, 0, 0, 0, st, macs, nullptr, 0, cur_planar)) return 1;
             if (stride != 1 || inpl != planes) {
                 float* ds = dry ? nullptr : net->pool.p;
-                if (run_conv(net, p + ".downsample", cur, nullptr, nullptr, ds, N, hin, win, 0, 0, 0, 0, st, macs)) return 1;
+                if (run_conv(net, p + ".downsample", cur, nullptr, nullptr, ds, N, hin, win, 0, 0, 0, 0, st, macs, nullptr, 0, cur_planar)) return 1;
                 idt = ds;
             }
             if (run_conv(net, p + ".conv2", t1, nullptr, idt, outb, N, hs[li + 1], ws[li + 1], 1, 0, 0, 0, st, macs)) return 1;
             cur = outb;
+            cur_planar = false;
             inpl = planes;
         }
     }
@@ -888,13 +925,17 @@
                 PlanarBuf &bm = u == 3 ? net->pmid : u == 2 ? net->pmid2 : u == 1 ? net->pmid1 : net->pmid0;
                 const int cout1 = net->conv[n1].cout;
                 PlanarBuf& bo = cout1 == cin0 ? bs : u == 1 ? net->pout1 : net->pout0;
-                if (bs.ensure((int)D, N, hh, ww, cin0, st) || bm.ensure((int)D, N, hh, ww, cmid, st) || (&bo != &bs && bo.ensure((int)D, N, hh, ww, cout1, st)))
+                const bool one_sum = prev_gs == 0 && !prev_planar && &bo != &bs;
+                const int sum_groups = one_sum ? 1 : (int)D;
+                if (bs.ensure(sum_groups, N, hh, ww, cin0, st) || bm.ensure((int)D, N, hh, ww, cmid, st) || (&bo != &bs && bo.ensure((int)D, N, hh, ww, cout1, st)))
                     return fail_alloc();
+                const float* skip_pl = u < 3 ? enc_skip[2 - u] : nullptr;
                 if (prof_begin(net, n0 + ".up", kPlanarEntryFamily[u], 0.0, st)) return 1;
-                HIP_OK(cerb_launch_upsample2_add_planar(skips[u], prev, bs.b.p, (int)D, N, hh, ww, cin0, prev_gs, bs.gs(), use_roi ? roi_sum[u] : nullptr, prev_planar ? 1 : 0, st));
+                HIP_OK(cerb_launch_upsample2_add_planar(skip_pl ? skip_pl : skips[u], prev, bs.b.p, sum_groups, N, hh, ww, cin0, prev_gs, bs.gs(), use_roi ? roi_sum[u] : nullptr,
+                                                        prev_planar ? 1 : 0, st, skip_pl ? 1 : 0));
                 if (prof_end(net, st)) return 1;
                 net->planar_level = u;
-                if (run_conv(net, n0, bs.b.p, nullptr, nullptr, bm.b.p, N, hh, ww, 1, 0, bs.gs(), 0, st, macs, use_roi ? roi_mid[u] : nullptr, bm.gs()))
+                if (run_conv(net, n0, bs.b.p, nullptr, nullptr, bm.b.p, N, hh, ww, 1, 0, one_sum ? 0 : bs.gs(), 0, st, macs, use_roi ? roi_mid[u] : nullptr, bm.gs()))
                     return 1;
                 if (run_conv(net, n1, bm.b.p, nullptr, nullptr, bo.b.p, N, hh, ww, 1, 0, bm.gs(), 0, st, macs, use_roi ? roi_out[u] : nullptr, bo.gs()))
                     return 1;
diff --git a/cerberus_amd/csrc/cerb_common.h b/cerberus_amd/csrc/cerb_common.h
--- a/cerberus_amd/csrc/cerb_common.h
+++ b/cerberus_amd/csrc/cerb_common.h
@@ -23,6 +23,7 @@
     int groups;
     long long in_gs, prev_gs, w_gs, bias_gs, resid_gs, out_gs;
     int pl_byp, pl_bxp;
+    int in_pl;
     int level_tag;
     double* bn_part;
     int bn_bpg;
diff --git a/cerberus_amd/csrc/cerb_net.h b/cerberus_amd/csrc/cerb_net.h
--- a/cerberus_amd/csrc/cerb_net.h
+++ b/cerberus_amd/csrc/cerb_net.h
@@ -23,7 +23,7 @@
 bool cerb_wino4b_packed(const ConvParams& p);
 hipError_t cerb_launch_wino4p(ConvParams p, hipStream_t st);
 hipError_t cerb_launch_upsample2_add_planar(const float* skip, const float* prev, float* out, int groups, int N, int H, int W, int C, long long prev_gs,
-                                            long long out_gs, const int* roi, int prev_planar, hipStream_t st);
+                                            long long out_gs, const int* roi, int prev_planar, hipStream_t st, int skip_planar = 0);
 hipError_t cerb_launch_upsample2_add(const float* skip, const float* prev, float* out, int groups, int N, int H, int W, int C,
                                      long long prev_gs, const int* roi, hipStream_t st);
 extern "C" int cerb_conv_chunk(int ks, int stride);
@@ -316,5 +316,6 @@
 int train_wino2_fresh(cerb_net* net, const std::string& name, PackedConv& cm, int dgrad, hipStream_t st);
 int train_wino4_slot(cerb_net* net, const std::string& name, PackedConv& cm, int w4b, int dgrad, hipStream_t st, float** out);
 int run_conv(cerb_net* net, const std::string& name, const float* in, const float* prev, const float* resid, float* out, int N, int H, int W, int relu, int mode,
-             long long in_gs, long long prev_gs, hipStream_t st, double* macs, const int* roi = nullptr, long long planar_out_gs = 0);
+             long long in_gs, long long prev_gs, hipStream_t st, double* macs, const int* roi = nullptr, long long planar_out_gs = 0,
+             int in_planar = 0);
 #endif
diff --git a/cerberus_amd/csrc/conv_igemm.hip b/cerberus_amd/csrc/conv_igemm.hip
--- a/cerberus_amd/csrc/conv_igemm.hip
+++ b/cerberus_amd/csrc/conv_igemm.hip
@@ -40,9 +40,10 @@
     int g, cb, n, oy0, ox0, tx, ty;
 };
 
-template <int KS, int STRIDE, int TH, int TW, int CB, int MODE, bool PL = false>
+template <int KS, int STRIDE, int TH, int TW, int CB, int MODE, bool PL = false, bool IPL = false>
 __global__ __launch_bounds__(256, 2) void conv_igemm_kernel(ConvParams p) {
     using C = ConvCfg<KS, STRIDE, TH, TW, CB, MODE>;
+    static_assert(!IPL || (MODE == 0 && STRIDE == 2 && CB == 16 && (TH * STRIDE) % 16 == 0 && (TW * STRIDE) % 16 == 0), "planar input: stage entries only");
     constexpr int WD = C::WD;
     static_assert(TH * TW == 256, "tile must hold 256 pixels (4 waves x 2 x 32)");
     static_assert(MODE == 0 || (KS == 3 && STRIDE == 1 && CB == 32 && C::IH % C::RPS == 0 && C::S_COMB + C::ITER <= C::NQ),
@@ -99,9 +100,22 @@
         w.ox0 = w.tx * TW;
         return w;
     };
+    const int ibyp = cerb_planar_blocks(p.H), ibxp = cerb_planar_blocks(p.W), incc = p.Cin >> 4;
+    auto in_block = [&](const Item& w) {
+        return ((((long long)w.n * ibyp + ((w.oy0 * STRIDE) >> 4)) * ibxp + ((w.ox0 * STRIDE) >> 4)) * incc) * 4096;
+    };
     auto in_base = [&](const Item& w) {
+        if constexpr (IPL) return reinterpret_cast<const char*>(p.in + w.g * p.in_gs + in_block(w));
         return reinterpret_cast<const char*>(p.in + w.g * p.in_gs) +
                ((((long long)w.n * p.H + (w.oy0 * STRIDE - C::PAD)) * p.W + (w.ox0 * STRIDE - C::PAD)) * p.Cin) * 4;
+    };
+    auto in_rsrc = [&](const Item& w) {
+        if constexpr (IPL) {
+            const long long left = ((long long)p.N * ibyp * ibxp * incc * 4096 - in_block(w)) * 4;
+            return __builtin_amdgcn_make_buffer_rsrc(const_cast<char*>(in_base(w)), 0, (int)(unsigned)(left < 0xffffffffll ? left : 0xffffffffll), 0x00020000);
+        } else {
+            return make_rsrc(in_base(w));
+        }
     };
     auto w_base = [&](const Item& w) {
         return reinterpret_cast<const char*>(p.wpack + w.g * p.w_gs + (long long)w.cb * nchunk * C::NQ * 2 * 256);
@@ -133,7 +147,13 @@
         for (int s = 0; s < C::ITER; ++s) {
             const int f = min(tid + s * 256, C::NF - 1);
             const int pix = f / C::PARTS, part = f % C::PARTS;
-            soff[s] = (unsigned)((((pix / C::IW) * C::GSTEP * p.W + (pix % C::IW) * C::GSTEP) * p.Cin + part * 4) * 4);
+            if constexpr (IPL) {
+                const int dy = (pix / C::IW) * C::GSTEP - C::PAD, dx = (pix % C::IW) * C::GSTEP - C::PAD;
+                const int yy = dy & 15, xx = dx & 15;
+                soff[s] = (unsigned)(((((dy + 16) >> 4) * ibxp + ((dx + 16) >> 4)) * incc * 4096 + (((yy & 3) * 4 + (xx & 3)) * 16 + (yy >> 2) * 4 + (xx >> 2)) * 16 + part * 4) * 4);
+            } else {
+                soff[s] = (unsigned)((((pix / C::IW) * C::GSTEP * p.W + (pix % C::IW) * C::GSTEP) * p.Cin + part * 4) * 4);
+            }
         }
         ldsw0 = (tid / C::PARTS) * C::PS + (tid % C::PARTS) * 4;
     }
@@ -236,7 +256,7 @@
 
     Item w = decode(item);
     {
-        const __amdgpu_buffer_rsrc_t r0 = make_rsrc(in_base(w));
+        const __amdgpu_buffer_rsrc_t r0 = in_rsrc(w);
 #pragma unroll
         for (int s = 0; s < C::ITER; ++s) issue(r0, 0, s);
     }
@@ -279,8 +299,8 @@
             const bool last_ch = (ch == nchunk - 1);
             const Item wp_ = last_ch ? wnx : w;
             const int chp = last_ch ? 0 : ch + 1;
-            const __amdgpu_buffer_rsrc_t r_stage = make_rsrc(in_base(wp_));
-            const int stage_off = chp * (CB * 4);
+            const __amdgpu_buffer_rsrc_t r_stage = in_rsrc(wp_);
+            const int stage_off = IPL ? chp * 16384 : chp * (CB * 4);
             __amdgpu_buffer_rsrc_t r_prev = r_stage;
             if (MODE == 1) {
                 r_prev = make_rsrc(prev_base(wp_));
@@ -381,13 +401,13 @@
     }
 }
 
-template <int KS, int STRIDE, int TH, int TW, int CB, int MODE, bool PL = false>
+template <int KS, int STRIDE, int TH, int TW, int CB, int MODE, bool PL = false, bool IPL = false>
 static hipError_t launch_cfg(ConvParams p, hipStream_t st) {
     using C = ConvCfg<KS, STRIDE, TH, TW, CB, MODE>;
     p.tiles_x = (p.Wo + TW - 1) / TW;
     p.tiles_y = (p.Ho + TH - 1) / TH;
     const long long items = (long long)p.groups * p.N * p.tiles_x * p.tiles_y * (p.Cout / 64);
-    auto kern = conv_igemm_kernel<KS, STRIDE, TH, TW, CB, MODE, PL>;
+    auto kern = conv_igemm_kernel<KS, STRIDE, TH, TW, CB, MODE, PL, IPL>;
     static bool attr_done[64] = {};
     if (cerb_attr_needed(attr_done)) {
         hipError_t e = hipFuncSetAttribute(reinterpret_cast<const void*>(kern), hipFuncAttributeMaxDynamicSharedMemorySize, C::LDS_BYTES);
@@ -406,6 +426,17 @@
 
 hipError_t cerb_launch_conv(const ConvParams& p, int ks, int stride, int mode, hipStream_t st) {
     const bool small = p.Wo < 32;
+    if (p.in_pl) {
+        const bool pl = p.pl_byp > 0;
+        if (stride != 2 || mode != 0 || p.resid || (p.H & 15) || (p.W & 15) || p.H < 16 || p.W < 16 || (p.Cin & 15) || p.groups != 1 || (ks != 1 && ks != 3)) return hipErrorInvalidValue;
+        if (pl && ((p.Ho & 15) || (p.Wo & 15) || p.Ho < 16 || p.Wo < 16 || p.pl_byp != cerb_planar_blocks(p.Ho) || p.pl_bxp != cerb_planar_blocks(p.Wo))) return hipErrorInvalidValue;
+        if (ks == 3) {
+            if (pl) return small ? launch_cfg<3, 2, 16, 16, 16, 0, true, true>(p, st) : launch_cfg<3, 2, 8, 32, 16, 0, true, true>(p, st);
+            return small ? launch_cfg<3, 2, 16, 16, 16, 0, false, true>(p, st) : launch_cfg<3, 2, 8, 32, 16, 0, false, true>(p, st);
+        }
+        if (pl) return small ? launch_cfg<1, 2, 16, 16, 16, 0, true, true>(p, st) : launch_cfg<1, 2, 8, 32, 16, 0, true, true>(p, st);
+        return small ? launch_cfg<1, 2, 16, 16, 16, 0, false, true>(p, st) : launch_cfg<1, 2, 8, 32, 16, 0, false, true>(p, st);
+    }
     if (p.pl_byp > 0) {
         if (stride != 2 || mode != 0 || p.resid || (p.Ho & 15) || (p.Wo & 15) || p.Ho < 16 || p.Wo < 16 || p.groups != 1 || p.pl_byp != cerb_planar_blocks(p.Ho) ||
             p.pl_bxp != cerb_planar_blocks(p.Wo))
diff --git a/cerberus_amd/csrc/dev_entry.hip b/cerberus_amd/csrc/dev_entry.hip
--- a/cerberus_amd/csrc/dev_entry.hip
+++ b/cerberus_amd/csrc/dev_entry.hip
@@ -165,11 +165,12 @@
     p.in = in; p.wpack = dw; p.bias = bias; p.out = out;
     p.N = N; p.H = H; p.W = W; p.Ho = H / 2; p.Wo = W / 2; p.Cin = Cin; p.Cout = Cout; p.relu = relu; p.groups = 1;
     p.w_gs = (long long)Cout * Cin * ks * ks; p.bias_gs = Cout;
-    p.out_gs = planar ? cerb_planar_elems(N, p.Ho, p.Wo, Cout) : (long long)N * p.Ho * p.Wo * Cout;
-    if (planar) {
+    p.out_gs = (planar & 1) ? cerb_planar_elems(N, p.Ho, p.Wo, Cout) : (long long)N * p.Ho * p.Wo * Cout;
+    if (planar & 1) {
         p.pl_byp = cerb_planar_blocks(p.Ho);
         p.pl_bxp = cerb_planar_blocks(p.Wo);
     }
+    p.in_pl = (planar & 2) ? 1 : 0;
     hipError_t e = cerb_launch_conv(p, ks, 2, 0, (hipStream_t)st);
     if (e == hipSuccess) e = hipStreamSynchronize((hipStream_t)st);
     (void)hipFree(dw);
diff --git a/cerberus_amd/csrc/net_kernels.hip b/cerberus_amd/csrc/net_kernels.hip
--- a/cerberus_amd/csrc/net_kernels.hip
+++ b/cerberus_amd/csrc/net_kernels.hip
@@ -321,7 +321,7 @@
     return hipGetLastError();
 }
 
-template <bool PREV_PLANAR, int C>
+template <bool PREV_PLANAR, int C, bool SKIP_PLANAR = false>
 __global__ __launch_bounds__(256) void upsample2_add_planar_kernel(const float* __restrict__ skip, const float* __restrict__ prev, float* __restrict__ out,
                                                                    int groups, int N, int H, int W, long long prev_gs, long long out_gs, int byp, int bxp,
                                                                    int by_lo, int by_cnt, int bx_lo, int bx_cnt) {
@@ -338,18 +338,21 @@
         const int y0 = 16 * by + 4 * ty, x0 = 16 * bx + 4 * tx;
         if (y0 >= H || x0 >= W) continue;
         const int ch = cc * 16 + cq * 4;
+        const long long pblk = ((((long long)n * byp + by + 1) * bxp + bx + 1) * NCC + cc) * 4096 + lane * 4;
         f32x4 sk[4][4];
 #pragma unroll
         for (int i = 0; i < 4; ++i)
 #pragma unroll
-            for (int j = 0; j < 4; ++j) sk[i][j] = *reinterpret_cast<const f32x4*>(skip + (((long long)n * H + y0 + i) * W + x0 + j) * C + ch);
+            for (int j = 0; j < 4; ++j)
+                sk[i][j] = SKIP_PLANAR ? *reinterpret_cast<const f32x4*>(skip + pblk + (i * 4 + j) * 256)
+                                       : *reinterpret_cast<const f32x4*>(skip + (((long long)n * H + y0 + i) * W + x0 + j) * C + ch);
         int rr[4], qq[4];
 #pragma unroll
         for (int k = 0; k < 4; ++k) {
             rr[k] = min(max((y0 >> 1) - 1 + k, 0), Hp - 1);
             qq[k] = min(max((x0 >> 1) - 1 + k, 0), Wp - 1);
         }
-        float* ob = out + ((((long long)n * byp + by + 1) * bxp + bx + 1) * NCC + cc) * 4096 + lane * 4;
+        float* ob = out + pblk;
         long long pcol[4];
         if constexpr (PREV_PLANAR) {
 #pragma unroll
@@ -398,8 +401,9 @@
 }
 
 hipError_t cerb_launch_upsample2_add_planar(const float* skip, const float* prev, float* out, int groups, int N, int H, int W, int C, long long prev_gs,
-                                            long long out_gs, const int* roi, int prev_planar, hipStream_t st) {
+                                            long long out_gs, const int* roi, int prev_planar, hipStream_t st, int skip_planar) {
     if ((C != 64 && C != 128 && C != 256) || (H & 3) || (W & 3)) return hipErrorInvalidValue;
+    if (skip_planar && ((H & 15) || (W & 15))) return hipErrorInvalidValue;
     int by_lo = 0, by_hi = (H + 15) / 16, bx_lo = 0, bx_hi = (W + 15) / 16;
     if (roi && roi[1] > roi[0] && roi[3] > roi[2]) {
         by_lo = roi[0] / 16; by_hi = (roi[1] + 15) / 16;
@@ -416,6 +420,10 @@
     auto kern = C == 64    ? (prev_planar ? upsample2_add_planar_kernel<true, 64> : upsample2_add_planar_kernel<false, 64>)
                 : C == 128 ? (prev_planar ? upsample2_add_planar_kernel<true, 128> : upsample2_add_planar_kernel<false, 128>)
                            : (prev_planar ? upsample2_add_planar_kernel<true, 256> : upsample2_add_planar_kernel<false, 256>);
+    if (skip_planar)
+        kern = C == 64    ? (prev_planar ? upsample2_add_planar_kernel<true, 64, true> : upsample2_add_planar_kernel<false, 64, true>)
+               : C == 128 ? (prev_planar ? upsample2_add_planar_kernel<true, 128, true> : upsample2_add_planar_kernel<false, 128, true>)
+                          : (prev_planar ? upsample2_add_planar_kernel<true, 256, true> : upsample2_add_planar_kernel<false, 256, true>);
     hipLaunchKernelGGL(kern, dim3((unsigned)blocks), dim3(256), 0, st, skip, prev, out, groups, N, H, W, prev_gs, out_gs,
                        cerb_planar_blocks(H), cerb_planar_blocks(W), by_lo, by_hi - by_lo, bx_lo, bx_hi - bx_lo);
     return hipGetLastError();
```

Result: no change. 155.9, median of 6 (+1.0%).
